# adamnelsonarcher/BB-OCR

Hardware: AMD Instinct MI355X
Metric: book-page images/sec end-to-end (detect+recognize) @1280x960 (higher is better)
Workload: dtype fp16

## Files before the change

bb-ocr_amd/_lib.py:

```python
from __future__ import annotations

import ctypes as C
import os

_HERE = os.path.dirname(os.path.abspath(__file__))
LIB_PATH = os.environ.get("BBOCR_LIB_PATH") or os.path.join(_HERE, "libbbocr.so")


class bbocr_config(C.Structure):
    _fields_ = [("device", C.c_int), ("det_sub_batch", C.c_int), ("rec_max_cols", C.c_int), ("precision", C.c_int), ("call_slots", C.c_int),
                ("host_threads", C.c_int), ("reserved", C.c_int * 2)]


PRECISIONS = {"bf16": 0, "fp16": 1, "exact": 2, "mixed": 3, "exact_rec": 4}
PAGE_GRAY, PAGE_BGR, PAGE_RGB, PAGE_YCBCR4, PAGE_YCBCR3 = 0, 1, 2, 3, 4
PAGE_PX_BYTES = {PAGE_GRAY: 1, PAGE_BGR: 3, PAGE_RGB: 3, PAGE_YCBCR4: 4, PAGE_YCBCR3: 3}


class bbocr_tensor_desc(C.Structure):
    _fields_ = [("name", C.c_char_p), ("ndim", C.c_int), ("shape", C.c_int64 * 4), ("data", C.POINTER(C.c_float))]


class bbocr_params(C.Structure):
    _fields_ = [
        ("text_threshold", C.c_double), ("low_text", C.c_double), ("link_threshold", C.c_double), ("mag_ratio", C.c_double),
        ("slope_ths", C.c_double), ("ycenter_ths", C.c_double), ("height_ths", C.c_double), ("width_ths", C.c_double),
        ("add_margin", C.c_double), ("contrast_ths", C.c_double), ("adjust_contrast", C.c_double),
        ("canvas_size", C.c_int), ("min_size", C.c_int), ("ignore_mask", C.c_uint * 4), ("decoder", C.c_int), ("beam_width", C.c_int), ("rotation_info", C.c_int * 4),
    ]


class bbocr_preproc_params(C.Structure):
    _fields_ = [("scale", C.c_double), ("blur_sigma", C.c_double), ("contrast", C.c_double), ("brightness", C.c_double),
                ("clahe_clip", C.c_double), ("unsharp_radius", C.c_double), ("unsharp_percent", C.c_int), ("unsharp_threshold", C.c_int),
                ("reserved", C.c_int * 4)]


class bbocr_jpeg_plan(C.Structure):
    _fields_ = [("width", C.c_int), ("height", C.c_int), ("components", C.c_int), ("sampling", (C.c_int * 2) * 3), ("restart_interval", C.c_int),
                ("mcu_cols", C.c_int), ("mcu_rows", C.c_int), ("segments", C.c_int), ("scan_offset", C.c_longlong), ("scan_bytes", C.c_longlong),
                ("supported", C.c_int), ("reason", C.c_int), ("orientation", C.c_int), ("reserved", C.c_int * 3)]


class bbocr_boxlist(C.Structure):
    _fields_ = [
        ("n_images", C.c_int), ("poly_off", C.POINTER(C.c_int)), ("polys", C.POINTER(C.c_int)),
        ("hori_off", C.POINTER(C.c_int)), ("hori", C.POINTER(C.c_int)),
        ("free_off", C.POINTER(C.c_int)), ("free_q", C.POINTER(C.c_double)),
    ]


class bbocr_result(C.Structure):
    _fields_ = [
        ("n_images", C.c_int), ("box_off", C.POINTER(C.c_int)), ("quads", C.POINTER(C.c_double)),
        ("is_free", C.POINTER(C.c_int)), ("text_off", C.POINTER(C.c_int)), ("text_idx", C.POINTER(C.c_int)),
        ("conf", C.POINTER(C.c_double)),
    ]


_vp = C.c_void_p
PROTOTYPES = {
    "bbocr_create": (C.c_int, [C.POINTER(bbocr_config), C.POINTER(_vp)]),
    "bbocr_destroy": (None, [_vp]),
    "bbocr_last_error": (C.c_char_p, [_vp]),
    "bbocr_default_params": (None, [C.POINTER(bbocr_params)]),
    "bbocr_load_weights": (C.c_int, [_vp, C.c_int, C.POINTER(bbocr_tensor_desc), C.c_int]),
    "bbocr_alloc_weights": (C.c_int, [_vp, C.c_int]),
    "bbocr_weights_blob_size": (C.c_int, [_vp, C.POINTER(C.c_size_t)]),
    "bbocr_weights_export": (C.c_int, [_vp, _vp, C.c_size_t]),
    "bbocr_weights_import": (C.c_int, [_vp, _vp, C.c_size_t]),
    "bbocr_dist_unique_id": (C.c_int, [_vp]),
    "bbocr_dist_init": (C.c_int, [_vp, C.c_int, C.c_int, _vp]),
    "bbocr_dist_finalize": (C.c_int, [_vp]),
    "bbocr_bcast_weights": (C.c_int, [_vp, C.c_int]),
    "bbocr_scatter_images": (C.c_int, [_vp, _vp, C.c_longlong, C.c_size_t, C.c_int, _vp, C.POINTER(C.c_longlong), C.POINTER(C.c_longlong)]),
    "bbocr_gather_results": (C.c_int, [_vp, _vp, C.c_size_t, C.c_int, C.POINTER(_vp), C.POINTER(C.c_size_t)]),
    "bbocr_result_pack": (C.c_int, [C.POINTER(bbocr_result), C.POINTER(_vp), C.POINTER(C.c_size_t)]),
    "bbocr_result_unpack": (C.c_int, [_vp, C.c_size_t, C.POINTER(C.POINTER(bbocr_result))]),
    "bbocr_free_bytes": (None, [_vp]),
    "bbocr_detect_dims": (C.c_int, [C.c_int, C.c_int, C.c_int, C.c_double, C.POINTER(C.c_int), C.POINTER(C.c_int), C.POINTER(C.c_int),
                                    C.POINTER(C.c_int), C.POINTER(C.c_double)]),
    "bbocr_detect": (C.c_int, [_vp, _vp, C.c_int, C.c_int, C.c_int, C.POINTER(bbocr_params), _vp]),
    "bbocr_boxes": (C.c_int, [_vp, _vp, C.c_int, C.c_int, C.c_int, C.c_double, C.POINTER(bbocr_params), C.POINTER(C.POINTER(bbocr_boxlist))]),
    "bbocr_recognize": (C.c_int, [_vp, _vp, C.c_int, C.c_int, C.c_int, C.POINTER(bbocr_boxlist), C.POINTER(bbocr_params),
                                  C.POINTER(C.POINTER(bbocr_result))]),
    "bbocr_readtext_batch": (C.c_int, [_vp, _vp, _vp, C.c_int, C.c_int, C.c_int, C.POINTER(bbocr_params), C.POINTER(C.POINTER(bbocr_result))]),
    "bbocr_free_boxlist": (None, [C.POINTER(bbocr_boxlist)]),
    "bbocr_free_result": (None, [C.POINTER(bbocr_result)]),
    "bbocr_stage_times": (C.c_int, [_vp, C.POINTER(C.c_float), C.c_int]),
    "bbocr_set_profiling": (C.c_int, [_vp, C.c_int]),
    "bbocr_conv_profile": (C.c_int, [_vp, C.c_int, C.POINTER(C.c_double), C.POINTER(C.c_double), C.POINTER(C.c_longlong)]),
    "bbocr_host_cpu_share": (C.c_int, []),
    "bbocr_host_component_polys": (C.c_int, [C.POINTER(C.c_int), C.POINTER(C.c_int), C.c_int, C.c_int, C.c_int, C.c_double, C.POINTER(C.c_int)]),
    "bbocr_host_group_boxes": (C.c_int, [C.POINTER(C.c_int), C.c_int, C.POINTER(bbocr_params), C.POINTER(C.POINTER(bbocr_boxlist))]),
    "bbocr_host_ctc_beam": (C.c_int, [C.POINTER(C.c_float), C.c_int, C.c_int, C.c_int, C.c_int, C.c_int, C.POINTER(C.c_int), C.POINTER(C.c_int)]),
    "bbocr_op_conv2d": (C.c_int, [_vp, _vp, C.c_int, C.c_int, C.c_int, C.c_int, C.POINTER(C.c_float), C.POINTER(C.c_float), C.c_int, C.c_int,
                                  C.c_int, C.c_int, C.c_int, C.c_int, C.c_int, C.c_int, _vp, C.c_int, C.c_int, _vp]),
    "bbocr_crnn_logits": (C.c_int, [_vp, _vp, C.c_int, C.c_int, _vp]),
    "bbocr_op_ctc": (C.c_int, [_vp, _vp, C.c_int, C.c_int, C.c_int, C.c_int, C.POINTER(C.c_int), C.POINTER(C.c_int), C.POINTER(C.c_double),
                               C.POINTER(C.c_uint), C.c_int]),
    "bbocr_op_resize_u8": (C.c_int, [_vp, _vp, C.c_int, C.c_int, C.c_int, C.c_int, _vp, C.c_int, C.c_int]),
    "bbocr_op_ycc_to_rgb": (C.c_int, [_vp, _vp, C.c_size_t, C.c_int, _vp, _vp]),
    "bbocr_upload_pages": (C.c_int, [_vp, C.POINTER(C.c_void_p), C.c_int, C.c_size_t, _vp]),
    "bbocr_op_crops": (C.c_int, [_vp, _vp, C.c_int, C.c_int, C.POINTER(C.c_int), C.c_int, C.POINTER(C.c_double), C.c_int, C.c_int, C.c_float,
                                 _vp, C.POINTER(C.c_int), C.c_int]),
    "bbocr_preprocess_book_cover": (C.c_int, [_vp, _vp, C.c_int, C.c_int, _vp, C.POINTER(C.c_int), C.POINTER(C.c_int)]),
    "bbocr_preproc_defaults": (None, [C.POINTER(bbocr_preproc_params), C.c_int]),
    "bbocr_preprocess_chain": (C.c_int, [_vp, _vp, C.c_int, C.c_int, C.POINTER(bbocr_preproc_params), _vp, C.POINTER(C.c_int), C.POINTER(C.c_int)]),
    "bbocr_op_preprocess_stage": (C.c_int, [_vp, C.c_int, _vp, C.c_int, C.c_int, _vp, C.c_int, C.c_int, C.c_double]),
    "bbocr_auto_crop": (C.c_int, [_vp, _vp, C.c_int, C.c_int, C.c_longlong, C.c_int, C.c_int, C.POINTER(C.c_int), C.POINTER(C.c_int),
                                  C.POINTER(C.c_int), C.c_int, C.POINTER(C.c_int)]),
    "bbocr_op_autocrop_stage": (C.c_int, [_vp, C.c_int, _vp, C.c_int, C.c_int, C.c_longlong, C.c_int, _vp]),
    "bbocr_ocr_thumbnail": (C.c_int, [_vp, _vp, C.c_int, C.c_int, C.c_longlong, C.c_int, C.c_int, C.c_int, _vp, _vp, C.POINTER(C.c_int),
                                      C.POINTER(C.c_int)]),
    "bbocr_op_thumbnail_stage": (C.c_int, [_vp, C.c_int, _vp, C.c_int, C.c_int, C.c_longlong, C.c_int, C.c_int, C.c_int, _vp, _vp,
                                           C.POINTER(C.c_int), C.POINTER(C.c_int)]),
    "bbocr_thumbnail_dims": (C.c_int, [C.c_int, C.c_int, C.c_int, C.POINTER(C.c_int), C.POINTER(C.c_int)]),
    "bbocr_host_thumbnail_plan": (C.c_int, [C.c_int, C.c_int, C.c_int, C.POINTER(C.c_int), C.POINTER(C.c_int), C.POINTER(C.c_int),
                                            C.POINTER(C.c_int), C.POINTER(C.c_float)]),
    "bbocr_host_resample_coeffs": (C.c_int, [C.c_int, C.c_float, C.c_float, C.c_int, C.POINTER(C.c_int), C.POINTER(C.c_int), C.c_int,
                                             C.POINTER(C.c_int)]),
    "bbocr_host_jpeg_qtables": (C.c_int, [C.c_int, C.POINTER(C.c_uint16)]),
    "bbocr_host_jpeg_plan": (C.c_int, [_vp, C.c_size_t, C.POINTER(bbocr_jpeg_plan)]),
    "bbocr_jpeg_decode": (C.c_int, [_vp, C.POINTER(C.c_void_p), C.POINTER(C.c_size_t), C.c_int, C.c_int, C.POINTER(C.c_void_p),
                                    C.POINTER(C.c_longlong), C.POINTER(C.c_int)]),
    "bbocr_jpeg_imread": (C.c_int, [_vp, C.POINTER(C.c_void_p), C.POINTER(C.c_size_t), C.c_int, C.POINTER(C.c_void_p), C.POINTER(C.c_longlong),
                                    C.POINTER(C.c_int)]),
    "bbocr_page_orient": (C.c_int, [_vp, _vp, C.c_int, C.c_int, C.c_longlong, C.c_int, C.c_int, C.c_int, _vp, C.c_longlong, C.POINTER(C.c_int),
                                    C.POINTER(C.c_int)]),
    "bbocr_op_jpeg_stage": (C.c_int, [_vp, C.c_int, _vp, C.c_size_t, C.c_int, _vp, C.c_size_t, C.POINTER(C.c_int)]),
    "bbocr_jpeg_encode_bound": (C.c_size_t, [C.c_int, C.c_int, C.c_int]),
    "bbocr_host_jpeg_header": (C.c_int, [C.c_int, C.c_int, C.c_int, C.c_int, _vp, C.c_int, _vp, C.c_size_t, C.POINTER(C.c_size_t)]),
    "bbocr_jpeg_encode": (C.c_int, [_vp, _vp, C.c_int, C.c_int, C.c_longlong, C.c_int, C.c_int, C.c_int, _vp, C.c_int, _vp, C.c_size_t,
                                    C.POINTER(C.c_size_t)]),
    "bbocr_op_jpeg_encode_stage": (C.c_int, [_vp, C.c_int, _vp, C.c_int, C.c_int, C.c_longlong, C.c_int, C.c_int, C.c_int, _vp, C.c_size_t,
                                             C.POINTER(C.c_size_t)]),
}

_lib = None


def load():
    global _lib
    if _lib is not None:
        return _lib
    if not os.path.exists(LIB_PATH):
        raise RuntimeError(
            f"{LIB_PATH} is missing: the MI355X backend has no CPU fallback. "
            "Build it with `python -c 'import __graft_entry__ as g; g.build()'` (hipcc --offload-arch=gfx950).")
    try:
        import torch
    except Exception:
        pass
    lib = C.CDLL(LIB_PATH)
    for name, (res, args) in PROTOTYPES.items():
        try:
            fn = getattr(lib, name)
        except AttributeError as e:
            raise RuntimeError(f"libbbocr.so does not export {name}") from e
        fn.restype = res
        fn.argtypes = args
    _lib = lib
    return lib
```

bb-ocr_amd/csrc/abi_ops.cpp:

```cpp
#include "ctx.h"

extern "C" {

int bbocr_op_preprocess_stage(bbocr_ctx* ctx, int stage, const uint8_t* dev_src, int H, int W, uint8_t* dev_dst, int dh, int dw, double param) {
    return guarded(ctx, [&](bbocr_ctx* ctx) {
        if (!dev_src || !dev_dst || H <= 0 || W <= 0 || dh <= 0 || dw <= 0) fail(BBOCR_ERR_ARG, "bad arguments");
        if (stage != 0 && (dh != H || dw != W)) fail(BBOCR_ERR_ARG, "only stage 0 changes the size");
        const size_t n = (size_t)H * W;
        if (stage == 0) {
            pp_resize(ctx, dev_src, H, W, dev_dst, dh, dw);
        } else if (stage == 1) {
            pp_gauss(ctx, dev_src, H, W, dev_dst, param);
        } else if (stage == 2 || stage == 3) {
            if (stage == 2) {
                ctx->pp_a.ensure(n);
                pp_gauss(ctx, dev_src, H, W, (uint8_t*)ctx->pp_a.p, 0.0);
            }
            HIPCHK(launch_pp_lut(dev_src, dev_dst, pp_fold_lut(ctx, n, stage == 2 ? param : 0.0, stage == 3 ? param : 0.0), n, ctx->stream));
        } else if (stage == 4) {
            pp_clahe(ctx, dev_src, H, W, pp_fold_lut(ctx, n, 0.0, 0.0), dev_dst, param);
        } else if (stage == 5) {
            ctx->pp_b.ensure(n);
            ctx->pp_c.ensure(n);
            pp_unsharp(ctx, dev_src, H, W, dev_dst, (uint8_t*)ctx->pp_b.p, (uint8_t*)ctx->pp_c.p, (float)param, 30, 3);
        } else if (stage == 7) {
            ctx->pp_b.ensure(n);
            ctx->pp_c.ensure(n);
            pp_unsharp(ctx, dev_src, H, W, dev_dst, (uint8_t*)ctx->pp_b.p, (uint8_t*)ctx->pp_c.p, 1.0f, (int)param, 3);
        } else if (stage == 6) {
            HIPCHK(launch_gray(dev_src, dev_dst, n, ctx->stream));
        } else {
            fail(BBOCR_ERR_ARG, "unknown pre-processing stage");
        }
        slot_sync(ctx, ctx->stream);
    });
}

int bbocr_host_cpu_share(void) { return host_cpu_share(); }

int bbocr_host_component_polys(const int* comps, const int* rowext, int n, int w, int h, double ratio, int* polys_out) {
    if (!comps || !rowext || !polys_out || n < 0 || w <= 0 || h <= 0 || !(ratio > 0)) return BBOCR_ERR_ARG;
    try {
        for (int i = 0; i < n; ++i) {
            const int* q = comps + (size_t)i * 7;
            bbocr::Component cc{q[0], q[1], q[2], q[3], q[4], q[5], q[6]};
            float box[4][2];
            bbocr::component_box(cc, rowext + (size_t)cc.row_off * 2, w, h, box);
            bbocr::box_to_poly(box, 1.0 / ratio, 1.0 / ratio, polys_out + (size_t)i * 8);
        }
    } catch (...) {
        return BBOCR_ERR_INTERNAL;
    }
    return BBOCR_OK;
}

int bbocr_host_group_boxes(const int* polys, int n, const bbocr_params* p, bbocr_boxlist** out) {
    if ((!polys && n > 0) || n < 0 || !out) return BBOCR_ERR_ARG;
    try {
        bbocr_params pp;
        bbocr_default_params(&pp);
        if (p) pp = *p;
        HostBoxes hb;
        hb.polys.assign(1, {});
        hb.hori.assign(1, {});
        hb.freeb.assign(1, {});
        for (int i = 0; i < n; ++i) {
            std::array<int, 8> a;
            memcpy(a.data(), polys + (size_t)i * 8, 32);
            hb.polys[0].push_back(a);
        }
        bbocr::GroupParams gp{pp.slope_ths, pp.ycenter_ths, pp.height_ths, pp.width_ths, pp.add_margin, pp.min_size};
        bbocr::group_text_box(hb.polys[0], gp, hb.hori[0], hb.freeb[0]);
        *out = export_boxes(hb);
    } catch (...) {
        return BBOCR_ERR_INTERNAL;
    }
    return BBOCR_OK;
}

int bbocr_host_ctc_beam(const float* probs, int n, int T, int C, int cs, int beam_width, int* text_off, int* text_idx) {
    if (!probs || !text_off || !text_idx || n <= 0 || T <= 0 || C <= 0 || C > cs || beam_width <= 0) return BBOCR_ERR_ARG;
    try {
        std::vector<int> seqs;
        for (int i = 0; i < n; ++i) { seqs.push_back(i * T); seqs.push_back(T); }
        std::vector<std::vector<int>> texts;
        ctc_beam_search_batch(probs, seqs.data(), n, C, cs, beam_width, texts);
        int o = 0;
        for (int i = 0; i < n; ++i) {
            text_off[i] = o;
            for (int v : texts[i]) text_idx[o++] = v;
        }
        text_off[n] = o;
    } catch (...) {
        return BBOCR_ERR_INTERNAL;
    }
    return BBOCR_OK;
}

int bbocr_op_conv2d(bbocr_ctx* ctx, const uint16_t* dev_in, int N, int H, int W, int Cin, const float* w, const float* bias, int Cout, int KH,
                    int KW, int pad, int dil, int relu_in, int relu_out, int out_f32, void* dev_out, int pool_mode, int pool_relu,
                    uint16_t* dev_pool_out) {
    return guarded(ctx, [&](bbocr_ctx* ctx) {
        if (!dev_in || !w || Cin <= 0 || (Cin & 31) || Cout <= 0 || KH <= 0 || KW <= 0) fail(BBOCR_ERR_ARG, "bad conv arguments");
        if (pool_mode < 0 || pool_mode > 2 || (pool_mode ? (!dev_pool_out || out_f32) : !dev_out)) fail(BBOCR_ERR_ARG, "bad conv output arguments");
        ConvPlan p = make_plan(Cin, Cout, KH, KW, pad, dil, det_el(ctx));
        std::vector<float> wv(w, w + (size_t)Cout * Cin * KH * KW), bv(Cout, 0.f);
        if (bias) std::copy(bias, bias + Cout, bv.begin());
        const size_t owned0 = ctx->owned.size();
        upload_plan(ctx, p, wv, bv);
        const int store = cdiv(Cout, 16) * 16;
        ConvArgs a = conv_args(p, Act{(uint16_t*)dev_in, N, H, W, Cin});
        a.relu_in0 = relu_in != 0; a.relu_out = relu_out != 0; a.out_f32 = out_f32 != 0;
        a.out = dev_out; a.out_cs = store; a.cout_store = store;
        a.pool_mode = pool_mode; a.pool_relu = pool_relu != 0; a.store_full = (pool_mode && dev_out) ? 1 : 0; a.pool_cs = store; a.pool_out = dev_pool_out;
        a.zero = ctx->zero_page;
        const hipError_t e = launch_conv(p, a, ctx->stream);
        const hipError_t e2 = hipStreamSynchronize(ctx->stream);
        while (ctx->owned.size() > owned0) { (void)hipFree(ctx->owned.back()); ctx->owned.pop_back(); ctx->owned_bytes.pop_back(); }
        HIPCHK(e);
        HIPCHK(e2);
    }, true);
}

int bbocr_crnn_logits(bbocr_ctx* ctx, const uint16_t* dev_crops, int n, int imgW, float* dev_logits) {
    return guarded(ctx, [&](bbocr_ctx* ctx) {
        if (!ctx->crnn_loaded) fail(BBOCR_ERR_STATE, "recogniser weights not loaded");
        if (!dev_crops || !dev_logits || n <= 0 || imgW < 64 || (imgW & 63)) fail(BBOCR_ERR_ARG, "bad crop batch");
        std::vector<BoxJob> jobs(n);
        std::vector<int> all(n);
        for (int i = 0; i < n; ++i) { jobs[i].d = CropDesc{}; jobs[i].d.imgW = imgW; all[i] = i; }
        RecPart part;
        rec_plan_part(jobs, all, 0, 0, part);
        const size_t rows = part.rows, rows_pad = align_up(rows, 256);
        ctx->seq_v.ensure(rows_pad * 256 * 2 * (rec_split(ctx) ? 2 : 1));
        ctx->seq_logits.ensure(rows_pad * 112 * 4);
        const CropDesc* dd = rec_upload_descs(ctx, part, ctx->crop_desc);
        uint16_t* wide = rec_wide_image(ctx, part);
        HIPCHK(hipMemsetAsync(wide, 0, 64 * part.cols * 2, ctx->stream));
        for (int i = 0; i < n; ++i)
            HIPCHK(hipMemcpy2DAsync(wide + part.descs[i].slot, part.cols * 2, dev_crops + (size_t)i * 64 * imgW, (size_t)imgW * 2, (size_t)imgW * 2, 64,
                                    hipMemcpyDeviceToDevice, ctx->stream));
        crnn_features_wide(ctx, part, dd, wide);
        RecRun run;
        rec_add_tables(run, part, lstm_tile_seqs(rec_mode(ctx)));
        ctx->seq_tables.ensure(run.tiles.size() * 4);
        HIPCHK(hipMemcpyAsync(ctx->seq_tables.p, run.tiles.data(), run.tiles.size() * 4, hipMemcpyHostToDevice, ctx->stream));
        crnn_sequence(ctx, rows_pad, (const int*)ctx->seq_tables.p, (int)(run.tiles.size() / 4), (float*)ctx->seq_logits.p);
        HIPCHK(hipMemcpyAsync(dev_logits, ctx->seq_logits.p, rows * 112 * 4, hipMemcpyDeviceToDevice, ctx->stream));
        slot_sync(ctx, ctx->stream);
    });
}

int bbocr_op_ctc(bbocr_ctx* ctx, const float* dev_logits, int n, int T, int C, int cs, int* text_off, int* text_idx, double* conf,
                 const unsigned int* ignore_mask, int beam_width) {
    return guarded(ctx, [&](bbocr_ctx* ctx) {
        if (!dev_logits || !text_off || !text_idx || !conf || n <= 0 || T <= 0 || C <= 0 || C > cs) fail(BBOCR_ERR_ARG, "bad ctc arguments");
        const bool beam = beam_width > 0;
        const size_t rows = (size_t)n * T;
        ctc_size(ctx, rows, n, cs, beam);
        std::vector<int> seqs;
        for (int i = 0; i < n; ++i) { seqs.push_back(i * T); seqs.push_back(T); }
        ctx->seq_tables.ensure(seqs.size() * 4);
        HIPCHK(hipMemcpyAsync(ctx->seq_tables.p, seqs.data(), seqs.size() * 4, hipMemcpyHostToDevice, ctx->stream));
        HIPCHK(launch_ctc(dev_logits, rows, C, cs, (const int*)ctx->seq_tables.p, n, (int*)ctx->ctc_idx.p, (float*)ctx->ctc_pmax.p,
                          (int*)ctx->ctc_out_idx.p, (CtcOut*)ctx->ctc_out.p, ctx->stream, ignore_mask, beam ? (float*)ctx->ctc_probs.p : nullptr));
        std::vector<int> oidx(rows);
        std::vector<CtcOut> oo(n);
        std::vector<float> probs(beam ? rows * cs : 0);
        std::vector<std::vector<int>> beam_texts;
        HIPCHK(hipMemcpyAsync(oidx.data(), ctx->ctc_out_idx.p, oidx.size() * 4, hipMemcpyDeviceToHost, ctx->stream));
        HIPCHK(hipMemcpyAsync(oo.data(), ctx->ctc_out.p, oo.size() * sizeof(CtcOut), hipMemcpyDeviceToHost, ctx->stream));
        if (beam) HIPCHK(hipMemcpyAsync(probs.data(), ctx->ctc_probs.p, probs.size() * sizeof(float), hipMemcpyDeviceToHost, ctx->stream));
        slot_sync(ctx, ctx->stream);
        if (beam) ctc_beam_search_batch(probs.data(), seqs.data(), n, C, cs, beam_width, beam_texts, &host_pool(ctx));
        std::vector<int> text;
        int o = 0;
        for (int i = 0; i < n; ++i) {
            text_off[i] = o;
            conf[i] = ctc_decode(oo[i], oidx.data() + (size_t)i * T, beam ? &beam_texts[i] : nullptr, text);
            for (int v : text) text_idx[o++] = v;
        }
        text_off[n] = o;
    });
}

int bbocr_op_resize_u8(bbocr_ctx* ctx, const uint8_t* dev_src, int N, int sh, int sw, int C, uint8_t* dev_dst, int dh, int dw) {
    return guarded(ctx, [&](bbocr_ctx* ctx) {
        if (!dev_src || !dev_dst || N <= 0 || sh <= 0 || sw <= 0 || dh <= 0 || dw <= 0 || C <= 0) fail(BBOCR_ERR_ARG, "bad resize arguments");
        HIPCHK(launch_resize_u8(dev_src, N, sh, sw, C, dev_dst, dh, dw, ctx->stream));
        slot_sync(ctx, ctx->stream);
    });
}

int bbocr_op_ycc_to_rgb(bbocr_ctx* ctx, const uint8_t* dev_ycc, size_t npix, int pixel_stride, uint8_t* dev_rgb, uint8_t* dev_gray) {
    return guarded(ctx, [&](bbocr_ctx* ctx) {
        if (!dev_ycc || !dev_rgb || npix == 0 || (pixel_stride != 3 && pixel_stride != 4)) fail(BBOCR_ERR_ARG, "bad colour-conversion arguments");
        HIPCHK(launch_ycc_to_rgb_gray(dev_ycc, pixel_stride, dev_rgb, dev_gray, npix, ctx->stream));
        slot_sync(ctx, ctx->stream);
    });
}

int bbocr_upload_pages(bbocr_ctx* root, const void* const* host_pages, int n, size_t bytes_each, void* dev_dst) {
    return lane_guarded(root, &bbocr_ctx::upload_lane, false, [&](hipStream_t st) {
        if (!host_pages || !dev_dst || n <= 0 || bytes_each == 0) fail(BBOCR_ERR_ARG, "bad upload arguments");
        for (int k = 0; k < n; ++k)
            if (!host_pages[k]) fail(BBOCR_ERR_ARG, "null page");
        for (int k = 0; k < n; ++k)
            HIPCHK(hipMemcpyAsync((unsigned char*)dev_dst + (size_t)k * bytes_each, host_pages[k], bytes_each, hipMemcpyHostToDevice, st));
        HIPCHK(hipStreamSynchronize(st));
    });
}

int bbocr_op_crops(bbocr_ctx* ctx, const uint8_t* dev_gray, int H, int W, const int* hori, int n_hori, const double* free_q, int n_free, int imgW,
                   float contrast, uint16_t* dev_out, int* n_out, int mode) {
    return guarded(ctx, [&](bbocr_ctx* ctx) {
        if (!dev_gray || !dev_out || !n_out || imgW < 64 || (imgW & 63) || mode < 0 || mode > 4) fail(BBOCR_ERR_ARG, "bad crop arguments");
        std::vector<BoxJob> jobs;
        auto take = [&](BoxJob& j) {
            if (mode == 0) {
                if (j.d.imgW == imgW) jobs.push_back(j);
                return;
            }
            j.d.imgW = imgW;
            j.d.rot = mode - 1;
            if (j.d.rot & 1) std::swap(j.d.rw, j.d.rh);
            crop_refit_fw(j.d);
            jobs.push_back(j);
        };
        for (int i = 0; i < n_hori; ++i) {
            BoxJob j;
            std::array<int, 4> b;
            memcpy(b.data(), hori + (size_t)i * 4, 16);
            if (plan_horizontal(b, 0, H, W, j)) take(j);
        }
        for (int i = 0; i < n_free; ++i) {
            BoxJob j;
            std::array<double, 8> f;
            memcpy(f.data(), free_q + (size_t)i * 8, 64);
            if (plan_free(f, 0, j)) take(j);
        }
        *n_out = (int)jobs.size();
        if (jobs.empty()) return;
        size_t a_total = 0, w_total = 0;
        rec_layout_scratch(jobs, 0, a_total, w_total);
        bool any_warp = false, any_tall = false;
        std::vector<CropDesc> descs;
        for (size_t i = 0; i < jobs.size(); ++i) {
            CropDesc& d = jobs[i].d;
            d.slot = (int)i;
            any_warp |= d.warp != 0;
            any_tall |= !(d.fw == d.rw && d.rh == 64);
            descs.push_back(d);
        }
        ctx->crop_scratch.ensure(std::max<size_t>(a_total, 16));
        ctx->crop_hscratch.ensure(std::max<size_t>(a_total, 16));
        ctx->crop_wscratch.ensure(std::max<size_t>(w_total, 16));
        ctx->crop_desc.ensure(descs.size() * sizeof(CropDesc));
        ctx->crop_luts.ensure(descs.size() * 256);
        HIPCHK(hipMemcpyAsync(ctx->crop_desc.p, descs.data(), descs.size() * sizeof(CropDesc), hipMemcpyHostToDevice, ctx->stream));
        HIPCHK(launch_crops(dev_gray, H, W, (const CropDesc*)ctx->crop_desc.p, 0, (int)descs.size(), imgW, any_warp, any_tall,
                            (uint8_t*)ctx->crop_wscratch.p, (uint8_t*)ctx->crop_scratch.p, (uint8_t*)ctx->crop_hscratch.p,
                            (const uint8_t*)ctx->crop_luts.p, dev_out, 1, ctx->stream));
        if (contrast > 0) {
            ctx->crop_hist.ensure(descs.size() * 256 * 4);
            HIPCHK(launch_crop_hist((const uint8_t*)ctx->crop_scratch.p, (const CropDesc*)ctx->crop_desc.p, 0, (int)descs.size(),
                                    (unsigned int*)ctx->crop_hist.p, ctx->stream));
            std::vector<unsigned int> hist(descs.size() * 256);
            HIPCHK(hipMemcpyAsync(hist.data(), ctx->crop_hist.p, hist.size() * 4, hipMemcpyDeviceToHost, ctx->stream));
            slot_sync(ctx, ctx->stream);
            std::vector<uint8_t> luts(descs.size() * 256);
            for (size_t k = 0; k < descs.size(); ++k)
                if (contrast_lut(&hist[k * 256], (size_t)descs[k].rw * descs[k].rh, (double)contrast, &luts[k * 256])) descs[k].lut_off = (int)(k * 256);
            HIPCHK(hipMemcpyAsync(ctx->crop_luts.p, luts.data(), luts.size(), hipMemcpyHostToDevice, ctx->stream));
            HIPCHK(hipMemcpyAsync(ctx->crop_desc.p, descs.data(), descs.size() * sizeof(CropDesc), hipMemcpyHostToDevice, ctx->stream));
        }
        HIPCHK(launch_crops(dev_gray, H, W, (const CropDesc*)ctx->crop_desc.p, 0, (int)descs.size(), imgW, any_warp, any_tall,
                            (uint8_t*)ctx->crop_wscratch.p, (uint8_t*)ctx->crop_scratch.p, (uint8_t*)ctx->crop_hscratch.p,
                            (const uint8_t*)ctx->crop_luts.p, dev_out, 2, ctx->stream, 0, 0, rec_mode(ctx)));
        slot_sync(ctx, ctx->stream);
    });
}

}
```

bb-ocr_amd/csrc/common.h:

```cpp
#pragma once
#include <hip/hip_runtime.h>
#include <stdint.h>
#include <atomic>
#include <string>

typedef __attribute__((ext_vector_type(8))) __bf16 bf16x8;
typedef __attribute__((ext_vector_type(8))) short s16x8;
typedef __attribute__((ext_vector_type(4))) float f32x4;
typedef __attribute__((ext_vector_type(4))) unsigned int u32x4;
typedef __attribute__((ext_vector_type(2))) unsigned int u32x2;

static inline uint16_t f32_to_bf16_host(float f) {
    uint32_t u;
    __builtin_memcpy(&u, &f, 4);
    if ((u & 0x7fffffffu) > 0x7f800000u) return (uint16_t)((u >> 16) | 0x40);
    u += 0x7fffu + ((u >> 16) & 1u);
    return (uint16_t)(u >> 16);
}
static inline float bf16_to_f32_host(uint16_t h) {
    uint32_t u = ((uint32_t)h) << 16;
    float f;
    __builtin_memcpy(&f, &u, 4);
    return f;
}

__device__ __forceinline__ float bf16_bits_to_f32(unsigned short h) {
    return __uint_as_float(((unsigned int)h) << 16);
}
__device__ __forceinline__ unsigned short f32_to_bf16_bits(float f) {
    __bf16 b = (__bf16)f;
    return __builtin_bit_cast(unsigned short, b);
}
typedef __attribute__((ext_vector_type(2))) __bf16 bf16x2_t;
typedef __attribute__((ext_vector_type(2))) float f32x2_t;
__device__ __forceinline__ unsigned int pack_bf16x2(float lo, float hi) {
    const f32x2_t v = {lo, hi};
    return __builtin_bit_cast(unsigned int, __builtin_convertvector(v, bf16x2_t));
}

typedef __attribute__((ext_vector_type(8))) _Float16 f16x8;
typedef __attribute__((ext_vector_type(2))) _Float16 f16x2_t;
static inline uint16_t f32_to_f16_host(float f) {
    const _Float16 h = (_Float16)f;
    uint16_t u;
    __builtin_memcpy(&u, &h, 2);
    return u;
}
static inline float f16_to_f32_host(uint16_t u) {
    _Float16 h;
    __builtin_memcpy(&h, &u, 2);
    return (float)h;
}
static inline uint16_t f32_to_el_host(int el, float f) { return el ? f32_to_f16_host(f) : f32_to_bf16_host(f); }
static inline float el_to_f32_host(int el, uint16_t u) { return el ? f16_to_f32_host(u) : bf16_to_f32_host(u); }

template <int EL> struct El;
template <> struct El<0> {
    typedef bf16x8 v8;
    static __device__ __forceinline__ f32x4 mfma(v8 a, v8 b, f32x4 c) { return __builtin_amdgcn_mfma_f32_16x16x32_bf16(a, b, c, 0, 0, 0); }
    static __device__ __forceinline__ unsigned int pack2(float lo, float hi) { return pack_bf16x2(lo, hi); }
    static __device__ __forceinline__ f32x2_t unpack2(unsigned int q) { return (f32x2_t){__uint_as_float(q << 16), __uint_as_float(q & 0xffff0000u)}; }
    static __device__ __forceinline__ unsigned short from_f32(float f) { return f32_to_bf16_bits(f); }
    static __device__ __forceinline__ float to_f32(unsigned short h) { return bf16_bits_to_f32(h); }
};
template <> struct El<1> {
    typedef f16x8 v8;
    static __device__ __forceinline__ f32x4 mfma(v8 a, v8 b, f32x4 c) { return __builtin_amdgcn_mfma_f32_16x16x32_f16(a, b, c, 0, 0, 0); }
    static __device__ __forceinline__ unsigned int pack2(float lo, float hi) {
        const f32x2_t v = {lo, hi};
        return __builtin_bit_cast(unsigned int, __builtin_convertvector(v, f16x2_t));
    }
    static __device__ __forceinline__ f32x2_t unpack2(unsigned int q) { return __builtin_convertvector(__builtin_bit_cast(f16x2_t, q), f32x2_t); }
    static __device__ __forceinline__ unsigned short from_f32(float f) { return __builtin_bit_cast(unsigned short, (_Float16)f); }
    static __device__ __forceinline__ float to_f32(unsigned short h) { return (float)__builtin_bit_cast(_Float16, h); }
};
__device__ __forceinline__ s16x8 sm16_key(s16x8 x) { return x ^ ((x >> 15) & (short)0x7fff); }

__device__ __forceinline__ int xcd_remap(int bid, int nblk) {
    const int q = nblk >> 3, r = nblk & 7, x = bid & 7, i = bid >> 3;
    return (x < r ? x * (q + 1) : r * (q + 1) + (x - r) * q) + i;
}

#define HIP_TRY(expr)                                                                      \
    do {                                                                                   \
        hipError_t _e = (expr);                                                            \
        if (_e != hipSuccess) {                                                            \
            throw std::string(#expr) + ": " + hipGetErrorString(_e);                       \
        }                                                                                  \
    } while (0)

static constexpr int kMaxDev = 32;
struct LdsOptIn {
    std::atomic<size_t> hw[kMaxDev];
};
static inline hipError_t lds_opt_in(LdsOptIn& st, const void* fn, size_t smem) {
    int d = 0;
    hipError_t e = hipGetDevice(&d);
    if (e != hipSuccess) return e;
    if (d < 0 || d >= kMaxDev) return hipErrorInvalidDevice;
    size_t cur = st.hw[d].load(std::memory_order_acquire);
    if (smem <= cur) return hipSuccess;
    e = hipFuncSetAttribute(fn, hipFuncAttributeMaxDynamicSharedMemorySize, (int)smem);
    if (e != hipSuccess) return e;
    while (cur < smem && !st.hw[d].compare_exchange_weak(cur, smem, std::memory_order_release)) {}
    return hipSuccess;
}
static inline int device_cus() {
    static std::atomic<int> n[kMaxDev];
    int d = 0;
    if (hipGetDevice(&d) != hipSuccess || d < 0 || d >= kMaxDev) return 256;
    int v = n[d].load(std::memory_order_acquire);
    if (v) return v;
    hipDeviceProp_t prop;
    v = (hipGetDeviceProperties(&prop, d) == hipSuccess && prop.multiProcessorCount > 0) ? prop.multiProcessorCount : 256;
    n[d].store(v, std::memory_order_release);
    return v;
}
```

bb-ocr_amd/csrc/conv_mfma.hip:

```cpp
#include "common.h"
#include "kernels.h"
#include <type_traits>
#include <utility>

__device__ __forceinline__ void lds_dma16(const void* gptr, const void* lds) {
    const unsigned la = (unsigned)(size_t)(const __attribute__((address_space(3))) void*)lds;
    asm volatile("s_mov_b32 m0, %1\n\ts_nop 0\n\tglobal_load_lds_dwordx4 %0, off" ::"v"(gptr), "s"(la) : "memory");
}

template <int EL, int MF, bool ADDUP = false>
__device__ __forceinline__ void conv_epilogue(const ConvArgs& a, f32x4 (&acc)[MF][4], int n, int nt, int oy0, int ox0, int wm, int wn, int fpr,
                                              int lane, int BN, int sub = 1, int sph = 0, int spw = 0) {
    const int g = lane >> 4, pl = lane & 15;
    const int cout0 = nt * BN + wn * 64 + g * 8;
    if (a.tail) {
        const float* tw = a.tail;
        const typename El<EL>::v8 w1f = *(const typename El<EL>::v8*)(a.tail_frag + lane * 8);
        float cb[8], b1r[4], w2a[4], w2b[4];
#pragma unroll
        for (int i = 0; i < 8; ++i) cb[i] = a.bias[(g & 1) * 8 + i];
#pragma unroll
        for (int r = 0; r < 4; ++r) { b1r[r] = tw[4 * g + r]; w2a[r] = tw[16 + 4 * g + r]; w2b[r] = tw[32 + 4 * g + r]; }
        const float b20 = tw[48], b21 = tw[49];
#pragma unroll
// ... 176 lines not shown
            store_frag(a.out, (size_t)(n * a.OH + oy) * a.OW * a.out_cs, a.out_cs, ox0 + fc * 16, a.OW, rowok && oy < a.OH, v, a.out_f32);
        }
        return;
    }
    auto pooled = [&](auto fpr_c) {
        constexpr int FPR = decltype(fpr_c)::value;
        if constexpr (MF % (2 * FPR) == 0) {
            const int POH = a.OH >> 1, POW = a.pool_mode == 1 ? (a.OW >> 1) : a.OW;
#pragma unroll
            for (int f = 0; f < MF; ++f) {
                if ((f / FPR) & 1) continue;
                const int F = wm * MF + f;
                const int fr = F / FPR, fc = F - fr * FPR;
                const int oy = oy0 + fr, xb = ox0 + fc * 16, ox = xb + pl;
                float v0[16], v1[16], m[16];
#pragma unroll
                for (int j = 0; j < 4; ++j)
#pragma unroll
                    for (int r = 0; r < 4; ++r) {
                        float x0 = fmaf(acc[f][j][r], sc, bs[j * 4 + r]), x1 = fmaf(acc[f + FPR][j][r], sc, bs[j * 4 + r]);
                        if (a.relu_out) { x0 = fmaxf(x0, 0.f); x1 = fmaxf(x1, 0.f); }
                        v0[j * 4 + r] = x0;
                        v1[j * 4 + r] = x1;
                        float p = fmaxf(x0, x1);
                        if (a.pool_relu) p = fmaxf(p, 0.f);
                        m[j * 4 + r] = p;
                    }
                if (a.store_full) {
                    store_frag(a.out, (size_t)(n * a.OH + oy) * a.OW * a.out_cs, a.out_cs, xb, a.OW, oy < a.OH, v0, a.out_f32);
                    store_frag(a.out, (size_t)(n * a.OH + oy + 1) * a.OW * a.out_cs, a.out_cs, xb, a.OW, oy + 1 < a.OH, v1, a.out_f32);
                }
                const int py = oy >> 1;
                const size_t prow = (size_t)(n * POH + py) * POW * a.pool_cs;
                if (a.pool_mode == 1) {
#pragma unroll
                    for (int i = 0; i < 16; ++i)
                        m[i] = fmaxf(m[i], __int_as_float(__builtin_amdgcn_update_dpp(0, __float_as_int(m[i]), 0xB1, 0xF, 0xF, true)));
                    const int px = ox >> 1;
                    auto store_pooled = [&](const float (&mv)[16], int coff) {
                        u32x4 lo, hi;
                        pack_runs(mv, lo, hi);
                        uint16_t* op = (uint16_t*)a.pool_out + prow + (size_t)px * a.pool_cs + cout0 + coff;
                        if (fullw) {
                            if (py < POH && px < POW) *(u32x4*)(op + (pl & 1) * 32) = (pl & 1) ? hi : lo;
                        } else if (!(pl & 1) && py < POH && px < POW) {
                            *(u32x4*)(op) = lo;
                            if (run1) *(u32x4*)(op + 32) = hi;
                        }
                    };
                    if (a.split_off) {
                        float mh[16], ml[16];
                        split_hi_lo(m, mh, ml);
                        store_pooled(mh, 0);
                        store_pooled(ml, a.split_off);
                    } else {
                        store_pooled(m, 0);
                    }
                } else {
                    store_frag(a.pool_out, prow, a.pool_cs, xb, POW, py < POH, m, false);
                }
            }
        }
    };
    if (fpr == 1) pooled(std::integral_constant<int, 1>{});
    else if (fpr == 2) pooled(std::integral_constant<int, 2>{});
    else pooled(std::integral_constant<int, 4>{});
}

template <int EL, int MF>
__device__ __forceinline__ void conv_epilogue_pool2x2_lean(const ConvArgs& a, f32x4 (&acc)[MF][4], int n, int oy0, int ox0, int wm, int lane,
                                                           int cout_base = 0) {
    static_assert(MF % 2 == 0, "fragment f and f + 1 are the two rows of a pooling window");
    const int g = lane >> 4, pl = lane & 15, odd = pl & 1;
    const int cout0 = cout_base + g * 8;
    const float sc = a.acc_scale;
    const float floor_v = (a.relu_out || a.pool_relu) ? 0.f : -__builtin_inff();
    float bsel[8];
#pragma unroll
    for (int q = 0; q < 2; ++q) {
        const f32x4 b4 = *(const f32x4*)(a.bias + cout0 + odd * 32 + q * 4);
        bsel[q * 4 + 0] = b4[0]; bsel[q * 4 + 1] = b4[1]; bsel[q * 4 + 2] = b4[2]; bsel[q * 4 + 3] = b4[3];
    }
    const int POH = a.OH >> 1, POW = a.OW >> 1;
    const int px = (ox0 + pl) >> 1;
#pragma unroll
    for (int f = 0; f < MF; f += 2) {
        const int py = (oy0 + wm * MF + f) >> 1;
        float o[8];
#pragma unroll
        for (int i = 0; i < 8; ++i) {
            const int i1 = 8 + i;
            float q0 = fmaxf(acc[f][i >> 2][i & 3], acc[f + 1][i >> 2][i & 3]);
            float q1 = fmaxf(acc[f][i1 >> 2][i1 & 3], acc[f + 1][i1 >> 2][i1 & 3]);
            q0 = fmaxf(q0, __int_as_float(__builtin_amdgcn_update_dpp(0, __float_as_int(q0), 0xB1 , 0xF, 0xF, true)));
            q1 = fmaxf(q1, __int_as_float(__builtin_amdgcn_update_dpp(0, __float_as_int(q1), 0xB1, 0xF, 0xF, true)));
            o[i] = fmaxf(fmaf(odd ? q1 : q0, sc, bsel[i]), floor_v);
        }
        const u32x4 pk = {El<EL>::pack2(o[0], o[1]), El<EL>::pack2(o[2], o[3]), El<EL>::pack2(o[4], o[5]), El<EL>::pack2(o[6], o[7])};
        uint16_t* op = (uint16_t*)a.pool_out + ((size_t)(n * POH + py) * POW + px) * a.pool_cs + cout0 + odd * 32;
        if (py < POH && px < POW) *(u32x4*)op = pk;
    }
}

template <int EL, int MF>
__device__ __forceinline__ void conv_epilogue_plain_lean(const ConvArgs& a, f32x4 (&acc)[MF][4], int n, int nt, int oy0, int ox0, int wm, int wn,
                                                         int fpr, int lane, int BN) {
    typedef short s16x2_t __attribute__((ext_vector_type(2)));
    const int g = lane >> 4, pl = lane & 15;
    const int cout0 = nt * BN + wn * 64 + g * 8;
    float bs[16];
#pragma unroll
    for (int h = 0; h < 2; ++h)
#pragma unroll
        for (int q = 0; q < 2; ++q) {
            const f32x4 b4 = *(const f32x4*)(a.bias + cout0 + h * 32 + q * 4);
            bs[h * 8 + q * 4 + 0] = b4[0]; bs[h * 8 + q * 4 + 1] = b4[1]; bs[h * 8 + q * 4 + 2] = b4[2]; bs[h * 8 + q * 4 + 3] = b4[3];
        }
    const bool relu = a.relu_out != 0;
    const bool inside = oy0 + a.TH <= a.OH && ox0 + a.TW <= a.OW;
    const s16x2_t z2 = {0, 0};
    const size_t lane_off = (size_t)(pl & 7) * a.out_cs + cout0 + (pl >> 3) * 32;
#pragma unroll
    for (int f = 0; f < MF; ++f) {
        const int F = wm * MF + f;
        const int fr = F / fpr, fc = F - fr * fpr;
        const int oy = oy0 + fr, xb = ox0 + fc * 16;
        unsigned int p[8];
#pragma unroll
        for (int i = 0; i < 8; ++i) {
            const int k = 2 * i;
            unsigned int q = El<EL>::pack2(acc[f][k >> 2][k & 3] + bs[k], acc[f][(k + 1) >> 2][(k + 1) & 3] + bs[k + 1]);
            if (relu) q = __builtin_bit_cast(unsigned int, __builtin_elementwise_max(__builtin_bit_cast(s16x2_t, q), z2));
            p[i] = q;
        }
        uint16_t* op = (uint16_t*)a.out + ((size_t)(n * a.OH + oy) * a.OW + xb) * a.out_cs + lane_off;
        u32x4 dA, dB;
#pragma unroll
        for (int i = 0; i < 4; ++i) {
            dA[i] = (unsigned)__builtin_amdgcn_update_dpp((int)p[i], (int)p[4 + i], 0x118 , 0xF, 0xC, false);
            dB[i] = (unsigned)__builtin_amdgcn_update_dpp((int)p[4 + i], (int)p[i], 0x108 , 0xF, 0x3, false);
        }
        if (inside) {
            *(u32x4*)op = dA;
            *(u32x4*)(op + (size_t)8 * a.out_cs) = dB;
        } else {
            const int xA = xb + (pl & 7);
            if (oy < a.OH && xA < a.OW) *(u32x4*)op = dA;
            if (oy < a.OH && xA + 8 < a.OW) *(u32x4*)(op + (size_t)8 * a.out_cs) = dB;
        }
    }
}

template <int EL, int MF>
__device__ __forceinline__ void conv_epilogue_post1x1(const ConvArgs& a, f32x4 (&acc)[MF][4], int n, int oy0, int ox0, int wm, int fpr, int lane) {
    const int g = lane >> 4, pl = lane & 15;
    const int cout0 = g * 8;
    const float sc = a.acc_scale;
    const float floor_v = a.relu_out ? 0.f : -__builtin_inff();
    float bs[16];
#pragma unroll
    for (int h = 0; h < 2; ++h)
#pragma unroll
        for (int q = 0; q < 2; ++q) {
            const f32x4 b4 = *(const f32x4*)(a.bias + cout0 + h * 32 + q * 4);
            bs[h * 8 + q * 4 + 0] = b4[0]; bs[h * 8 + q * 4 + 1] = b4[1]; bs[h * 8 + q * 4 + 2] = b4[2]; bs[h * 8 + q * 4 + 3] = b4[3];
        }
    typename El<EL>::v8 wf[2][4];
#pragma unroll
    for (int ks = 0; ks < 2; ++ks)
#pragma unroll
        for (int j = 0; j < 4; ++j) wf[ks][j] = *(const typename El<EL>::v8*)(a.post_w + ((size_t)(ks * 4 + j) * 64 + lane) * 8);
#pragma unroll
    for (int f = 0; f < MF; ++f) {
        const int F = wm * MF + f;
        const int fr = F / fpr, fc = F - fr * fpr;
        const int oy = oy0 + fr, xb = ox0 + fc * 16;
        u32x4 bk[2];
#pragma unroll
        for (int h = 0; h < 2; ++h)
#pragma unroll
            for (int i = 0; i < 4; ++i) {
                const int k = h * 8 + i * 2;
                const float x0 = fmaxf(fmaf(acc[f][k >> 2][k & 3], sc, bs[k]), floor_v), x1 = fmaxf(fmaf(acc[f][(k + 1) >> 2][(k + 1) & 3], sc, bs[k + 1]), floor_v);
                bk[h][i] = El<EL>::pack2(x0, x1);
            }
        f32x4 y[4];
#pragma unroll
        for (int j = 0; j < 4; ++j) {
            y[j] = El<EL>::mfma(wf[0][j], __builtin_bit_cast(typename El<EL>::v8, bk[0]), (f32x4){0.f, 0.f, 0.f, 0.f});
            y[j] = El<EL>::mfma(wf[1][j], __builtin_bit_cast(typename El<EL>::v8, bk[1]), y[j]);
        }
        const u32x4 lo = {El<EL>::pack2(y[0][0], y[0][1]), El<EL>::pack2(y[0][2], y[0][3]), El<EL>::pack2(y[1][0], y[1][1]), El<EL>::pack2(y[1][2], y[1][3])};
        const u32x4 hi = {El<EL>::pack2(y[2][0], y[2][1]), El<EL>::pack2(y[2][2], y[2][3]), El<EL>::pack2(y[3][0], y[3][1]), El<EL>::pack2(y[3][2], y[3][3])};
        u32x4 dA, dB;
#pragma unroll
        for (int i = 0; i < 4; ++i) {
            dA[i] = (unsigned)__builtin_amdgcn_update_dpp((int)lo[i], (int)hi[i], 0x118 , 0xF, 0xC, false);
            dB[i] = (unsigned)__builtin_amdgcn_update_dpp((int)hi[i], (int)lo[i], 0x108 , 0xF, 0x3, false);
        }
        const int co = cout0 + (pl >> 3) * 32;
        const int xA = xb + (pl & 7), xB = xb + 8 + (pl & 7);
        uint16_t* op = (uint16_t*)a.out + (size_t)(n * a.OH + oy) * a.OW * a.out_cs + co;
        if (oy < a.OH && xA < a.OW) *(u32x4*)(op + (size_t)xA * a.out_cs) = dA;
        if (oy < a.OH && xB < a.OW) *(u32x4*)(op + (size_t)xB * a.out_cs) = dB;
    }
}

void pack_post1x1_weights(const float* w, uint16_t* out, int el) {
    size_t o = 0;
    for (int ks = 0; ks < 2; ++ks)
        for (int nf = 0; nf < 4; ++nf)
            for (int l = 0; l < 64; ++l) {
                const int row = l & 15;
                const int cout = (nf >> 1) * 32 + (row >> 2) * 8 + (nf & 1) * 4 + (row & 3);
                for (int j = 0; j < 8; ++j) out[o++] = f32_to_el_host(el, w[(size_t)cout * 64 + ks * 32 + 8 * (l >> 4) + j]);
            }
}

template <int EL, int WM, int WN, int MF, int PITER>
__global__ void __launch_bounds__(WM * WN * 64, 2) conv_mfma_kernel(const ConvArgs a) {
    constexpr int NW = WM * WN, NT = NW * 64, BN = WN * 64;
    constexpr int WBUF = BN * 64;
    constexpr int WPIECES = WBUF / 16;
    extern __shared__ __attribute__((aligned(16))) unsigned char smem[];
    constexpr int WRING = 2;
    unsigned char* const wbuf = smem;
    unsigned char* const pbuf = smem + WRING * WBUF;
    const int patch_bytes = a.NP * 64;

    const int tid = threadIdx.x;
    const int lane = tid & 63;
    const int wave = __builtin_amdgcn_readfirstlane(tid >> 6);
    const int wm = wave / WN, wn = wave % WN;

    int bid = xcd_remap(blockIdx.x, gridDim.x);
    const int nt = bid % a.ntiles_n;
    bid /= a.ntiles_n;
    const int tx = bid % a.tiles_x;
    bid /= a.tiles_x;
    const int ty = bid % a.tiles_y;
    const int n = bid / a.tiles_y;
    const int oy0 = ty * a.TH, ox0 = tx * a.TW;
    const int iy0 = oy0 - a.pad_h, ix0 = ox0 - a.pad_w;
    const int nk = a.nchunks * a.ntaps;

    const int n_wi = a.NP >> 4;
    const int l_pix = (lane & 7) + ((lane >> 5) << 3);
    const int l_kg = (lane >> 3) & 3;
    int src_pix[PITER];
#pragma unroll
    for (int it = 0; it < PITER; ++it) {
        const int wi = wave + it * NW;
        int sp = -1;
        if (wi < n_wi) {
            const int pix = wi * 16 + l_pix;
            const int py = pix / a.PW, px = pix - py * a.PW;
            const int iy = iy0 + py, ix = ix0 + px;
            if (py < a.PH && iy >= 0 && iy < a.H && ix >= 0 && ix < a.W) sp = (n * a.H + iy) * a.W + ix;
        }
        src_pix[it] = sp;
    }
    constexpr int NPART = (PITER + 3) / 4, PH = PITER / NPART;
    u32x4 pre[PH];
    auto load_part = [&](int chunk, auto part_c) {
        constexpr int part = decltype(part_c)::value;
        const int c = chunk * 32;
        const bool s0 = c < a.C0;
        const uint16_t* src = s0 ? a.in0 : a.in1;
        const int cs = s0 ? a.in0_cs : a.in1_cs;
        const int cb = (s0 ? c : c - a.C0) + l_kg * 8;
#pragma unroll
        for (int i = 0; i < PH; ++i) {
            const int sp = src_pix[part * PH + i];
            u32x4 v = {0u, 0u, 0u, 0u};
            if (sp >= 0) v = *(const u32x4*)(src + (size_t)sp * cs + cb);
            pre[i] = v;
        }
    };
    auto store_part = [&](int chunk, auto part_c) {
        constexpr int part = decltype(part_c)::value;
        unsigned char* pb = pbuf + (chunk & 1) * patch_bytes;
        const bool relu = (chunk * 32 < a.C0) ? a.relu_in0 : a.relu_in1;
#pragma unroll
        for (int i = 0; i < PH; ++i) {
            const int wi = wave + (part * PH + i) * NW;
            if (wi < n_wi) {
                u32x4 v = pre[i];
                if (relu) {
                    const s16x8 z = {0, 0, 0, 0, 0, 0, 0, 0};
                    v = __builtin_bit_cast(u32x4, __builtin_elementwise_max(__builtin_bit_cast(s16x8, v), z));
                }
                *(u32x4*)(pb + (size_t)(l_kg * a.NP + wi * 16 + l_pix) * 16) = v;
            }
        }
    };
    using P0 = std::integral_constant<int, 0>;
    const int S = (a.ntaps - 1) / NPART;
    auto stage_patch_load = [&](int chunk, int tap) {
        if (tap == 0) load_part(chunk, P0{});
        if constexpr (NPART > 1) { if (tap == S) load_part(chunk, std::integral_constant<int, (NPART > 1 ? 1 : 0)>{}); }
        if constexpr (NPART > 2) { if (tap == 2 * S) load_part(chunk, std::integral_constant<int, (NPART > 2 ? 2 : 0)>{}); }
        if constexpr (NPART > 3) { if (tap == 3 * S) load_part(chunk, std::integral_constant<int, (NPART > 3 ? 3 : 0)>{}); }
    };
    auto stage_patch_store = [&](int chunk, int tap) {
        if (tap == S - 1) store_part(chunk, P0{});
        if constexpr (NPART > 1) { if (tap == 2 * S - 1) store_part(chunk, std::integral_constant<int, (NPART > 1 ? 1 : 0)>{}); }
        if constexpr (NPART > 2) { if (tap == 3 * S - 1) store_part(chunk, std::integral_constant<int, (NPART > 2 ? 2 : 0)>{}); }
        if constexpr (NPART > 3) { if (tap == 4 * S - 1) store_part(chunk, std::integral_constant<int, (NPART > 3 ? 3 : 0)>{}); }
    };
    auto stage_patch_now = [&](int chunk) {
        load_part(chunk, P0{});
        store_part(chunk, P0{});
        if constexpr (NPART > 1) { load_part(chunk, std::integral_constant<int, (NPART > 1 ? 1 : 0)>{}); store_part(chunk, std::integral_constant<int, (NPART > 1 ? 1 : 0)>{}); }
        if constexpr (NPART > 2) { load_part(chunk, std::integral_constant<int, (NPART > 2 ? 2 : 0)>{}); store_part(chunk, std::integral_constant<int, (NPART > 2 ? 2 : 0)>{}); }
        if constexpr (NPART > 3) { load_part(chunk, std::integral_constant<int, (NPART > 3 ? 3 : 0)>{}); store_part(chunk, std::integral_constant<int, (NPART > 3 ? 3 : 0)>{}); }
    };
    const unsigned char* wsrc = (const unsigned char*)a.wpk + (size_t)nt * nk * WBUF;
    auto issue_w = [&](int ks, int buf) {
#pragma unroll
        for (int p0 = 0; p0 < WPIECES; p0 += NT) {
            if (p0 + wave * 64 < WPIECES) {
                __builtin_amdgcn_global_load_lds(
                    (const __attribute__((address_space(1))) void*)(wsrc + (size_t)ks * WBUF + (size_t)(p0 + tid) * 16),
                    (__attribute__((address_space(3))) void*)(wbuf + buf * WBUF + (p0 + wave * 64) * 16), 16, 0, 0);
            }
        }
    };

    const int fpr = a.TW >> 4;
    int frag_off[MF];
#pragma unroll
    for (int f = 0; f < MF; ++f) {
        const int F = wm * MF + f;
        const int fr = F / fpr, fc = F - fr * fpr;
        frag_off[f] = (fr * a.PW + fc * 16) * 16;
    }
    const int lane_patch_off = ((lane >> 4) * a.NP + (lane & 15)) * 16;
    const int lane_w_off = wn * 4 * 1024 + lane * 16;

    f32x4 acc[MF][4];
#pragma unroll
    for (int f = 0; f < MF; ++f)
#pragma unroll
        for (int j = 0; j < 4; ++j) acc[f][j] = (f32x4){0.f, 0.f, 0.f, 0.f};

    {
        issue_w(0, 0);
        stage_patch_now(0);
        __syncthreads();
        int ks = 0;
        for (int c = 0; c < a.nchunks; ++c) {
            const bool more = (c + 1 < a.nchunks);
            if (more && a.ntaps < 3) load_part(c + 1, P0{});
            const unsigned char* pbase = pbuf + (c & 1) * patch_bytes + lane_patch_off;
            int ky = 0, kx = 0;
            for (int tap = 0; tap < a.ntaps; ++tap, ++ks) {
                if (more && a.ntaps >= 3) stage_patch_load(c + 1, tap);
                if (ks + 1 < nk) issue_w(ks + 1, (ks + 1) & 1);
                const unsigned char* wb = wbuf + (ks & 1) * WBUF + lane_w_off;
                typename El<EL>::v8 af[4];
#pragma unroll
                for (int j = 0; j < 4; ++j) af[j] = *(const typename El<EL>::v8*)(wb + j * 1024);
                const unsigned char* pb = pbase + ((ky * a.PW + kx) * a.dil) * 16;
                typename El<EL>::v8 bq[MF];
#pragma unroll
                for (int f = 0; f < MF; ++f) bq[f] = *(const typename El<EL>::v8*)(pb + frag_off[f]);
#pragma unroll
                for (int f = 0; f < MF; ++f) {
#pragma unroll
                    for (int j = 0; j < 4; ++j) acc[f][j] = El<EL>::mfma(af[j], bq[f], acc[f][j]);
                }
                __builtin_amdgcn_sched_group_barrier(0x100, 4 + MF, 0);
                __builtin_amdgcn_sched_group_barrier(0x008, 4 * MF, 0);
                if (more) {
                    if (a.ntaps >= 3) stage_patch_store(c + 1, tap);
                    else if (tap == a.ntaps - 1) store_part(c + 1, P0{});
                }
                __syncthreads();
                if (++kx == a.KW) { kx = 0; ++ky; }
            }
        }
    }

    conv_epilogue<EL, MF>(a, acc, n, nt, oy0, ox0, wm, wn, fpr, lane, BN);
}

template <int EL, int WM, int WN, int MF, int NPB, int RING, int NPS = NPB * 64, bool FUSE1 = false, int NF = 4, int EPI = 0, int KS = 3>
__global__ void __launch_bounds__(WM * WN * 64, 2) conv3x3_dma_kernel(const ConvArgs a) {
    constexpr int NTAP = KS * KS, PAD = KS == 3 ? 1 : 0;
    static_assert((KS == 3 || KS == 2) && (KS == 3 || (!FUSE1 && EPI == 0)), "kernel size");
    constexpr int NW = WM * WN, NT = NW * 64, BN = WN * 64;
    static_assert(NW == 4, "one wave per 8-channel group of the patch");
    constexpr int WBUF = BN * 64, WPIECES = WBUF / 16, WPT = WPIECES / NT;
    static_assert(WPIECES % NT == 0 && (RING == 3 || RING == 4), "uniform DMA issue");
    constexpr int NP = NPS, PSLOTS = NTAP + 1 - RING;
    constexpr int PPER = (NPB + PSLOTS - 1) / PSLOTS;
    static_assert(NPS <= NPB * 64 && NPS > (NPB - 1) * 64 && NPS % 4 == 0, "patch size");
    static_assert(PSLOTS >= 1 && PPER * PSLOTS >= NPB, "patch does not fit the DMA schedule");
    extern __shared__ __attribute__((aligned(16))) unsigned char smem[];
    unsigned char* const wbuf = smem;
    unsigned char* const pbuf = smem + RING * WBUF;
    constexpr int patch_bytes = NP * 64;

    const int tid = threadIdx.x;
    const int lane = tid & 63;
    const int wave = __builtin_amdgcn_readfirstlane(tid >> 6);
    const int wm = wave / WN, wn = wave % WN;
    const int sub = a.sub;
    const int nk = a.nchunks * NTAP;
    const int fpr = FUSE1 ? 1 : a.TW >> 4;
    const int PW = FUSE1 ? 18 : a.PW;

    const int tile = xcd_remap(blockIdx.x, gridDim.x);
    struct Geo {
        int n, nt, oy0, ox0, sph, spw;
        const unsigned char* wsrc;
    };
    auto geom = [&](int id, Geo& g) {
        g.nt = id % a.ntiles_n;
        id /= a.ntiles_n;
        const int tx = id % a.tiles_x;
        id /= a.tiles_x;
        const int ty = id % a.tiles_y;
        int n = id / a.tiles_y;
        g.sph = 0; g.spw = 0;
        g.n = n;
        g.oy0 = ty * a.TH; g.ox0 = tx * a.TW;
        g.wsrc = (const unsigned char*)a.wpk + (size_t)g.nt * nk * WBUF;
    };
    int spix[NPB];
    const int pw_magic = (65536 + a.PW - 1) / a.PW;
    const int stack_magic = ((1 << 20) + a.stack) / (a.stack + 1);
    auto geom_pix = [&](const Geo& g) {
        const int iy0 = g.oy0 - PAD, ix0 = g.ox0 - PAD;
#pragma unroll
        for (int pb = 0; pb < NPB; ++pb) {
            const int pix = pb * 64 + lane;
            const int py = (pix * pw_magic) >> 16, px = pix - py * a.PW;
            int ly = iy0 + py;
            const int lx = ix0 + px;
            int sph = 0, spw = 0;
            bool rowok = ly >= 0;
            if (sub > 1) {
                const int vy = ly < 0 ? 0 : ly;
                const int q = (vy * stack_magic) >> 20;
                ly = vy - q * (a.stack + 1);
                sph = q / sub;
                spw = q - sph * sub;
                rowok = rowok && ly < a.stack && q < sub * sub;
            }
            const int iy = ly * sub + sph, ix = lx * sub + spw;
            spix[pb] = (py < a.PH && rowok && iy < a.H && lx >= 0 && ix < a.W) ? (g.n * a.H + iy) * a.W + ix : -1;
        }
    };
    Geo cur;
    geom(tile, cur);
    if constexpr (!FUSE1) geom_pix(cur);

    auto issue_p = [&](int sp, int chunk, int par, auto pb_c) {
        constexpr int pb = decltype(pb_c)::value;
        const int c = chunk * 32;
        const bool s0 = c < a.C0;
        const uint16_t* src = s0 ? a.in0 : a.in1;
        const int cs = s0 ? a.in0_cs : a.in1_cs;
        const int cb = (s0 ? c : c - a.C0) + wave * 8;
        const uint16_t* gp = sp >= 0 ? src + (size_t)sp * cs + cb : (const uint16_t*)a.zero;
        if ((pb + 1) * 64 <= NPS || pb * 64 + lane < NPS)
            lds_dma16(gp, pbuf + par * patch_bytes + (wave * NP + pb * 64) * 16);
    };
    auto issue_w = [&](const unsigned char* slice, int slot) {
#pragma unroll
        for (int p0 = 0; p0 < WPIECES; p0 += NT) lds_dma16(slice + (size_t)(p0 + tid) * 16, wbuf + slot * WBUF + (p0 + wave * 64) * 16);
    };
    int frag_off[MF];
#pragma unroll
    for (int f = 0; f < MF; ++f) {
        const int F = wm * MF + f;
        const int fr = F / fpr, fc = F - fr * fpr;
        frag_off[f] = (fr * PW + fc * 16) * 16;
    }
    const int lane_patch_off = ((lane >> 4) * NP + (lane & 15)) * 16;
    const int lane_w_off = wn * 4 * 1024 + lane * 16;

    struct Sched {
        static constexpr int pcnt(int tap) {
            if (FUSE1 || tap >= PSLOTS) return 0;
            const int base = NPB / PSLOTS, extra = NPB % PSLOTS;
            return base + (tap < extra ? 1 : 0);
        }
        static constexpr int pfirst(int tap) { int s = 0; for (int t = 0; t < tap; ++t) s += pcnt(t); return s; }
        static constexpr int wcnt(bool more, int tap) { return (more || tap < NTAP - (RING - 1)) ? WPT : 0; }
        static constexpr int younger(bool more, int tap) {
            int nv = wcnt(more, tap) + (more ? pcnt(tap) : 0);
            for (int back = 1; back <= RING - 2; ++back) {
                const int t = tap - back;
                const bool m = t >= 0 ? more : true;
                const int tt = t >= 0 ? t : t + NTAP;
                const int pc = m ? pcnt(tt) : 0;
                nv += (back == RING - 2) ? pc : (wcnt(m, tt) + pc);
            }
            return nv;
        }
    };
    static_assert(FUSE1 || Sched::pfirst(NTAP) == NPB, "patch DMA schedule must cover the patch");

#pragma unroll
    for (int i = 0; i < RING - 1; ++i)
        if (i < nk) issue_w(cur.wsrc + (size_t)i * WBUF, i);
    if constexpr (!FUSE1) {
        [&]<int... PB>(std::integer_sequence<int, PB...>) { (issue_p(spix[PB], 0, 0, std::integral_constant<int, PB>{}), ...); }(std::make_integer_sequence<int, NPB>{});
    } else {
        static_assert(!FUSE1 || (RING == 3 && BN == 64 && NPS == 324), "fused conv1_1 producer: 16x16 tiles, 3-deep ring of 4 KB slices");
        u32x2* const rgbp = (u32x2*)(wbuf + 2 * WBUF);
        const uint8_t* rgb = (const uint8_t*)a.in0;
        const float m0 = 0.485f * 255.0f, m1 = 0.456f * 255.0f, m2 = 0.406f * 255.0f;
        const float s0 = 0.229f * 255.0f, s1 = 0.224f * 255.0f, s2 = 0.225f * 255.0f;
        static_assert(NT == 256, "two patch pixels per thread");
        int pq[2];
        bool on_canvas[2];
        unsigned int cr[2], cg[2], cb[2];
#pragma unroll
        for (int it = 0; it < 2; ++it) {
            const int p = tid + it * NT;
            const int py = p / 20, px = p - py * 20;
            const int iy = cur.oy0 - 2 + py, ix = cur.ox0 - 2 + px;
            pq[it] = p;
            on_canvas[it] = p < 400 && iy >= 0 && iy < a.H && ix >= 0 && ix < a.W;
            const bool on_page = on_canvas[it] && iy < a.rgb_H && ix < a.rgb_W;
            const uint8_t* q = rgb + (on_page ? ((size_t)(cur.n * a.rgb_H + iy) * a.rgb_W + ix) * 3 : (size_t)cur.n * a.rgb_H * a.rgb_W * 3);
            cr[it] = q[0]; cg[it] = q[1]; cb[it] = q[2];
            if (!on_page) { cr[it] = 0u; cg[it] = 0u; cb[it] = 0u; }
        }
        typename El<EL>::v8 w1[4];
#pragma unroll
        for (int j = 0; j < 4; ++j) w1[j] = *(const typename El<EL>::v8*)(a.c11_w + ((size_t)j * 64 + lane) * 8);
        const int g = lane >> 4, pl = lane & 15;
        f32x4 b1[4];
#pragma unroll
        for (int h = 0; h < 2; ++h)
#pragma unroll
            for (int q4 = 0; q4 < 2; ++q4) b1[h * 2 + q4] = *(const f32x4*)(a.c11_b + h * 32 + g * 8 + q4 * 4);
        __builtin_amdgcn_sched_barrier(0);
#pragma unroll
        for (int it = 0; it < 2; ++it) {
            if (pq[it] < 400) {
                u32x2 v = {0u, 0u};
                if (on_canvas[it]) {
                    v[0] = El<EL>::pack2(((float)cr[it] - m0) / s0, ((float)cg[it] - m1) / s1);
                    v[1] = El<EL>::pack2(((float)cb[it] - m2) / s2, 0.f);
                }
                rgbp[pq[it]] = v;
            }
        }
        __syncthreads();
        auto frag_geo = [&](int fi, int& pp, int& py, int& px) {
            pp = fi * 16 + pl;
            py = pp / 18;
            px = pp - py * 18;
        };
#pragma unroll
        for (int b3 = 0; b3 < 2; ++b3) {
            typename El<EL>::v8 bfr[3];
            int pps[3], pys[3], pxs[3];
#pragma unroll
            for (int q = 0; q < 3; ++q) {
                const int fi = wave + (b3 * 3 + q) * NW;
                frag_geo(fi < 21 ? fi : 20, pps[q], pys[q], pxs[q]);
                const int pc = pps[q] < 324 ? pys[q] * 20 + pxs[q] : 0;
                const int t0 = 2 * g, t1 = t0 + 1;
                const u32x2 a0 = rgbp[pc + (t0 / 3) * 20 + (t0 % 3)];
                const u32x2 a1 = rgbp[pc + (t1 / 3) * 20 + (t1 % 3)];
                const u32x2 t8 = rgbp[pc + 2 * 20 + 2];
                const unsigned int x = g == 0 ? (t8[0] << 16) : (g == 1 ? (t8[1] << 16) : 0u);
                const unsigned int y = g == 0 ? (t8[0] & 0xffff0000u) : 0u;
                bfr[q] = __builtin_bit_cast(typename El<EL>::v8, (u32x4){a0[0], a0[1] | x, a1[0], a1[1] | y});
            }
            f32x4 d[3][4];
#pragma unroll
            for (int q = 0; q < 3; ++q)
#pragma unroll
                for (int j = 0; j < 4; ++j) d[q][j] = El<EL>::mfma(w1[j], bfr[q], b1[j]);
#pragma unroll
            for (int q = 0; q < 3; ++q) {
                const int fi = wave + (b3 * 3 + q) * NW;
                const int pp = pps[q];
                const int iy = cur.oy0 - 1 + pys[q], ix = cur.ox0 - 1 + pxs[q];
                const bool inside = iy >= 0 && iy < a.H && ix >= 0 && ix < a.W;
                const float cap = inside ? __builtin_inff() : 0.f;
                if (fi < 21 && pp < 324) {
#pragma unroll
                    for (int h = 0; h < 2; ++h) {
                        u32x4 o;
#pragma unroll
                        for (int i = 0; i < 4; ++i) {
                            const int k = h * 8 + i * 2;
                            const float x0 = __builtin_amdgcn_fmed3f(d[q][k >> 2][k & 3], 0.f, cap), x1 = __builtin_amdgcn_fmed3f(d[q][(k + 1) >> 2][(k + 1) & 3], 0.f, cap);
                            o[i] = El<EL>::pack2(x0, x1);
                        }
                        *(u32x4*)(pbuf + h * patch_bytes + (g * NP + pp) * 16) = o;
                    }
                }
            }
        }
    }
    asm volatile("s_waitcnt vmcnt(0) lgkmcnt(0)\n\ts_barrier" ::: "memory");

    int wslot = 0, par = 0;
    const unsigned char* wp = cur.wsrc + (size_t)(RING - 1) * WBUF;
    f32x4 acc[MF][4];
#pragma unroll
    for (int f = 0; f < MF; ++f)
#pragma unroll
        for (int j = 0; j < 4; ++j) acc[f][j] = (f32x4){0.f, 0.f, 0.f, 0.f};
    static_assert(MF % 2 == 0 && MF >= 4, "B fragments are scheduled in pairs, four ahead");
    typename El<EL>::v8 pre[4];
    auto step = [&](auto tap_c, auto more_c, int c) {
        constexpr int tap = decltype(tap_c)::value;
        constexpr bool MORE = decltype(more_c)::value;
        constexpr int ky = tap / KS, kx = tap % KS;
        const unsigned char* wb = wbuf + wslot * WBUF + lane_w_off;
        const unsigned char* pb = pbuf + par * patch_bytes + lane_patch_off + (ky * PW + kx) * 16;
        typename El<EL>::v8 af[NF], bq[MF];
#pragma unroll
        for (int j = 0; j < NF; ++j) af[j] = *(const typename El<EL>::v8*)(wb + j * 1024);
        if constexpr (tap == 0) {
#pragma unroll
            for (int f = 0; f < 4; ++f) bq[f] = *(const typename El<EL>::v8*)(pb + frag_off[f]);
        } else {
#pragma unroll
            for (int f = 0; f < 4; ++f) bq[f] = pre[f];
        }
        if constexpr (Sched::wcnt(MORE, tap) > 0) {
            int slot = wslot + RING - 1;
            if (slot >= RING) slot -= RING;
            issue_w(wp, slot);
            wp += WBUF;
        }
        if constexpr (MORE && Sched::pcnt(tap) > 0) {
            constexpr int p0 = Sched::pfirst(tap);
            const int nc = c + 1;
            [&]<int... I>(std::integer_sequence<int, I...>) { (issue_p(spix[p0 + I], nc, par ^ 1, std::integral_constant<int, p0 + I>{}), ...); }(
                std::make_integer_sequence<int, Sched::pcnt(tap)>{});
        }
        __builtin_amdgcn_sched_barrier(0);
        constexpr int kyn = (tap + 1) / KS, kxn = (tap + 1) % KS;
        const unsigned char* pbn = pbuf + par * patch_bytes + lane_patch_off + (kyn * PW + kxn) * 16;
#pragma unroll
        for (int g = 0; g < MF / 2; ++g) {
#pragma unroll
            for (int f = 2 * g; f < 2 * g + 2; ++f)
#pragma unroll
                for (int j = 0; j < NF; ++j) acc[f][j] = El<EL>::mfma(af[j], bq[f], acc[f][j]);
            __builtin_amdgcn_sched_barrier(0);
#pragma unroll
            for (int f = 2 * g + 4; f < 2 * g + 6; ++f) {
                if (f < MF) bq[f] = *(const typename El<EL>::v8*)(pb + frag_off[f]);
                else if constexpr (tap < NTAP - 1) pre[f - MF] = *(const typename El<EL>::v8*)(pbn + frag_off[f - MF]);
            }
            __builtin_amdgcn_sched_barrier(0);
        }
        asm volatile("s_waitcnt vmcnt(%0)\n\ts_barrier" ::"n"(Sched::younger(MORE, tap)) : "memory");
        wslot = wslot + 1 == RING ? 0 : wslot + 1;
    };
    auto relu_patch = [&](int c) {
        if (!((c * 32 < a.C0) ? a.relu_in0 : a.relu_in1)) return;
        const s16x8 z = {0, 0, 0, 0, 0, 0, 0, 0};
        s16x8* pp = (s16x8*)(pbuf + par * patch_bytes);
#pragma unroll
        for (int i = 0; i < (NP * 4 + NT - 1) / NT; ++i) {
            const int k = tid + i * NT;
            if ((i + 1) * NT <= NP * 4 || k < NP * 4) pp[k] = __builtin_elementwise_max(pp[k], z);
        }
        asm volatile("s_waitcnt lgkmcnt(0)\n\ts_barrier" ::: "memory");
    };
    auto chunk = [&](auto more_c, int c) {
        relu_patch(c);
        [&]<int... T>(std::integer_sequence<int, T...>) { (step(std::integral_constant<int, T>{}, more_c, c), ...); }(std::make_integer_sequence<int, NTAP>{});
        par ^= 1;
    };
    for (int c = 0; c + 1 < a.nchunks; ++c) chunk(std::true_type{}, c);
    chunk(std::false_type{}, a.nchunks - 1);
    if constexpr (FUSE1) conv_epilogue_pool2x2_lean<EL, MF>(a, acc, cur.n, cur.oy0, cur.ox0, wm, lane);
    else if constexpr (EPI == 1) conv_epilogue_post1x1<EL, MF>(a, acc, cur.n, cur.oy0, cur.ox0, wm, fpr, lane);
    else if constexpr (KS == 3 && NF == 4) {
        if (a.lean == 1) conv_epilogue_plain_lean<EL, MF>(a, acc, cur.n, cur.nt, cur.oy0, cur.ox0, wm, wn, fpr, lane, BN);
        else if (a.lean == 3) conv_epilogue_pool2x2_lean<EL, MF>(a, acc, cur.n, cur.oy0, cur.ox0, wm, lane, cur.nt * BN + wn * 64);
        else conv_epilogue<EL, MF>(a, acc, cur.n, cur.nt, cur.oy0, cur.ox0, wm, wn, fpr, lane, BN, sub, cur.sph, cur.spw);
    } else conv_epilogue<EL, MF>(a, acc, cur.n, cur.nt, cur.oy0, cur.ox0, wm, wn, fpr, lane, BN, sub, cur.sph, cur.spw);
}

template <int EL, int NCH, bool DB, int NF = 2, bool LEAN = false>
__global__ void __launch_bounds__(256, 2) conv3x3_resw_kernel(const ConvArgs a) {
    static_assert(NF == 2 || (NF == 4 && NCH == 1), "resident weights");
    constexpr int MF = 4, NP = 324, NPB = 6, NK = NCH * 9;
    constexpr int WSL = NF * 1024;
    constexpr int PCH = NP * 64;
    constexpr int NBUF = DB ? 2 : 1;
    extern __shared__ __attribute__((aligned(16))) unsigned char smem[];
    unsigned char* const wres = smem;
    unsigned char* const pbuf = smem + NK * WSL;
    const int tid = threadIdx.x, lane = tid & 63;
    const int wave = __builtin_amdgcn_readfirstlane(tid >> 6);
    const int wm = wave;
    const int ntiles = a.N * a.tiles_x * a.tiles_y;
    {
        const unsigned char* wsrc = (const unsigned char*)a.wpk;
        if constexpr (NF == 4) {
#pragma unroll
            for (int ks = 0; ks < NK; ++ks)
                __builtin_amdgcn_global_load_lds((const __attribute__((address_space(1))) void*)(wsrc + (size_t)ks * 4096 + (size_t)tid * 16),
                                                 (__attribute__((address_space(3))) void*)(wres + ks * WSL + wave * 1024), 16, 0, 0);
        } else {
#pragma unroll
            for (int k2 = 0; k2 < (NK + 1) / 2; ++k2) {
                const int ks = k2 * 2 + (tid >> 7);
                if (ks < NK)
                    __builtin_amdgcn_global_load_lds((const __attribute__((address_space(1))) void*)(wsrc + (size_t)ks * 4096 + (size_t)(tid & 127) * 16),
                                                     (__attribute__((address_space(3))) void*)(wres + (k2 * 2 + (wave >> 1)) * WSL + (wave & 1) * 1024), 16, 0, 0);
            }
        }
    }
    const int pw_magic = (65536 + 18 - 1) / 18;
    auto issue_patch = [&](int tile, int buf) {
        int id = tile;
        const int tx = id % a.tiles_x;
        id /= a.tiles_x;
        const int ty = id % a.tiles_y;
        const int n = id / a.tiles_y;
        const int iy0 = ty * 16 - 1, ix0 = tx * 16 - 1;
#pragma unroll
        for (int pb = 0; pb < NPB; ++pb) {
            const int pix = pb * 64 + lane;
            const int py = (pix * pw_magic) >> 16, px = pix - py * 18;
            const int iy = iy0 + py, ix = ix0 + px;
            const bool ok = py < 18 && iy >= 0 && iy < a.H && ix >= 0 && ix < a.W;
            const size_t sp = ((size_t)(n * a.H + iy) * a.W + ix) * a.in0_cs + wave * 8;
#pragma unroll
            for (int c = 0; c < NCH; ++c) {
                const uint16_t* gp = ok ? a.in0 + sp + c * 32 : (const uint16_t*)a.zero;
                if ((pb + 1) * 64 <= NP || pix < NP)
                    __builtin_amdgcn_global_load_lds((const __attribute__((address_space(1))) void*)gp,
                                                     (__attribute__((address_space(3))) void*)(pbuf + (buf * NCH + c) * PCH + (wave * NP + pb * 64) * 16), 16, 0, 0);
            }
        }
    };
    int frag_off[MF];
#pragma unroll
    for (int f = 0; f < MF; ++f) frag_off[f] = ((wm * MF + f) * 18) * 16;
    const int lane_patch_off = ((lane >> 4) * NP + (lane & 15)) * 16;
    const int lane_w_off = lane * 16;

    int tile = xcd_remap(blockIdx.x, gridDim.x);
    if (tile < ntiles) issue_patch(tile, 0);
    int buf = 0;
    for (; tile < ntiles; tile += gridDim.x) {
        const int next = tile + gridDim.x;
        if constexpr (DB) {
            asm volatile("s_waitcnt lgkmcnt(0)\n\ts_barrier" ::: "memory");
            if (next < ntiles) {
                issue_patch(next, buf ^ 1);
                asm volatile("s_waitcnt vmcnt(%0)\n\ts_barrier" ::"n"(NPB * NCH) : "memory");
            } else {
                asm volatile("s_waitcnt vmcnt(0)\n\ts_barrier" ::: "memory");
            }
        } else {
            asm volatile("s_waitcnt vmcnt(0)\n\ts_barrier" ::: "memory");
        }
        f32x4 acc[MF][4];
#pragma unroll
        for (int f = 0; f < MF; ++f)
#pragma unroll
            for (int j = 0; j < 4; ++j) acc[f][j] = (f32x4){0.f, 0.f, 0.f, 0.f};
#pragma unroll
        for (int c = 0; c < NCH; ++c) {
            const unsigned char* pc = pbuf + (buf * NCH + c) * PCH + lane_patch_off;
            const bool relu = a.relu_in0;
#pragma unroll
            for (int tap = 0; tap < 9; ++tap) {
                const unsigned char* wb = wres + (c * 9 + tap) * WSL + lane_w_off;
                const unsigned char* pb = pc + ((tap / 3) * 18 + (tap % 3)) * 16;
                typename El<EL>::v8 af[NF], bq[MF];
#pragma unroll
                for (int j = 0; j < NF; ++j) af[j] = *(const typename El<EL>::v8*)(wb + j * 1024);
#pragma unroll
                for (int f = 0; f < MF; ++f) bq[f] = *(const typename El<EL>::v8*)(pb + frag_off[f]);
                if (relu) {
                    const s16x8 z = {0, 0, 0, 0, 0, 0, 0, 0};
#pragma unroll
                    for (int f = 0; f < MF; ++f) bq[f] = __builtin_bit_cast(typename El<EL>::v8, __builtin_elementwise_max(__builtin_bit_cast(s16x8, bq[f]), z));
                }
#pragma unroll
                for (int f = 0; f < MF; ++f)
#pragma unroll
                    for (int j = 0; j < NF; ++j) acc[f][j] = El<EL>::mfma(af[j], bq[f], acc[f][j]);
            }
        }
        int id = tile;
        const int tx = id % a.tiles_x;
        id /= a.tiles_x;
        const int ty = id % a.tiles_y;
        const int n = id / a.tiles_y;
        if constexpr (!DB) {
            asm volatile("s_waitcnt lgkmcnt(0)\n\ts_barrier" ::: "memory");
            if (next < ntiles) issue_patch(next, 0);
        }
        if constexpr (LEAN) conv_epilogue_pool2x2_lean<EL, MF>(a, acc, n, ty * 16, tx * 16, wm, lane);
        else conv_epilogue<EL, MF>(a, acc, n, 0, ty * 16, tx * 16, wm, 0, 1, lane, 64);
        if constexpr (DB) buf ^= 1;
    }
}

template <int EL>
static hipError_t launch_resw(const ConvArgs& a, hipStream_t s) {
    const int ntiles = a.N * a.tiles_x * a.tiles_y;
    const int ncu = device_cus();
    auto go = [&](auto kern, size_t smem, int per_cu, LdsOptIn& attr) -> hipError_t {
        if (hipError_t e = lds_opt_in(attr, (const void*)kern, smem); e != hipSuccess) return e;
        const int grid = ntiles < ncu * per_cu ? ntiles : ncu * per_cu;
        hipLaunchKernelGGL(kern, dim3(grid), dim3(256), smem, s, a);
        return hipGetLastError();
    };
    constexpr size_t P = 324 * 64, W1 = 9 * 2048, W2 = 18 * 2048;
    static LdsOptIn at[3];
    if (a.cout_store == 64) return go(conv3x3_resw_kernel<EL, 1, true, 4, true>, 9 * 4096 + 2 * P, 2, at[2]);
    if (a.nchunks == 1) return go(conv3x3_resw_kernel<EL, 1, true>, W1 + 2 * P, 2, at[0]);
    return go(conv3x3_resw_kernel<EL, 2, false>, W2 + 2 * P, 2, at[1]);
}

template <int EL>
__global__ void __launch_bounds__(256, 2) conv3x3_up4_kernel(const ConvArgs a) {
    constexpr int MF = 4, NF = 2, NP = 324, NK = 18, WSL = NF * 1024, PCH = NP * 64, NFRAG = 21;
    typedef typename El<EL>::v8 v8;
    extern __shared__ __attribute__((aligned(16))) unsigned char smem[];
    unsigned char* const wres = smem;
    unsigned char* const pbuf = smem + NK * WSL;
    const int tid = threadIdx.x, lane = tid & 63;
// ... 221 lines not shown
    for (int i = 0; i < RING - 1; ++i)
        if (i < nk) issue(i, i);
    asm volatile("s_waitcnt vmcnt(0) lgkmcnt(0)\n\ts_barrier" ::: "memory");
    int slot = 0;
    for (int ks = 0; ks < nk; ++ks) {
        const bool ahead = ks + RING - 1 < nk;
        if (ahead) {
            int sl = slot + RING - 1;
            if (sl >= RING) sl -= RING;
            issue(ks + RING - 1, sl);
        }
        const unsigned char* sb = smem + slot * SLOT;
        typename El<EL>::v8 af[4], bq[MF];
#pragma unroll
        for (int j = 0; j < 4; ++j) af[j] = *(const typename El<EL>::v8*)(sb + lane_w_off + j * 1024);
#pragma unroll
        for (int f = 0; f < MF; ++f) bq[f] = *(const typename El<EL>::v8*)(sb + lane_p_off + f * 256);
        if ((ks * 32 < a.C0) ? a.relu_in0 : a.relu_in1) {
            const s16x8 z = {0, 0, 0, 0, 0, 0, 0, 0};
#pragma unroll
            for (int f = 0; f < MF; ++f) bq[f] = __builtin_bit_cast(typename El<EL>::v8, __builtin_elementwise_max(__builtin_bit_cast(s16x8, bq[f]), z));
        }
#pragma unroll
        for (int f = 0; f < MF; ++f)
#pragma unroll
            for (int j = 0; j < 4; ++j) acc[f][j] = El<EL>::mfma(af[j], bq[f], acc[f][j]);
        if (ahead) asm volatile("s_waitcnt vmcnt(%0) lgkmcnt(0)\n\ts_barrier" ::"n"((RING - 2) * (WPT + PBW)) : "memory");
        else asm volatile("s_waitcnt vmcnt(0) lgkmcnt(0)\n\ts_barrier" ::: "memory");
        slot = slot + 1 == RING ? 0 : slot + 1;
    }
    conv_epilogue<EL, MF, ADDUP>(a, acc, 0, nt, 0, px0, wm, wn, 16, lane, BN);
}

template <int EL, int WM, int WN, int MF, bool ADDUP>
static hipError_t launch_dma1x1_k(const ConvArgs& a, long long grid, hipStream_t s) {
    constexpr int RING = 3, NPX = WM * MF * 16;
    auto k = conv1x1_dma_kernel<EL, WM, WN, MF, RING, ADDUP>;
    const size_t smem = (size_t)RING * ((size_t)WN * 64 * 64 + (size_t)NPX * 64);
    static LdsOptIn attr;
    if (hipError_t e = lds_opt_in(attr, (const void*)k, smem); e != hipSuccess) return e;
    hipLaunchKernelGGL(k, dim3((int)grid), dim3(WM * WN * 64), smem, s, a);
    return hipGetLastError();
}

template <int EL, int WM, int WN, int MF>
static hipError_t launch_dma1x1(ConvArgs a, hipStream_t s) {
    constexpr int NPX = WM * MF * 16;
    const long long total = (long long)a.N * a.H * a.W;
    if (total > 0x7fffffffLL) return hipErrorInvalidValue;
    a.N = 1; a.OH = 1; a.OW = (int)total; a.TH = 1; a.TW = NPX; a.tiles_y = 1;
    a.tiles_x = (int)((total + NPX - 1) / NPX);
    const long long grid = (long long)a.tiles_x * a.ntiles_n;
    if (grid > 0x7fffffffLL) return hipErrorInvalidValue;
    return a.addup ? launch_dma1x1_k<EL, WM, WN, MF, true>(a, grid, s) : launch_dma1x1_k<EL, WM, WN, MF, false>(a, grid, s);
}

static inline int cdiv(int a, int b) { return (a + b - 1) / b; }

size_t conv_packed_elems(const ConvPlan& p) {
    return (size_t)p.Cout_pad * p.Cin_pad * p.KH * p.KW;
}

void pack_conv_weights(const ConvPlan& p, const float* w, uint16_t* out) {
    const int BN = p.BN, ntn = p.Cout_pad / BN, nch = p.Cin_pad / 32, ntaps = p.KH * p.KW, nfr = BN / 16;
    size_t o = 0;
    for (int nt = 0; nt < ntn; ++nt)
        for (int c = 0; c < nch; ++c)
            for (int tap = 0; tap < ntaps; ++tap)
                for (int fr = 0; fr < nfr; ++fr) {
                    const int wn = fr >> 2, nf = fr & 3;
                    for (int l = 0; l < 64; ++l) {
                        const int row = l & 15;
                        const int cout = nt * BN + wn * 64 + (nf >> 1) * 32 + (row >> 2) * 8 + (nf & 1) * 4 + (row & 3);
                        for (int j = 0; j < 8; ++j) {
                            const int cin = c * 32 + 8 * (l >> 4) + j;
                            float v = 0.f;
                            if (cout < p.Cout && cin < p.Cin) v = w[((size_t)cout * p.Cin + cin) * ntaps + tap];
                            out[o++] = f32_to_el_host(p.el, v);
                        }
                    }
                }
}

template <int EL, int WM, int WN, int MF, int PITER>
static hipError_t launch_one(const ConvArgs& a, size_t smem, int grid, hipStream_t s) {
    auto k = conv_mfma_kernel<EL, WM, WN, MF, PITER>;
    static LdsOptIn attr;
    if (hipError_t e = lds_opt_in(attr, (const void*)k, smem); e != hipSuccess) return e;
    hipLaunchKernelGGL(k, dim3(grid), dim3(WM * WN * 64), smem, s, a);
    return hipGetLastError();
}

template <int EL, int WM, int WN, int MF, int PITER>
static hipError_t launch_cfg(const ConvArgs& a, int grid, hipStream_t s) {
    const size_t smem = (size_t)2 * WN * 64 * 64 + (size_t)2 * a.NP * 64;
    if (smem > 160 * 1024) return hipErrorInvalidValue;
    return launch_one<EL, WM, WN, MF, PITER>(a, smem, grid, s);
}

template <int EL, int WM, int WN, int MF, int NPB, int RING, int NPS = NPB * 64, bool FUSE1 = false, int NF = 4, int EPI = 0, int KS = 3>
static hipError_t launch_dma_one(ConvArgs a, int grid, hipStream_t s) {
    auto k = conv3x3_dma_kernel<EL, WM, WN, MF, NPB, RING, NPS, FUSE1, NF, EPI, KS>;
    const size_t smem_max = (size_t)RING * WN * 64 * 64 + (size_t)2 * NPS * 64;
    const size_t smem = (a.nchunks == 1 && !FUSE1) ? smem_max - (size_t)NPS * 64 : smem_max;
    static LdsOptIn attr;
    if (hipError_t e = lds_opt_in(attr, (const void*)k, smem_max); e != hipSuccess) return e;
    {
        a.lean = 0;
        const bool plain = !FUSE1 && EPI == 0 && KS == 3 && NF == 4 && a.sub == 1 && !a.out_f32 && !a.tail && !a.split_off && !a.addup && !a.post_w &&
                           a.acc_scale == 1.f && a.cout_store == a.ntiles_n * WN * 64 && a.out_cs % 8 == 0;
        if (plain && a.pool_mode == 0 && a.out) a.lean = 1;
        else if (plain && a.pool_mode == 1 && !a.store_full && a.TH == 16 && a.TW == 16 && a.pool_out) a.lean = 3;
    }
    hipLaunchKernelGGL(k, dim3(grid), dim3(WM * WN * 64), smem, s, a);
    return hipGetLastError();
}

template <int EL, int WM, int WN, int MF>
static hipError_t launch_dma(const ConvArgs& a, int npb, int grid, hipStream_t s) {
    if constexpr (WN == 1) {
        if (a.c11_w) {
            if (!(npb == 6 && a.PH == 18 && a.PW == 18 && a.TH == 16 && a.TW == 16 && a.nchunks == 2 && a.sub == 1)) return hipErrorInvalidValue;
            if (!(a.pool_mode == 1 && !a.store_full && !a.split_off && !a.out_f32 && !a.tail && a.cout_store == 64 && a.ntiles_n == 1 && a.acc_scale > 0.f))
                return hipErrorInvalidValue;
            return launch_dma_one<EL, WM, WN, MF, 6, 3, 324, true>(a, grid, s);
        }
    }
    if (a.post_w) {
        if constexpr (WN == 1)
            if (npb == 6 && a.PH == 18 && a.PW == 18 && a.cout_store == 64 && a.ntiles_n == 1 && a.sub == 1 && !a.pool_mode && !a.split_off &&
                !a.out_f32 && !a.tail && !a.addup)
                return launch_dma_one<EL, WM, WN, MF, 6, 3, 324, false, 4, 1>(a, grid, s);
        return hipErrorNotSupported;
    }
    if constexpr (WN == 1) {
        if (npb == 6 && a.PH * a.PW == 324) {
            if (a.cout_store <= 32 && a.nchunks <= 2 && a.sub == 1 && !a.C1 && !a.pool_mode && a.TH == 16 && a.TW == 16 && a.ntiles_n == 1)
                return launch_resw<EL>(a, s);
            if (a.cout_store == 64 && a.nchunks == 1 && a.sub == 1 && !a.C1 && a.pool_mode == 1 && !a.store_full && !a.split_off && !a.out_f32 &&
                !a.tail && !a.relu_in0 && a.TH == 16 && a.TW == 16 && a.ntiles_n == 1 && a.acc_scale > 0.f)
                return launch_resw<EL>(a, s);
            if (a.cout_store <= 32) return launch_dma_one<EL, WM, WN, MF, 6, 3, 324, false, 2>(a, grid, s);
            return launch_dma_one<EL, WM, WN, MF, 6, 3, 324>(a, grid, s);
        }
        if (npb == 6) return launch_dma_one<EL, WM, WN, MF, 6, 3>(a, grid, s);
    } else if (npb == 6) {
        const size_t wb = (size_t)WN * 64 * 64, pb = (size_t)2 * npb * 64 * 64;
        return 4 * wb + pb <= 80 * 1024 ? launch_dma_one<EL, WM, WN, MF, 6, 4>(a, grid, s) : launch_dma_one<EL, WM, WN, MF, 6, 3>(a, grid, s);
    }
    if (npb == 7) return launch_dma_one<EL, WM, WN, MF, 7, 3>(a, grid, s);
    return hipErrorInvalidValue;
}

int conv_plan_bn(int Cout) {
    return Cout > 64 ? 128 : 64;
}

template <int EL>
static hipError_t launch_conv_el(const ConvPlan& p, ConvArgs a, hipStream_t s) {
    const int BN = p.BN;
    constexpr int NWV = 4;
    constexpr int BM = 256;
    a.KH = p.KH; a.KW = p.KW; a.pad_h = p.pad_h; a.pad_w = p.pad_w; a.dil = p.dil;
    a.OH = a.H + 2 * p.pad_h - (p.KH - 1) * p.dil;
    a.OW = a.W + 2 * p.pad_w - (p.KW - 1) * p.dil;
    if (a.OH <= 0 || a.OW <= 0) return hipErrorInvalidValue;
    a.ntaps = p.KH * p.KW;
    a.sub = 1;
    if (a.post_w && !(a.zero && p.KH == 3 && p.KW == 3 && p.dil == 1 && p.pad_h == 1 && p.pad_w == 1 && BN == 64 && p.Cout_pad == 64))
        return hipErrorNotSupported;
    if (a.zero && !a.pool_mode && p.KH == 3 && p.KW == 3 && p.dil > 1 && p.pad_h == p.dil && p.pad_w == p.dil) {
        const int d = p.dil, LH = cdiv(a.OH, d), LW = cdiv(a.OW, d);
        long long best = -1;
        for (int th = 16; th >= 4; th >>= 1) {
            const int tw = 256 / th, ph = th + 2, pw = tw + 2, npb = cdiv(ph * pw, 64);
            if (npb != 6 && npb != 7) continue;
            const long long cost = (long long)cdiv(d * d * (LH + 1), th) * cdiv(LW, tw);
            if (best < 0 || cost < best) { best = cost; a.TH = th; a.TW = tw; a.PH = ph; a.PW = pw; a.NP = npb * 64; }
        }
        if (best > 0 && (a.C0 + a.C1 == p.Cin_pad) && !(a.C0 & 31) && !(a.C1 & 31) && [&] {
                const long long vmax = (long long)d * d * (LH + 1) + 18, magic = ((1LL << 20) + LH) / (LH + 1);
                return vmax * (magic * (LH + 1) - (1LL << 20)) < (1LL << 20) && vmax * magic < (1LL << 31);
            }()) {
            a.sub = d;
            a.stack = LH;
            a.tiles_x = cdiv(LW, a.TW);
            a.tiles_y = cdiv(d * d * (LH + 1), a.TH);
            a.ntiles_n = p.Cout_pad / BN;
            a.nchunks = p.Cin_pad / 32;
            a.wpk = p.d_w;
            a.bias = p.d_b;
            const long long g = (long long)a.N * a.tiles_x * a.tiles_y * a.ntiles_n;
            if (g > 0 && g <= 0x7fffffffLL)
                return BN == 128 ? launch_dma<EL, 2, 2, 8>(a, a.NP / 64, (int)g, s) : launch_dma<EL, 4, 1, 4>(a, a.NP / 64, (int)g, s);
            a.sub = 1;
            a.stack = 0;
        }
    }
    const int ring = 2;
    const int max_piter = 16;
    const bool dma2x2 = a.zero && p.KH == 2 && p.KW == 2 && p.dil == 1 && p.pad_h == 0 && p.pad_w == 0 && !a.pool_mode && !a.tail &&
                        !a.addup && !a.post_w && (BN == 128 || BN == 64);
    if (dma2x2) {
        a.TH = 4; a.TW = 64; a.PH = 5; a.PW = 65; a.NP = 384;
    } else {
        long long best = -1;
        for (int th = 16; th >= 4; th >>= 1) {
            const int tw = BM / th;
            const int ph = th + (p.KH - 1) * p.dil, pw = tw + (p.KW - 1) * p.dil;
            const int np = cdiv(ph * pw, 16) * 16;
            const int pit = cdiv(np / 16, NWV), pit_r = pit <= 4 ? 4 : (pit <= 8 ? 8 : 16), nparts = pit_r / 4;
            if (pit > max_piter || (size_t)ring * BN * 64 + (size_t)2 * np * 64 > 160 * 1024) continue;
            if (a.ntaps >= 3 ? (a.ntaps - 1) / nparts < 1 : nparts > 1) continue;
            if (a.pool_mode && (BN == 128 ? 8 : 4) % (2 * (tw / 16)) != 0) continue;
            const long long tiles = (long long)cdiv(a.OH, th) * cdiv(a.OW, tw);
            const long long cost = tiles * ((long long)BM * a.ntaps + 2LL * np);
            if (best < 0 || cost < best) { best = cost; a.TH = th; a.TW = tw; a.PH = ph; a.PW = pw; a.NP = np; }
        }
        if (best < 0) return hipErrorInvalidValue;
    }
    a.tiles_x = cdiv(a.OW, a.TW);
    a.tiles_y = cdiv(a.OH, a.TH);
    a.ntiles_n = p.Cout_pad / BN;
    a.nchunks = p.Cin_pad / 32;
    if (a.C0 + a.C1 != p.Cin_pad || (a.C0 & 31) || (a.C1 & 31)) return hipErrorInvalidValue;
    if ((a.in0_cs & 7) || (a.C1 && (a.in1_cs & 7)) || (a.out_cs & (a.out_f32 ? 3 : 7)) || (a.cout_store & 15)) return hipErrorInvalidValue;
    a.wpk = p.d_w;
    a.bias = p.d_b;
    const long long grid_ll = (long long)a.N * a.tiles_x * a.tiles_y * a.ntiles_n;
    if (grid_ll <= 0 || grid_ll > 0x7fffffffLL) return hipErrorInvalidValue;
    const int grid = (int)grid_ll;
    if (a.addup && !(p.KH == 1 && p.KW == 1 && a.zero && !a.pool_mode && !a.out_f32 && !a.tail && a.cout_store % 64 == 0 &&
                     a.cout_store == p.Cout_pad))
        return hipErrorInvalidValue;
    if (p.KH == 1 && p.KW == 1 && p.pad_h == 0 && p.pad_w == 0 && a.zero && !a.pool_mode)
        return BN == 256 ? launch_dma1x1<EL, 2, 4, 8>(a, s) : (BN == 128 ? launch_dma1x1<EL, 2, 2, 8>(a, s) : launch_dma1x1<EL, 4, 1, 4>(a, s));
    if (dma2x2)
        return BN == 128 ? launch_dma_one<EL, 2, 2, 8, 6, 4, 384, false, 4, 0, 2>(a, grid, s) : launch_dma_one<EL, 4, 1, 4, 6, 3, 384, false, 4, 0, 2>(a, grid, s);
    if (p.KH == 3 && p.KW == 3 && p.dil == 1 && p.pad_h == 1 && p.pad_w == 1 && a.zero) {
        const int npb = cdiv(a.PH * a.PW, 64);
        if (npb == 6 || npb == 7) {
            a.NP = npb * 64;
            return BN == 128 ? launch_dma<EL, 2, 2, 8>(a, npb, grid, s) : launch_dma<EL, 4, 1, 4>(a, npb, grid, s);
        }
    }
    if (a.c11_w || a.addup || a.post_w) return hipErrorNotSupported;
    const int piter = cdiv(a.NP / 16, NWV);
    if (BN == 128) return piter <= 4 ? launch_cfg<EL, 2, 2, 8, 4>(a, grid, s) : (piter <= 8 ? launch_cfg<EL, 2, 2, 8, 8>(a, grid, s) : launch_cfg<EL, 2, 2, 8, 16>(a, grid, s));
    if (BN == 64) return piter <= 4 ? launch_cfg<EL, 4, 1, 4, 4>(a, grid, s) : (piter <= 8 ? launch_cfg<EL, 4, 1, 4, 8>(a, grid, s) : launch_cfg<EL, 4, 1, 4, 16>(a, grid, s));
    return hipErrorInvalidValue;
}

hipError_t launch_conv(const ConvPlan& p, ConvArgs a, hipStream_t s) {
    a.acc_scale = p.acc_scale;
    if (a.split_off && (a.out_f32 || a.tail || a.addup || p.el != 1)) return hipErrorInvalidValue;
    return p.el ? launch_conv_el<1>(p, a, s) : launch_conv_el<0>(p, a, s);
}
```

bb-ocr_amd/csrc/crnn_misc.hip:

```cpp
#include "common.h"
#include "kernels.h"

__global__ void __launch_bounds__(256) crop_warp_kernel(const uint8_t* __restrict__ gray, int H, int W, const CropDesc* __restrict__ descs,
                                                        int first, uint8_t* __restrict__ wscratch) {
    const CropDesc d = descs[first + blockIdx.y];
    if (!d.warp) return;
    const uint8_t* src = gray + (size_t)d.img * H * W;
    uint8_t* dst = wscratch + d.warp_off;
    const int total = d.sw * d.sh;
    for (int i = blockIdx.x * 256 + threadIdx.x; i < total; i += gridDim.x * 256) {
        const int x = i % d.sw, y = i / d.sw;
        const double X0 = d.Minv[0] * (double)x + (d.Minv[1] * (double)y + d.Minv[2]);
        const double Y0 = d.Minv[3] * (double)x + (d.Minv[4] * (double)y + d.Minv[5]);
        const double W0 = d.Minv[6] * (double)x + (d.Minv[7] * (double)y + d.Minv[8]);
        const double Wi = W0 != 0.0 ? 32.0 / W0 : 0.0;
        double fX = X0 * Wi, fY = Y0 * Wi;
        fX = fX < -2147483648.0 ? -2147483648.0 : (fX > 2147483647.0 ? 2147483647.0 : fX);
        fY = fY < -2147483648.0 ? -2147483648.0 : (fY > 2147483647.0 ? 2147483647.0 : fY);
        const long long X = (long long)rint(fX), Y = (long long)rint(fY);
        long long sxl = X >> 5, syl = Y >> 5;
        sxl = sxl < -32768 ? -32768 : (sxl > 32767 ? 32767 : sxl);
        syl = syl < -32768 ? -32768 : (syl > 32767 ? 32767 : syl);
        const int sx = (int)sxl, sy = (int)syl;
        const int ax = (int)(X & 31), ay = (int)(Y & 31);
// ... 239 lines not shown
                f32x2_t best = {0.f, 0.f};
#pragma unroll
                for (int py = 0; py < 2; ++py)
#pragma unroll
                    for (int px = 0; px < 2; ++px) {
                        f32x2_t a = bias;
#pragma unroll
                        for (int ky = 0; ky < 3; ++ky)
#pragma unroll
                            for (int kx = 0; kx < 3; ++kx) {
                                const f32x2_t wv = *(const f32x2_t*)(w + (ky * 3 + kx) * 32 + c);
                                const float x = v[py + ky][px + kx];
                                a = __builtin_elementwise_fma(wv, (f32x2_t){x, x}, a);
                            }
                        best = __builtin_elementwise_max(best, a);
                    }
                if constexpr (MODE == REC_SPLIT) {
                    const float h0 = El<1>::to_f32(El<1>::from_f32(best[0])), h1 = El<1>::to_f32(El<1>::from_f32(best[1]));
                    o[c2] = El<1>::pack2(h0, h1);
                    ol[c2] = El<1>::pack2((best[0] - h0) * SPLIT_LO_SCALE, (best[1] - h1) * SPLIT_LO_SCALE);
                } else {
                    o[c2] = El<MODE == REC_F16 ? 1 : 0>::pack2(best[0], best[1]);
                }
            }
            *(u32x4*)(op + c8) = o;
            if constexpr (MODE == REC_SPLIT) *(u32x4*)(op + 32 + c8) = ol;
        }
    }
}

void pack_crnn_conv0_mfma(const float* w_tap_major, uint16_t* out, int el) {
    size_t o = 0;
    for (int j = 0; j < 2; ++j)
        for (int l = 0; l < 64; ++l) {
            const int m = l & 15, kg = l >> 4;
            const int cout = 8 * (m >> 2) + 4 * j + (m & 3);
            for (int t = 0; t < 8; ++t) {
                const float v = w_tap_major[t * 32 + cout];
                const float hi = el_to_f32_host(el, f32_to_el_host(el, v));
                const float lo = el_to_f32_host(el, f32_to_el_host(el, v - hi));
                const float lo2 = el_to_f32_host(el, f32_to_el_host(el, (v - hi) - lo));
                out[o++] = f32_to_el_host(el, kg == 0 ? hi : (kg == 1 ? lo : (kg == 2 ? lo2 : 0.f)));
            }
        }
}

template <int EL>
__global__ void __launch_bounds__(256) crnn_conv0_mfma_kernel(const uint16_t* __restrict__ in, const uint16_t* __restrict__ afrag, const float* __restrict__ w,
                                                              const float* __restrict__ b, uint16_t* __restrict__ out, int W) {
    constexpr int TW = 64, PITCH = TW + 16, ROWS = 66;
    __shared__ __attribute__((aligned(16))) uint16_t tile[ROWS * PITCH];
    typedef typename El<EL>::v8 v8;
    const int tid = threadIdx.x, lane = tid & 63, wave = tid >> 6;
    const int g = lane >> 4, n = lane & 15;
    const int x0 = blockIdx.x * TW, img = blockIdx.y;
    const int OW = W >> 1;
    const uint16_t* src = in + (size_t)img * 64 * W;
    for (int idx = tid; idx < ROWS * (PITCH / 4); idx += 256) {
        const int row = idx / (PITCH / 4), ch = idx - row * (PITCH / 4);
        const int iy = row - 1, ix = x0 - 8 + ch * 4;
        u32x2 v = {0u, 0u};
        if (iy >= 0 && iy < 64 && ix >= 0 && ix + 4 <= W) v = *(const u32x2*)(src + (size_t)iy * W + ix);
        *(u32x2*)(tile + row * PITCH + ch * 4) = v;
    }
    const v8 a0 = *(const v8*)(afrag + (size_t)lane * 8), a1 = *(const v8*)(afrag + (size_t)(64 + lane) * 8);
    float w8[8], bi[8];
#pragma unroll
    for (int i = 0; i < 8; ++i) {
        w8[i] = w[8 * 32 + 8 * g + i];
        bi[i] = b[8 * g + i];
    }
    __syncthreads();
    auto frag = [&](int y, int cf, f32x4& d0, f32x4& d1) {
        const uint16_t* p = tile + (y + 1) * PITCH + 8 + cf * 16 + n;
        u32x4 bq;
#pragma unroll
        for (int i = 0; i < 4; ++i) {
            const int t0 = 2 * i, t1 = 2 * i + 1;
            const unsigned int lo = p[(t0 / 3 - 1) * PITCH + (t0 % 3 - 1)], hi = p[(t1 / 3 - 1) * PITCH + (t1 % 3 - 1)];
            bq[i] = lo | (hi << 16);
        }
        const float x8 = El<EL>::to_f32(p[PITCH + 1]);
        d0 = El<EL>::mfma(a0, __builtin_bit_cast(v8, bq), (f32x4){bi[0], bi[1], bi[2], bi[3]});
        d1 = El<EL>::mfma(a1, __builtin_bit_cast(v8, bq), (f32x4){bi[4], bi[5], bi[6], bi[7]});
#pragma unroll
        for (int r = 0; r < 4; ++r) {
            d0[r] = fmaf(w8[r], x8, d0[r]);
            d1[r] = fmaf(w8[4 + r], x8, d1[r]);
        }
    };
#pragma unroll 1
    for (int rp = 0; rp < 8; ++rp) {
        const int y = 2 * (wave * 8 + rp);
#pragma unroll
        for (int cf = 0; cf < 4; ++cf) {
            f32x4 u0, u1, l0, l1;
            frag(y, cf, u0, u1);
            frag(y + 1, cf, l0, l1);
            float m[8];
#pragma unroll
            for (int r = 0; r < 4; ++r) {
                m[r] = __builtin_fmaxf(__builtin_fmaxf(u0[r], l0[r]), 0.f);
                m[4 + r] = __builtin_fmaxf(__builtin_fmaxf(u1[r], l1[r]), 0.f);
            }
#pragma unroll
            for (int i = 0; i < 8; ++i)
                m[i] = fmaxf(m[i], __int_as_float(__builtin_amdgcn_update_dpp(0, __float_as_int(m[i]), 0xB1 , 0xF, 0xF, true)));
            const int px = (x0 + cf * 16 + n) >> 1;
            if (!(n & 1) && px < OW) {
                const u32x4 o = {El<EL>::pack2(m[0], m[1]), El<EL>::pack2(m[2], m[3]), El<EL>::pack2(m[4], m[5]), El<EL>::pack2(m[6], m[7])};
                *(u32x4*)(out + (((size_t)img * 32 + (y >> 1)) * OW + px) * 32 + 8 * g) = o;
            }
        }
    }
}

hipError_t launch_crnn_conv0(const uint16_t* in, const float* w, const float* b, uint16_t* out, int n, int W, int mode, hipStream_t s,
                             const uint16_t* afrag) {
    const size_t total = (size_t)n * 32 * (W / 2);
    if (total == 0) return hipSuccess;
    if (afrag && mode != REC_SPLIT && (W & 3) == 0 && n <= 65535) {
        const dim3 grid((W + 63) / 64, n);
        if (mode == REC_F16) hipLaunchKernelGGL(crnn_conv0_mfma_kernel<1>, grid, dim3(256), 0, s, in, afrag, w, b, out, W);
        else hipLaunchKernelGGL(crnn_conv0_mfma_kernel<0>, grid, dim3(256), 0, s, in, afrag, w, b, out, W);
        return hipGetLastError();
    }
    const int grid = (int)((total + 255) / 256 < 16384 ? (total + 255) / 256 : 16384);
    if (mode == REC_SPLIT) hipLaunchKernelGGL(crnn_conv0_kernel<REC_SPLIT>, dim3(grid), dim3(256), 0, s, in, w, b, out, n, W);
    else if (mode == REC_F16) hipLaunchKernelGGL(crnn_conv0_kernel<REC_F16>, dim3(grid), dim3(256), 0, s, in, w, b, out, n, W);
    else hipLaunchKernelGGL(crnn_conv0_kernel<REC_BF16>, dim3(grid), dim3(256), 0, s, in, w, b, out, n, W);
    return hipGetLastError();
}

template <int MODE>
__device__ __forceinline__ void rowmean3_8(const uint16_t* p0, const uint16_t* p1, const uint16_t* p2, uint16_t* o, int lo_off) {
    typedef El<MODE == REC_BF16 ? 0 : 1> E;
    const u32x4 a = *(const u32x4*)(p0), bq = *(const u32x4*)(p1), c = *(const u32x4*)(p2);
    u32x4 oh, ol;
    if constexpr (MODE == REC_SPLIT) {
        const u32x4 al = *(const u32x4*)(p0 + lo_off), bl = *(const u32x4*)(p1 + lo_off), cl = *(const u32x4*)(p2 + lo_off);
        const float inv = 1.0f / SPLIT_LO_SCALE;
#pragma unroll
        for (int j = 0; j < 4; ++j) {
            const f32x2_t m = ((E::unpack2(a[j]) + E::unpack2(al[j]) * inv) + (E::unpack2(bq[j]) + E::unpack2(bl[j]) * inv) +
                               (E::unpack2(c[j]) + E::unpack2(cl[j]) * inv)) / 3.0f;
            const f32x2_t h = E::unpack2(E::pack2(m[0], m[1]));
            oh[j] = E::pack2(h[0], h[1]);
            ol[j] = E::pack2((m[0] - h[0]) * SPLIT_LO_SCALE, (m[1] - h[1]) * SPLIT_LO_SCALE);
        }
        *(u32x4*)(o) = oh;
        *(u32x4*)(o + lo_off) = ol;
    } else {
#pragma unroll
        for (int j = 0; j < 4; ++j) {
            const f32x2_t m = (E::unpack2(a[j]) + E::unpack2(bq[j]) + E::unpack2(c[j])) / 3.0f;
            oh[j] = E::pack2(m[0], m[1]);
        }
        *(u32x4*)(o) = oh;
    }
}

__global__ void __launch_bounds__(256) crnn_zero_gaps_kernel(uint16_t* __restrict__ t, const CropDesc* __restrict__ descs, int first, int H, int Wl,
                                                             int C8, int shift, int gapw) {
    const CropDesc d = descs[first + blockIdx.x];
    const int x0 = (d.slot + d.imgW) >> shift;
    const int total = H * gapw * C8;
    for (int i = threadIdx.x; i < total; i += 256) {
        const int c8 = i % C8, r = i / C8;
        const int gx = r % gapw, y = r / gapw;
        if (x0 + gx < Wl) *(u32x4*)(t + ((size_t)y * Wl + x0 + gx) * C8 * 8 + (size_t)c8 * 8) = (u32x4){0u, 0u, 0u, 0u};
    }
}
hipError_t launch_crnn_zero_gaps(uint16_t* t, const CropDesc* descs_dev, int first, int count, int H, int Wl, int C, int shift, hipStream_t s) {
    if (count <= 0) return hipSuccess;
    hipLaunchKernelGGL(crnn_zero_gaps_kernel, dim3(count), dim3(256), 0, s, t, descs_dev, first, H, Wl, C / 8, shift, 4 >> shift);
    return hipGetLastError();
}

template <int MODE>
__global__ void __launch_bounds__(256) rowmean3_gather_kernel(const uint16_t* __restrict__ in, int Wc, int C8, const CropDesc* __restrict__ descs,
                                                              int first, uint16_t* __restrict__ out) {
    constexpr int M = MODE == REC_SPLIT ? 2 : 1;
    const CropDesc d = descs[first + blockIdx.y];
    const int T = d.imgW / 4 - 1, xs = d.slot >> 2;
    const size_t plane = (size_t)Wc * C8 * 8 * M;
    const int total = T * C8;
    for (int i = blockIdx.x * 256 + threadIdx.x; i < total; i += gridDim.x * 256) {
        const int t = i / C8, c8 = i - t * C8;
        const uint16_t* p = in + ((size_t)(xs + t) * C8 * M + c8) * 8;
        rowmean3_8<MODE>(p, p + plane, p + 2 * plane, out + ((size_t)(d.pad_ + t) * C8 * M + c8) * 8, C8 * 8);
    }
}
hipError_t launch_rowmean3_gather(const uint16_t* in, int Wc, int C, const CropDesc* descs_dev, int first, int count, uint16_t* out, int mode,
                                  hipStream_t s) {
    if (count <= 0) return hipSuccess;
    if (mode == REC_SPLIT) hipLaunchKernelGGL(rowmean3_gather_kernel<REC_SPLIT>, dim3(8, count), dim3(256), 0, s, in, Wc, C / 8, descs_dev, first, out);
    else if (mode == REC_F16) hipLaunchKernelGGL(rowmean3_gather_kernel<REC_F16>, dim3(8, count), dim3(256), 0, s, in, Wc, C / 8, descs_dev, first, out);
    else hipLaunchKernelGGL(rowmean3_gather_kernel<REC_BF16>, dim3(8, count), dim3(256), 0, s, in, Wc, C / 8, descs_dev, first, out);
    return hipGetLastError();
}
```

bb-ocr_amd/csrc/ctx.h:

```cpp
#pragma once
#include "../../include/bbocr.h"

#include <algorithm>
#include <atomic>
#include <chrono>
#include <condition_variable>
#include <cmath>
#include <cstring>
#include <functional>
#include <map>
#include <memory>
#include <mutex>
#include <string>
#include <thread>
#include <unordered_map>
#include <vector>

#include "boxpost.h"
#include "hostpool.h"
#include "common.h"
#include "kernels.h"


using clk = std::chrono::steady_clock;
// ... 169 lines not shown

    struct ProfRec { hipEvent_t e0, e1; double flops; int group; };
    int profiling = 0;
    int prof_group = 0;
    std::vector<ProfRec> prof_recs;
    std::vector<hipEvent_t> prof_pool;
    double prof_ms[2] = {0, 0}, prof_flops[2] = {0, 0};
    long long prof_launches[2] = {0, 0};

    void* dist_comm = nullptr;
    int dist_rank = 0, dist_world = 0;
    std::unique_ptr<HostPool> pool;
    std::vector<void*> owned;
    std::vector<size_t> owned_bytes;

    Arena arena;
    DevBuf heat, gray, resized;
    DevBuf ccl_label, ccl_stat, ccl_slot, ccl_comps, ccl_rowext, ccl_counters;
    DevBuf crop_desc, crop_scratch, crop_hscratch, crop_wscratch, crop_luts, crop_hist;
    DevBuf ctc_idx, ctc_pmax, ctc_out_idx, ctc_out, ctc_probs, crop_desc2;
    PinBuf desc_pin, desc_pin2;
    PinBuf ctc_pin;
    DevBuf seq_v, seq_xp, seq_h, seq_lin, seq_logits, seq_tables;
};

inline int det_el(const bbocr_ctx* c) { return (c->cfg.precision == BBOCR_PREC_FP16 || c->cfg.precision == BBOCR_PREC_EXACT || c->cfg.precision == BBOCR_PREC_EXACT_REC) ? 1 : 0; }
inline int rec_el(const bbocr_ctx* c) { return c->cfg.precision != BBOCR_PREC_BF16 ? 1 : 0; }
inline bool rec_split(const bbocr_ctx* c) { return c->cfg.precision == BBOCR_PREC_EXACT || c->cfg.precision == BBOCR_PREC_EXACT_REC; }
inline bool det_split(const bbocr_ctx* c) { return c->cfg.precision == BBOCR_PREC_EXACT; }

struct TensorMap {
    std::unordered_map<std::string, const bbocr_tensor_desc*> m;
    bool zeros = false;
    std::vector<float> zero_buf;
    TensorMap() : zeros(true), zero_buf((size_t)5 << 20, 0.f) {}
    TensorMap(const bbocr_tensor_desc* d, int n) {
        for (int i = 0; i < n; ++i) {
            std::string k = d[i].name ? d[i].name : "";
            if (k.rfind("module.", 0) == 0) k = k.substr(7);
            m[k] = &d[i];
        }
    }
    const float* get(const std::string& name, size_t numel, bool required = true) const {
        if (zeros) {
            if (zero_buf.size() < numel) fail(BBOCR_ERR_INTERNAL, "allocation-only load: tensor '" + name + "' larger than the zero buffer");
            return zero_buf.data();
        }
        auto it = m.find(name);
        if (it == m.end()) {
            if (required) fail(BBOCR_ERR_WEIGHTS, "missing tensor '" + name + "'");
            return nullptr;
        }
        size_t n = 1;
        for (int i = 0; i < it->second->ndim; ++i) n *= (size_t)it->second->shape[i];
        if (n != numel || !it->second->data)
            fail(BBOCR_ERR_WEIGHTS, "tensor '" + name + "' has " + std::to_string(n) + " elements, expected " + std::to_string(numel));
        return it->second->data;
    }
};

struct RgbSource { const uint8_t* rgb; int Himg, Wimg; };

struct DetDims {
    int H32, W32, h, w, th, tw;
    double ratio;
};

struct HostBoxes {
    std::vector<std::vector<std::array<int, 8>>> polys;
    std::vector<std::vector<std::array<int, 4>>> hori;
    std::vector<std::vector<std::array<double, 8>>> freeb;
};

struct BoxJob {
    int img;
    bool is_free;
    double quad[8];
    CropDesc d;
    std::vector<int> text;
    double conf = 0.0;
};

struct RecChunk {
    int imgW, T, first, n;
    size_t row0;
};

struct RecPart {
    std::vector<CropDesc> descs;
    std::vector<int> order;
    std::vector<RecChunk> chunks;
    size_t rows = 0, cols = 0;
    bool any_warp = false, any_tall = false;
};

struct RecRun {
    std::vector<int> tiles, seqs, seq_k;
    size_t rows = 0;
    int n_results = 0;
};

struct RecEarly {
    bool active = false;
    int pages = 0;
    std::vector<BoxJob> jobs;
    std::vector<int> box_off;
    size_t a_total = 0, w_total = 0;
    RecPart part;
};

constexpr int REC_GAP = 4;

template <typename T> inline T* upload(bbocr_ctx* c, const std::vector<T>& v) {
    void* d = nullptr;
    HIPCHK(hipMalloc(&d, v.size() * sizeof(T)));
    c->owned.push_back(d);
    c->owned_bytes.push_back(v.size() * sizeof(T));
    HIPCHK(hipMemcpy(d, v.data(), v.size() * sizeof(T), hipMemcpyHostToDevice));
    return (T*)d;
}

ConvPlan make_plan(int Cin, int Cout, int KH, int KW, int pad, int dil, int el = 0, int bn = 0);
void upload_plan(bbocr_ctx* c, ConvPlan& p, const std::vector<float>& w, const std::vector<float>& b);
void free_weights(bbocr_ctx* c);
size_t weights_blob_bytes(const bbocr_ctx* c);
void weights_export(bbocr_ctx* c, void* dev_dst, size_t bytes);
void weights_import(bbocr_ctx* c, const void* dev_src, size_t bytes);
void load_craft(bbocr_ctx* c, const TensorMap& tm);
void load_crnn(bbocr_ctx* c, const TensorMap& tm);
ConvArgs conv_args(const ConvPlan& p, const Act& a0, const Act* a1 = nullptr, const Act* addup = nullptr);
hipError_t launch_conv_profiled(bbocr_ctx* c, const ConvPlan& p, ConvArgs a, bool may_decline = false);
void run_conv(bbocr_ctx* c, const ConvPlan& p, const Act& a0, bool relu0, const Act* a1, bool relu1, bool relu_out, void* out, int out_cs, int cout_store, bool out_f32, const Act* addup = nullptr);
void prof_collect(bbocr_ctx* c);
Act conv_act(bbocr_ctx* c, const ConvPlan& p, const Act& a0, bool relu0, const Act* a1, bool relu1, bool relu_out, int store);
Act conv_pool_act(bbocr_ctx* c, const ConvPlan& p, const Act& a0, bool relu0, bool relu_out, int store, int mode, bool pool_relu, Act* full, const RgbSource* rgb = nullptr);
Act pool_act(bbocr_ctx* c, const Act& a, int kh, int kw, int sh, int sw, int ph, int pw, bool relu_in);
void craft_up_stage(bbocr_ctx* c, const ConvPlan& py, const ConvPlan& ps, const Act& y, const Act& skip, uint16_t* z, uint16_t* out);
bool craft_up3b_post(bbocr_ctx* c, const Act& u3a, uint16_t* u3b, uint16_t* z);
bool craft_up4(bbocr_ctx* c, const Act& s1, const uint16_t* z, uint16_t* u4b);
void craft_cls_tail(bbocr_ctx* c, const Act& c2, float* heat);
DetDims det_dims(int H, int W, int canvas, double mag);
void detect_impl(bbocr_ctx* c, const uint8_t* rgb, int B, int H, int W, const bbocr_params& p, float* heat, const std::function<void(int, int)>& after_sub = nullptr);
void boxes_impl(bbocr_ctx* c, const float* heat, int B, int h, int w, double ratio, const bbocr_params& p, HostBoxes& hb, hipStream_t st);
bbocr_boxlist* export_boxes(const HostBoxes& hb);
void import_boxes(const bbocr_boxlist* bl, HostBoxes& hb);
bool plan_horizontal(const std::array<int, 4>& box, int img, int H, int W, BoxJob& j);
bool plan_free(const std::array<double, 8>& fq, int img, BoxJob& j);
int rec_mode(const bbocr_ctx* c);
void crop_refit_fw(CropDesc& d);
void rec_layout_scratch(std::vector<BoxJob>& jobs, size_t first, size_t& a_total, size_t& w_total);
bool contrast_lut(const unsigned int* hist, size_t npx, double target, uint8_t* lut);
void rec_plan_part(const std::vector<BoxJob>& jobs, const std::vector<int>& sel, int res0, size_t row_base, RecPart& part);
const CropDesc* rec_upload_descs(bbocr_ctx* c, const RecPart& part, DevBuf& desc_buf);
uint16_t* rec_wide_image(bbocr_ctx* c, const RecPart& part);
void crnn_features_wide(bbocr_ctx* c, const RecPart& part, const CropDesc* descs, const uint16_t* wide);
void rec_add_tables(RecRun& run, const RecPart& part, int tile_seqs);
void crnn_sequence(bbocr_ctx* c, size_t rows_pad, const int* tiles_dev, int ntiles, float* logits);
void ctc_size(bbocr_ctx* c, size_t rows, int nseq, int cs, bool beam);
double ctc_decode(const CtcOut& o, const int* idx, const std::vector<int>* beam_text, std::vector<int>& text);
void rec_early_begin(bbocr_ctx* c, const uint8_t* gray, int pages, int B, int H, int W, const HostBoxes& hb, const bbocr_params& p, RecEarly& e);
void recognize_impl(bbocr_ctx* c, const uint8_t* gray, int B, int H, int W, const HostBoxes& hb, const bbocr_params& p, std::vector<BoxJob>& jobs, std::vector<int>& box_off, RecEarly* early = nullptr);
bbocr_result* export_result(int B, const std::vector<BoxJob>& jobs, const std::vector<int>& box_off);
void pp_resize(bbocr_ctx* c, const uint8_t* src, int H, int W, uint8_t* dst, int dh, int dw, bool src_bgr = false);
void pp_gauss(bbocr_ctx* c, const uint8_t* src, int H, int W, uint8_t* dst, double sigma);
const uint8_t* pp_fold_lut(bbocr_ctx* c, size_t n, double contrast, double brightness);
void pp_clahe(bbocr_ctx* c, const uint8_t* src, int H, int W, const uint8_t* d_lut, uint8_t* dst, double clip_limit);
void pp_unsharp(bbocr_ctx* c, const uint8_t* src, int H, int W, uint8_t* dst, uint8_t* tmp1, uint8_t* tmp2, float radius, int percent, int threshold);
void preprocess_chain_impl(bbocr_ctx* c, const uint8_t* bgr, int H, int W, const bbocr_preproc_params& q, uint8_t* out, int dh, int dw);
void gaussian_taps_fixed(int n, double sigma, int* k);

inline HostPool& host_pool(bbocr_ctx* c) {
    if (!c->pool) {
        const int want = c->cfg.host_threads > 0 ? c->cfg.host_threads : std::min(16, host_cpu_share());
        c->pool.reset(new HostPool(std::max(1, std::min(want, 64)) - 1));
    }
    return *c->pool;
}

inline bool other_call_in_flight(bbocr_ctx* c) {
    bbocr_ctx* root = c->root;
    std::lock_guard<std::mutex> lk(root->pool_mu);
    if (root != c && root->slot_busy) return true;
    for (bbocr_ctx* s : root->slots)
        if (s != c && s->slot_busy) return true;
    return false;
}

struct EnqLock {
    std::unique_lock<std::mutex> lk;
    explicit EnqLock(bbocr_ctx* c) : lk(c->root->enq_mu) {}
};
constexpr int kMaxSlots = 2;
bbocr_ctx* slot_create(bbocr_ctx* root);
void slot_destroy(bbocr_ctx* s);
void publish_times(const bbocr_ctx* s);
void dist_release(bbocr_ctx* root);

inline void slot_sync(bbocr_ctx* c, hipStream_t st) {
    if (!c->sync_ev) HIPCHK(hipEventCreateWithFlags(&c->sync_ev, hipEventDisableTiming));
    HIPCHK(hipEventRecord(c->sync_ev, st));
    HIPCHK(hipEventSynchronize(c->sync_ev));
}

inline void prof_release(bbocr_ctx* c, const bbocr_ctx::ProfRec& r) { c->prof_pool.push_back(r.e0); c->prof_pool.push_back(r.e1); }

inline void guarded_drain(bbocr_ctx* ctx) {
    if (ctx->stream) (void)hipStreamSynchronize(ctx->stream);
    if (ctx->stream2) (void)hipStreamSynchronize(ctx->stream2);
    if (ctx->seq_stream) (void)hipStreamSynchronize(ctx->seq_stream);
    ctx->cur = ctx->stream;
    (void)hipGetLastError();
    for (auto& r : ctx->prof_recs) prof_release(ctx, r);
    ctx->prof_recs.clear();
}

struct SlotLease {
    bbocr_ctx* root;
    bbocr_ctx* slot = nullptr;
    bool exclusive;
    SlotLease(bbocr_ctx* r, bool excl) : root(r), exclusive(excl) {
        std::unique_lock<std::mutex> lk(root->pool_mu);
        const int max_slots = root->cfg.call_slots == 1 ? 1 : kMaxSlots;
        if (exclusive) {
            root->pool_cv.wait(lk, [&] {
                if (root->slot_busy) return false;
                for (bbocr_ctx* s : root->slots) if (s->slot_busy) return false;
                return true;
            });
            root->slot_busy = true;
            for (bbocr_ctx* s : root->slots) s->slot_busy = true;
            slot = root;
            return;
        }
        for (;;) {
            if (!root->slot_busy) { slot = root; break; }
            for (bbocr_ctx* s : root->slots) if (!s->slot_busy) { slot = s; break; }
            if (slot) break;
            if ((int)root->slots.size() + 1 < max_slots) {
                slot = slot_create(root);
                root->slots.push_back(slot);
                break;
            }
            root->pool_cv.wait(lk);
        }
        slot->slot_busy = true;
        if (slot != root) {
            static_cast<WeightView&>(*slot) = static_cast<const WeightView&>(*root);
            slot->cfg = root->cfg;
            slot->profiling = root->profiling;
        }
    }
    ~SlotLease() {
        {
            std::lock_guard<std::mutex> lk(root->pool_mu);
            if (exclusive) {
                root->slot_busy = false;
                for (bbocr_ctx* s : root->slots) s->slot_busy = false;
            } else if (slot) {
                slot->slot_busy = false;
            }
        }
        root->pool_cv.notify_all();
    }
};

inline void set_err(bbocr_ctx* root, const std::string& m) {
    std::lock_guard<std::mutex> lk(root->pool_mu);
    root->err = m;
}

template <typename F> inline int status_of(bbocr_ctx* root, F&& f) {
    if (!root) return BBOCR_ERR_ARG;
    try {
        f();
        return BBOCR_OK;
    } catch (const StatusError& se) {
        set_err(root, se.msg);
        return se.code;
    } catch (const std::exception& ex) {
        set_err(root, ex.what());
        return BBOCR_ERR_INTERNAL;
    } catch (...) {
        set_err(root, "unknown failure");
        return BBOCR_ERR_INTERNAL;
    }
}

template <typename F> inline int guarded(bbocr_ctx* root, F&& f, bool exclusive = false) {
    return status_of(root, [&] {
        HIPCHK(hipSetDevice(root->cfg.device));
        SlotLease lease(root, exclusive);
        bbocr_ctx* ctx = lease.slot;
        try {
            ctx->cur = ctx->stream;
            HIPCHK(hipStreamSynchronize(nullptr));
            f(ctx);
            publish_times(ctx);
        } catch (...) {
            guarded_drain(ctx);
            throw;
        }
    });
}

template <typename F> inline int lane_guarded(bbocr_ctx* root, SideLane bbocr_ctx::*which, bool wait_default, F&& f) {
    return status_of(root, [&] {
        HIPCHK(hipSetDevice(root->cfg.device));
        SideLane& lane = root->*which;
// ... 13 lines not shown
```

bb-ocr_amd/csrc/kernels.h:

```cpp
#pragma once
#include <hip/hip_runtime.h>
#include <stdint.h>
#include <vector>

struct ConvArgs {
    const uint16_t* in0;
    const uint16_t* in1;
    const uint16_t* wpk;
    const float* bias;
    void* out;
    int C0, C1;
    int in0_cs, in1_cs;
    int N, H, W, OH, OW;
    int KH, KW, pad_h, pad_w, dil;
    int TH, TW, tiles_x, tiles_y, ntiles_n;
    int PH, PW, NP;
    int relu_in0, relu_in1, relu_out, out_f32;
    int out_cs, cout_store;
    int nchunks, ntaps;
    int pool_mode, pool_relu, store_full, pool_cs;
    void* pool_out;
    const uint16_t* aux_w;
    const float* tail;
    const uint16_t* tail_frag;
    const uint16_t* post_w;
    int sub;
    int stack;
    const void* zero;
    const uint16_t* addup;
    int up_H, up_W, up_cs;
    const uint16_t* c11_w;
    const float* c11_b;
    int rgb_H, rgb_W;
    const float* aux_b;
    float acc_scale;
    int lean;
    int split_off;
};

struct ConvPlan {
    int Cin = 0, Cout = 0;
    int Cin_pad = 0, Cout_pad = 0;
    int KH = 1, KW = 1, pad_h = 0, pad_w = 0, dil = 1;
    int BN = 64;
    int el = 0;
    float acc_scale = 1.f;
    int split = 0;
    uint16_t* d_w = nullptr;
    float* d_b = nullptr;
};

int conv_plan_bn(int Cout);
size_t conv_packed_elems(const ConvPlan& p);
void pack_conv_weights(const ConvPlan& p, const float* w, uint16_t* out);
hipError_t launch_conv(const ConvPlan& p, ConvArgs a, hipStream_t s);
hipError_t launch_up4_fused(const ConvPlan& p1, const ConvPlan& p3, ConvArgs a, hipStream_t s);

void pack_post1x1_weights(const float* w , uint16_t* out , int el);
void pack_conv1_1_weights_fused(const float* w , uint16_t* out , int el);
hipError_t launch_maxpool(const uint16_t* in, uint16_t* out, int N, int H, int W, int C, int kh, int kw, int sh, int sw, int ph, int pw,
                          int relu_in, hipStream_t s);
hipError_t launch_gray(const uint8_t* rgb, uint8_t* gray, size_t npix, hipStream_t s);
hipError_t launch_ycc_to_rgb_gray(const uint8_t* ycc, int stride, uint8_t* rgb, uint8_t* gray, size_t npix, hipStream_t s);
__device__ __forceinline__ void jpeg_ycc_to_rgb(int y, int cb, int cr, uint8_t* rgb) {
    cb -= 128;
    cr -= 128;
    int r = y + ((91881 * cr + 32768) >> 16);
    int g = y + ((-22554 * cb + 32768 - 46802 * cr) >> 16);
    int b = y + ((116130 * cb + 32768) >> 16);
    rgb[0] = (uint8_t)(r < 0 ? 0 : (r > 255 ? 255 : r));
    rgb[1] = (uint8_t)(g < 0 ? 0 : (g > 255 ? 255 : g));
    rgb[2] = (uint8_t)(b < 0 ? 0 : (b > 255 ? 255 : b));
}
hipError_t launch_resize_u8(const uint8_t* src, int N, int sh, int sw, int C, uint8_t* dst, int dh, int dw, hipStream_t s);

hipError_t launch_pair_conv1_1(const uint8_t* rgb, int N, int Hi, int Wi, int H, int W, const float* w , const float* b, uint16_t* out,
                               hipStream_t s);
hipError_t launch_pair_relu(const uint16_t* in, uint16_t* out, size_t npix, int C, hipStream_t s);
hipError_t launch_pair_maxpool3x3s1(const uint16_t* in, uint16_t* out, int N, int H, int W, int C, hipStream_t s);
hipError_t launch_pair_upcat(const uint16_t* y, int yh, int yw, int Cy, const uint16_t* skip, int Cs, uint16_t* out, int N, int H, int W, hipStream_t s);
hipError_t launch_pair_cls_tail(const uint16_t* in , const float* w1 , const float* tail , float* heat,
                                size_t npix, hipStream_t s);

struct CclOut {
    int root, left, top, right, bottom, area, row_off, img;
};
hipError_t launch_ccl(const float* heat, int N, int h, int w, float low_text, float link_thr, double text_thr, int* label, int* stat,
                      int* slot, CclOut* comps, int* rowext, int* counters, int cap_comps, int cap_rows, hipStream_t s);

struct CropDesc {
    int img;
    int sx0, sy0, sw, sh;
    int rw, rh;
    int fw;
    int imgW;
    int slot;
    int warp;
    int warp_off;
    int a_off;
    int lut_off;
    int pad_;
    int rot;
    double Minv[9];
};
hipError_t launch_crops(const uint8_t* gray, int H, int W, const CropDesc* descs_dev, int first, int count, int imgW, int any_warp,
                        int any_tall, uint8_t* wscratch, uint8_t* scratch, uint8_t* hscratch, const uint8_t* luts, uint16_t* out_bucket,
                        int stage_mask, hipStream_t s, int wide_row_stride = 0, int gap = 0, int mode = 0);
enum { REC_BF16 = 0, REC_F16 = 1, REC_SPLIT = 2 };
constexpr float SPLIT_LO_SCALE = 2048.f;
hipError_t launch_crop_hist(const uint8_t* scratch, const CropDesc* descs_dev, int first, int count, unsigned int* hist, hipStream_t s);
hipError_t launch_crnn_conv0(const uint16_t* in, const float* w , const float* b, uint16_t* out, int n, int W, int mode, hipStream_t s,
                             const uint16_t* afrag = nullptr );
void pack_crnn_conv0_mfma(const float* w_tap_major , uint16_t* out , int el);
hipError_t launch_crnn_zero_gaps(uint16_t* t, const CropDesc* descs_dev, int first, int count, int H, int Wl, int C, int shift, hipStream_t s);
hipError_t launch_rowmean3_gather(const uint16_t* in, int Wc, int C, const CropDesc* descs_dev, int first, int count, uint16_t* out, int mode,
                                  hipStream_t s);
hipError_t launch_lstm(const void* xproj, const uint16_t* whh_pk, uint16_t* out, const int* tiles_dev, int ntiles, int mode, float acc_scale,
                       hipStream_t s);
int lstm_tile_seqs(int mode);
size_t lstm_whh_packed_elems();
void pack_lstm_whh8(const float* whh_fwd, const float* whh_bwd, uint16_t* out, int el);
size_t lstm_whh_split_packed_elems();
float pack_lstm_whh_split(const float* whh_fwd, const float* whh_bwd, uint16_t* out);
int lstm8_xproj_channel(int dir, int gate, int unit);
struct CtcOut { int len; int cnt; float prod; int pad; };
hipError_t launch_ctc(const float* logits, size_t rows, int C, int cs, const int* seqs_dev, int nseq, int* idx_tmp, float* pmax_tmp,
                      int* out_idx, CtcOut* out, hipStream_t s, const unsigned int* ignore = nullptr, float* probs_out = nullptr);
void ctc_beam_search_host(const float* mat, int T, int C, int cs, int beam_width, std::vector<int>& text);
class HostPool;
void ctc_beam_search_batch(const float* probs, const int* seqs, int nseq, int C, int cs, int beam_width, std::vector<std::vector<int>>& texts,
                           HostPool* pool = nullptr);

int pp_resize_tile_rows(int H, int W, int dh, int dw);
hipError_t launch_pp_resize_cubic(const uint8_t* src, int H, int W, uint8_t* dst, int dh, int dw, const int* x0, const double* wx, const long long* nx,
                                  const int* y0, const double* wy, const long long* ny, unsigned long long KX, unsigned long long KY, hipStream_t s, int src_bgr = 0);
hipError_t launch_pp_gauss3(const uint8_t* src, int H, int W, uint8_t* dst, int k0, int k1, int k2, unsigned long long* sum, hipStream_t s);
hipError_t launch_pp_clahe_hist(const uint8_t* src, int H, int W, const uint8_t* lut, int tw, int th, int tx, int ty, unsigned int* hist,
                                hipStream_t s);
hipError_t launch_pp_clahe_apply(const uint8_t* src, int H, int W, const uint8_t* lut, const uint8_t* tile_luts, int tw, int th, int tx, int ty,
                                 uint8_t* dst, hipStream_t s);
hipError_t launch_pp_box_pass(const uint8_t* src, uint8_t* dst, int H, int W, int vertical, int r, unsigned int ww, unsigned int fw, hipStream_t s);
hipError_t launch_pp_fold_lut(const unsigned long long* sum, unsigned long long n, float contrast, float brightness, uint8_t* lut, hipStream_t s);
hipError_t launch_pp_clahe_luts(const unsigned int* hist, int tiles, int clip, float lut_scale, uint8_t* tile_luts, hipStream_t s);
hipError_t launch_pp_lut(const uint8_t* src, uint8_t* dst, const uint8_t* lut, size_t total, hipStream_t s);
bool pp_unsharp_fused_ok(int H, int W, int r, const uint8_t* a, const uint8_t* b, const uint8_t* c);
hipError_t launch_pp_unsharp_fused(const uint8_t* in, uint8_t* tmp, uint8_t* dst, int H, int W, unsigned int ww, unsigned int fw, int percent,
                                   int threshold, hipStream_t s);
hipError_t launch_pp_unsharp(const uint8_t* in, const uint8_t* blur, uint8_t* dst, size_t total, int percent, int threshold, hipStream_t s);

constexpr int AC_BOX = 35, AC_BOX_R = 17, AC_MEAN_C = 10;
constexpr int AC_GAU = 31, AC_GAU_R = 15, AC_GAU_C = 5;
struct AcTaps { int k[AC_GAU]; };
hipError_t launch_ac_gray_blur(const uint8_t* src, int H, int W, size_t pitch, int channels, uint8_t* dst, hipStream_t s);
hipError_t launch_ac_cues(const uint8_t* e, int H, int W, const AcTaps& taps, uint16_t* rbox, uint16_t* rgau, uint8_t* part, uint8_t* grad,
                          unsigned int* hist, int* thr, hipStream_t s);
hipError_t launch_ac_pack(const uint8_t* e, const uint8_t* part, const uint8_t* grad, const int* thr, int H, int W, int WW, uint32_t* bits, hipStream_t s);
hipError_t launch_ac_rect(const uint32_t* src, uint32_t* tmp, uint32_t* dst, int H, int W, int WW, int rx, int ry, int erode, const uint32_t* or_with,
                          hipStream_t s);
hipError_t launch_ac_components(const uint32_t* bits, int H, int W, int WW, int* label, uint8_t* flag, int* count, int cap, int* boxes, hipStream_t s);
hipError_t launch_ac_unpack(const uint32_t* bits, const int* label, int H, int W, int WW, uint8_t* dst, hipStream_t s);

enum : int { PAGE_GRAY = 0, PAGE_BGR = 1, PAGE_RGB = 2, PAGE_YCC4 = 3, PAGE_YCC3 = 4 };
__host__ __device__ constexpr int page_px_bytes(int layout) { return layout == PAGE_GRAY ? 1 : (layout == PAGE_YCC4 ? 4 : 3); }

constexpr int TH_PRECISION_BITS = 22;
struct ThQuant { unsigned short q[2][64]; };
hipError_t launch_th_reduce(const uint8_t* src, size_t pitch, int layout, int H, int W, int fx, int fy, uint8_t* dst, int rh, int rw, int C,
                            hipStream_t s);
hipError_t launch_th_resample_h(const uint8_t* src, size_t pitch, int layout, int y0, int rows, int ow, int C, const int* bounds, const int* kk,
                                int ksize, uint8_t* dst, hipStream_t s);
hipError_t launch_th_resample_v(const uint8_t* src, size_t spitch, int y0, int width, int oh, const int* bounds, const int* kk, int ksize,
                                uint8_t* dst, size_t dpitch, hipStream_t s);
hipError_t launch_th_jpeg(const uint8_t* src, size_t pitch, int C, int H, int W, const ThQuant& q, uint8_t* yp, int wp, uint8_t* cbp, uint8_t* crp,
                          hipStream_t s);
hipError_t launch_th_upsample(const uint8_t* yp, int wp, const uint8_t* cbp, const uint8_t* crp, int H, int W, int gray_only, uint8_t* rgb,
                              uint8_t* gray, uint8_t* ycc, hipStream_t s);
hipError_t launch_th_direct(const uint8_t* src, size_t pitch, int layout, int H, int W, uint8_t* rgb, uint8_t* gray, hipStream_t s);

constexpr int JE_TILE = 256;
constexpr int JE_STUFF_TILE = 2048;
constexpr int JE_BLOCK_MAX_BITS = 22 + 63 * 26;
struct JeHuff { uint32_t dc[2][16], ac[2][256]; };
struct JeStdTable { unsigned char bits[16], vals[162]; int n; };
constexpr JeStdTable JE_STD[4] = {
    {{0, 1, 5, 1, 1, 1, 1, 1, 1, 0, 0, 0, 0, 0, 0, 0}, {0, 1, 2, 3, 4, 5, 6, 7, 8, 9, 10, 11}, 12},
    {{0, 2, 1, 3, 3, 2, 4, 3, 5, 5, 4, 4, 0, 0, 1, 0x7D},
     {0x01, 0x02, 0x03, 0x00, 0x04, 0x11, 0x05, 0x12, 0x21, 0x31, 0x41, 0x06, 0x13, 0x51, 0x61, 0x07, 0x22, 0x71, 0x14, 0x32, 0x81, 0x91, 0xA1,
      0x08, 0x23, 0x42, 0xB1, 0xC1, 0x15, 0x52, 0xD1, 0xF0, 0x24, 0x33, 0x62, 0x72, 0x82, 0x09, 0x0A, 0x16, 0x17, 0x18, 0x19, 0x1A, 0x25, 0x26,
      0x27, 0x28, 0x29, 0x2A, 0x34, 0x35, 0x36, 0x37, 0x38, 0x39, 0x3A, 0x43, 0x44, 0x45, 0x46, 0x47, 0x48, 0x49, 0x4A, 0x53, 0x54, 0x55, 0x56,
      0x57, 0x58, 0x59, 0x5A, 0x63, 0x64, 0x65, 0x66, 0x67, 0x68, 0x69, 0x6A, 0x73, 0x74, 0x75, 0x76, 0x77, 0x78, 0x79, 0x7A, 0x83, 0x84, 0x85,
      0x86, 0x87, 0x88, 0x89, 0x8A, 0x92, 0x93, 0x94, 0x95, 0x96, 0x97, 0x98, 0x99, 0x9A, 0xA2, 0xA3, 0xA4, 0xA5, 0xA6, 0xA7, 0xA8, 0xA9, 0xAA,
      0xB2, 0xB3, 0xB4, 0xB5, 0xB6, 0xB7, 0xB8, 0xB9, 0xBA, 0xC2, 0xC3, 0xC4, 0xC5, 0xC6, 0xC7, 0xC8, 0xC9, 0xCA, 0xD2, 0xD3, 0xD4, 0xD5, 0xD6,
      0xD7, 0xD8, 0xD9, 0xDA, 0xE1, 0xE2, 0xE3, 0xE4, 0xE5, 0xE6, 0xE7, 0xE8, 0xE9, 0xEA, 0xF1, 0xF2, 0xF3, 0xF4, 0xF5, 0xF6, 0xF7, 0xF8, 0xF9,
      0xFA}, 162},
    {{0, 3, 1, 1, 1, 1, 1, 1, 1, 1, 1, 0, 0, 0, 0, 0}, {0, 1, 2, 3, 4, 5, 6, 7, 8, 9, 10, 11}, 12},
    {{0, 2, 1, 2, 4, 4, 3, 4, 7, 5, 4, 4, 0, 1, 2, 0x77},
     {0x00, 0x01, 0x02, 0x03, 0x11, 0x04, 0x05, 0x21, 0x31, 0x06, 0x12, 0x41, 0x51, 0x07, 0x61, 0x71, 0x13, 0x22, 0x32, 0x81, 0x08, 0x14, 0x42,
      0x91, 0xA1, 0xB1, 0xC1, 0x09, 0x23, 0x33, 0x52, 0xF0, 0x15, 0x62, 0x72, 0xD1, 0x0A, 0x16, 0x24, 0x34, 0xE1, 0x25, 0xF1, 0x17, 0x18, 0x19,
      0x1A, 0x26, 0x27, 0x28, 0x29, 0x2A, 0x35, 0x36, 0x37, 0x38, 0x39, 0x3A, 0x43, 0x44, 0x45, 0x46, 0x47, 0x48, 0x49, 0x4A, 0x53, 0x54, 0x55,
      0x56, 0x57, 0x58, 0x59, 0x5A, 0x63, 0x64, 0x65, 0x66, 0x67, 0x68, 0x69, 0x6A, 0x73, 0x74, 0x75, 0x76, 0x77, 0x78, 0x79, 0x7A, 0x82, 0x83,
      0x84, 0x85, 0x86, 0x87, 0x88, 0x89, 0x8A, 0x92, 0x93, 0x94, 0x95, 0x96, 0x97, 0x98, 0x99, 0x9A, 0xA2, 0xA3, 0xA4, 0xA5, 0xA6, 0xA7, 0xA8,
      0xA9, 0xAA, 0xB2, 0xB3, 0xB4, 0xB5, 0xB6, 0xB7, 0xB8, 0xB9, 0xBA, 0xC2, 0xC3, 0xC4, 0xC5, 0xC6, 0xC7, 0xC8, 0xC9, 0xCA, 0xD2, 0xD3, 0xD4,
      0xD5, 0xD6, 0xD7, 0xD8, 0xD9, 0xDA, 0xE2, 0xE3, 0xE4, 0xE5, 0xE6, 0xE7, 0xE8, 0xE9, 0xEA, 0xF2, 0xF3, 0xF4, 0xF5, 0xF6, 0xF7, 0xF8, 0xF9,
      0xFA}, 162},
};
constexpr JeHuff je_std_huff() {
    JeHuff h{};
    for (int t = 0; t < 4; ++t) {
        uint32_t* out = (t & 1) ? h.ac[t >> 1] : h.dc[t >> 1];
        uint32_t code = 0;
        int k = 0;
        for (int len = 1; len <= 16; ++len) {
            for (int i = 0; i < JE_STD[t].bits[len - 1]; ++i) out[JE_STD[t].vals[k++]] = (code++ << 5) | (uint32_t)len;
            code <<= 1;
        }
    }
    return h;
}
inline int je_blocks(int H, int W, int components) {
    return components == 1 ? ((H + 7) / 8) * ((W + 7) / 8) : 6 * ((H + 15) / 16) * ((W + 15) / 16);
}
hipError_t launch_je_coef(const uint8_t* src, size_t pitch, int layout, int components, int H, int W, const ThQuant& q, short* coef, hipStream_t s);
hipError_t launch_je_sizes(const short* coef, int n, int components, unsigned int* local, unsigned long long* tile_bits, hipStream_t s);
hipError_t launch_je_scan(unsigned long long* v, int n, hipStream_t s);
hipError_t launch_je_offsets(const unsigned int* local, const unsigned long long* tile_off, int n, long long* out, hipStream_t s);
hipError_t launch_je_pack(const short* coef, int n, int components, const unsigned int* local, const unsigned long long* tile_off, uint32_t* words,
                          hipStream_t s);
hipError_t launch_je_ff_count(const uint8_t* scan, long long bytes, unsigned long long* tile_ff, hipStream_t s);
hipError_t launch_je_stuff(const uint8_t* scan, long long bytes, const unsigned long long* tile_off, uint8_t* out, hipStream_t s);

constexpr int ORIENT_TILE = 64;
bool page_orient_pair_ok(int layout, int dst_layout);
hipError_t launch_page_orient(const uint8_t* src, int H, int W, size_t pitch, int layout, int orientation, int dst_layout, uint8_t* dst,
                              size_t dst_pitch, hipStream_t s);

constexpr int JD_LANES = 64;
constexpr int JD_SUBSEQ_BITS = 1024;
struct JpegHuff {
    unsigned short look[512];
    int maxcode[18];
    int valoff[18];
    unsigned char val[256];
};
struct JpegDesc {
    const uint8_t* data;
    const int* seg_byte;
    const int* seg_sub;
    const int* sub_seg;
    unsigned long long* entry;
    unsigned long long* exits;
    int* count;
    int* scan;
    int* first;
    int* flags;
    int* status;
    short* coef;
    uint8_t* plane[3];
    uint8_t* out;
    long long pitch;
    const JpegHuff* huff;
    const unsigned short* quant;
    int W, H, ncomp, bpm, mcux, mcuy, nmcu, ri, nseg, nsub, S, nblocks, px, passes;
    int tab_dc[3], tab_ac[3];
};
enum : int { JD_ERR_SYNC = 1, JD_ERR_CODE = 2, JD_ERR_COUNT = 4 };
hipError_t launch_jd_sync(const JpegDesc* descs, int n, int max_groups, int pass, hipStream_t s);
hipError_t launch_jd_scan(const JpegDesc* descs, int n, hipStream_t s);
hipError_t launch_jd_write(const JpegDesc* descs, int n, int max_groups, hipStream_t s);
hipError_t launch_jd_dc(const JpegDesc* descs, int n, int max_seg, hipStream_t s);
// ... 3 lines not shown
```

bb-ocr_amd/csrc/recognizer.cpp:

```cpp
#include "ctx.h"

void crop_refit_fw(CropDesc& d) {
    const int cw = (int)std::ceil(64 * ((double)d.rw / (double)d.rh));
    d.fw = cw > d.imgW ? d.imgW : cw;
}

static bool plan_sizes(CropDesc& d, int width, int height) {
    double ratio = (double)width / (double)height;
    if (ratio < 1.0) {
        ratio = 1.0 / ratio;
        d.rw = 64; d.rh = (int)(64 * ratio);
    } else {
        d.rw = (int)(64 * ratio); d.rh = 64;
    }
    if ((int)(64 * ratio) == 0) return false;
    d.imgW = (int)std::ceil(std::max(ratio, 1.0)) * 64;
    crop_refit_fw(d);
    return d.rw > 0 && d.rh > 0 && d.fw > 0;
}

bool plan_horizontal(const std::array<int, 4>& box, int img, int H, int W, BoxJob& j) {
    const int x_min = std::max(0, box[0]), x_max = std::min(box[1], W), y_min = std::max(0, box[2]), y_max = std::min(box[3], H);
    const int width = x_max - x_min, height = y_max - y_min;
    if (width <= 0 || height <= 0) return false;
    j.img = img;
    j.is_free = false;
    const double q[8] = {(double)x_min, (double)y_min, (double)x_max, (double)y_min, (double)x_max, (double)y_max, (double)x_min, (double)y_max};
    memcpy(j.quad, q, sizeof(q));
    CropDesc& d = j.d;
    memset(&d, 0, sizeof(d));
    d.img = img; d.sx0 = x_min; d.sy0 = y_min; d.sw = width; d.sh = height; d.warp = 0; d.lut_off = -1;
    return plan_sizes(d, width, height);
}

bool plan_free(const std::array<double, 8>& fq, int img, BoxJob& j) {
    float rect[4][2];
    for (int i = 0; i < 4; ++i) { rect[i][0] = (float)fq[2 * i]; rect[i][1] = (float)fq[2 * i + 1]; }
    auto dist = [&](int a, int b) {
        const float dx = rect[a][0] - rect[b][0], dy = rect[a][1] - rect[b][1];
        const float t0 = dx * dx, t1 = dy * dy;
        return std::sqrt(t0 + t1);
    };
    const int maxW = std::max((int)dist(2, 3), (int)dist(1, 0));
    const int maxH = std::max((int)dist(1, 2), (int)dist(0, 3));
    if (maxW <= 0 || maxH <= 0) return false;
    j.img = img;
    j.is_free = true;
    memcpy(j.quad, fq.data(), 64);
    CropDesc& d = j.d;
    memset(&d, 0, sizeof(d));
    d.img = img; d.sx0 = 0; d.sy0 = 0; d.sw = maxW; d.sh = maxH; d.warp = 1; d.lut_off = -1;
    bbocr::perspective_inverse(rect, maxW, maxH, d.Minv);
    return plan_sizes(d, maxW, maxH);
}

int rec_mode(const bbocr_ctx* c) { return rec_split(c) ? REC_SPLIT : (rec_el(c) ? REC_F16 : REC_BF16); }
static inline int rec_mul(const bbocr_ctx* c) { return rec_split(c) ? 2 : 1; }

void crnn_features_wide(bbocr_ctx* c, const RecPart& part, const CropDesc* descs, const uint16_t* wide) {
    Arena& ar = c->arena;
    c->prof_group = 1;
    const int m = rec_mul(c), Wt = (int)part.cols, count = (int)part.descs.size();
    Act c0{ar.alloc<uint16_t>((size_t)32 * (Wt / 2) * 32 * m), 1, 32, Wt / 2, 32 * m};
    if (!ar.dry) HIPCHK(launch_crnn_conv0(wide, c->r0_wb, c->r0_wb + 288, c0.p, 1, Wt, rec_mode(c), c->cur, c->r0_afrag));
    auto gaps = [&](const Act& a, int shift) {
        if (!ar.dry) HIPCHK(launch_crnn_zero_gaps(a.p, descs, 0, count, a.H, a.W, a.C, shift, c->cur));
    };
    gaps(c0, 1);
    Act q1 = conv_pool_act(c, c->r1, c0, false, true, 64, 1, false, nullptr);
    gaps(q1, 2);
    Act c2 = conv_act(c, c->r2, q1, false, nullptr, false, true, 128);
    gaps(c2, 2);
    Act q2 = conv_pool_act(c, c->r3, c2, false, true, 128, 2, false, nullptr);
    gaps(q2, 2);
    Act c4 = conv_act(c, c->r4, q2, false, nullptr, false, true, 256);
    gaps(c4, 2);
    Act q3 = conv_pool_act(c, c->r5, c4, false, true, 256, 2, false, nullptr);
    gaps(q3, 2);
    Act c6 = conv_act(c, c->r6, q3, false, nullptr, false, true, 256);
    if (!ar.dry) HIPCHK(launch_rowmean3_gather(c6.p, c6.W, 256, descs, 0, count, (uint16_t*)c->seq_v.p, rec_mode(c), c->cur));
}

void crnn_sequence(bbocr_ctx* c, size_t rows_pad, const int* tiles_dev, int ntiles, float* logits) {
    c->prof_group = 1;
    c->arena.dry = false;
    const bool sp = rec_split(c);
    const int m = rec_mul(c);
    c->seq_xp.ensure(rows_pad * 2048 * (sp ? 4 : 2));
    c->seq_h.ensure(rows_pad * 512 * 2 * m);
    c->seq_lin.ensure(rows_pad * 256 * 2 * m);
    const int Hh = (int)(rows_pad / 256);
    Act cur{(uint16_t*)c->seq_v.p, 1, Hh, 256, 256 * m};
    for (int l = 0; l < 2; ++l) {
        run_conv(c, c->xproj[l], cur, false, nullptr, false, false, c->seq_xp.p, 2048, 2048, sp);
        HIPCHK(launch_lstm(c->seq_xp.p, c->whh[l], (uint16_t*)c->seq_h.p, tiles_dev, ntiles, rec_mode(c), c->whh_scale[l], c->cur));
        Act hh{(uint16_t*)c->seq_h.p, 1, Hh, 256, 512 * m};
        uint16_t* dst = (uint16_t*)(l == 0 ? c->seq_lin.p : c->seq_v.p);
        run_conv(c, c->lin[l], hh, false, nullptr, false, false, dst, 256 * m, 256, false);
        cur.p = dst;
    }
    run_conv(c, c->pred, cur, false, nullptr, false, false, logits, 112, 112, true);
}

static size_t rec_max_rows(const bbocr_ctx* c) { return c->cfg.rec_max_cols > 0 ? (size_t)std::max(64, c->cfg.rec_max_cols / 4) : (size_t)1500000; }

void rec_plan_part(const std::vector<BoxJob>& jobs, const std::vector<int>& sel, int res0, size_t row_base, RecPart& part) {
    std::map<int, std::vector<int>> buckets;
    for (size_t k = 0; k < sel.size(); ++k) buckets[jobs[sel[k]].d.imgW].push_back((int)k);
    size_t rows = row_base, cols = 0;
    for (auto& kv : buckets) {
        const int imgW = kv.first, T = imgW / 4 - 1;
        RecChunk ch{imgW, T, (int)part.descs.size(), (int)kv.second.size(), rows};
        for (int i = 0; i < ch.n; ++i) {
            const int k = kv.second[i];
            CropDesc d = jobs[sel[k]].d;
            if (cols > 0x7ff00000u) fail(BBOCR_ERR_OVERFLOW, "recogniser pass wider than 2^31 columns");
            d.slot = (int)cols;
            d.pad_ = (int)(rows + (size_t)i * T);
            cols += (size_t)imgW + REC_GAP;
            part.any_warp |= d.warp != 0;
            part.any_tall |= !(d.fw == d.rw && d.rh == 64);
            part.descs.push_back(d);
            part.order.push_back(res0 + k);
        }
        rows += (size_t)ch.n * T;
        part.chunks.push_back(ch);
    }
    part.rows = rows - row_base;
    part.cols = cols;
}

const CropDesc* rec_upload_descs(bbocr_ctx* c, const RecPart& part, DevBuf& desc_buf) {
    const size_t bytes = part.descs.size() * sizeof(CropDesc);
    desc_buf.ensure(bytes);
    PinBuf& pin = (&desc_buf == &c->crop_desc2) ? c->desc_pin2 : c->desc_pin;
    pin.ensure(bytes);
    memcpy(pin.p, part.descs.data(), bytes);
    HIPCHK(hipMemcpyAsync(desc_buf.p, pin.p, bytes, hipMemcpyHostToDevice, c->stream));
    return (const CropDesc*)desc_buf.p;
}

uint16_t* rec_wide_image(bbocr_ctx* c, const RecPart& part) {
    c->arena.begin(true);
    (void)c->arena.alloc<uint16_t>((size_t)64 * part.cols);
    crnn_features_wide(c, part, nullptr, nullptr);
    c->arena.buf.ensure(c->arena.off);
    c->arena.begin(false);
    return c->arena.alloc<uint16_t>((size_t)64 * part.cols);
}

static void rec_launch_part(bbocr_ctx* c, const uint8_t* gray, int H, int W, const RecPart& part, DevBuf& desc_buf, bool stage_a) {
    if (part.descs.empty()) return;
    EnqLock enq(c);
    const CropDesc* dd = rec_upload_descs(c, part, desc_buf);
    const int n = (int)part.descs.size(), Wt = (int)part.cols;
    auto crops = [&](uint16_t* wide, int stage) {
        HIPCHK(launch_crops(gray, H, W, dd, 0, n, 0, part.any_warp, part.any_tall, (uint8_t*)c->crop_wscratch.p, (uint8_t*)c->crop_scratch.p,
                            (uint8_t*)c->crop_hscratch.p, (const uint8_t*)c->crop_luts.p, wide, stage, c->stream, wide ? Wt : 0, wide ? REC_GAP : 0,
                            wide ? rec_mode(c) : 0));
    };
    if (stage_a) crops(nullptr, 1);
    uint16_t* wide = rec_wide_image(c, part);
    crops(wide, 2);
    crnn_features_wide(c, part, dd, wide);
    if (!c->feat_ev) HIPCHK(hipEventCreateWithFlags(&c->feat_ev, hipEventDisableTiming));
    HIPCHK(hipEventRecord(c->feat_ev, c->stream));
}

void rec_add_tables(RecRun& run, const RecPart& part, int tile_seqs) {
    for (const RecChunk& ch : part.chunks) {
        for (int s0 = 0; s0 < ch.n; s0 += tile_seqs) {
            run.tiles.push_back((int)(ch.row0 + (size_t)s0 * ch.T));
            run.tiles.push_back(std::min(tile_seqs, ch.n - s0));
            run.tiles.push_back(ch.T);
            run.tiles.push_back(0);
        }
        for (int i = 0; i < ch.n; ++i) {
            run.seqs.push_back((int)(ch.row0 + (size_t)i * ch.T));
            run.seqs.push_back(ch.T);
            run.seq_k.push_back(part.order[ch.first + i]);
        }
    }
    run.rows += part.rows;
}

void ctc_size(bbocr_ctx* c, size_t rows, int nseq, int cs, bool beam) {
    c->ctc_idx.ensure(rows * 4);
    c->ctc_pmax.ensure(rows * 4);
    c->ctc_out_idx.ensure(rows * 4);
    c->ctc_out.ensure((size_t)nseq * sizeof(CtcOut));
    if (beam) c->ctc_probs.ensure(rows * cs * sizeof(float));
}

double ctc_decode(const CtcOut& o, const int* idx, const std::vector<int>* beam_text, std::vector<int>& text) {
    if (beam_text) text = *beam_text;
    else text.assign(idx, idx + o.len);
    return o.cnt > 0 ? std::pow((double)o.prod, 2.0 / std::sqrt((double)o.cnt)) : 0.0;
}

static void rec_finish(bbocr_ctx* c, RecRun& run, std::vector<std::vector<int>>& texts, std::vector<double>& confs) {
    const size_t rows = run.rows;
    if (rows == 0) return;
    const size_t rows_pad = align_up(rows, 256);
    auto t0 = clk::now();
    {
        std::vector<int>& tiles = run.tiles;
        const size_t nt = tiles.size() / 4;
        std::vector<size_t> perm(nt);
        for (size_t i = 0; i < nt; ++i) perm[i] = i;
        std::stable_sort(perm.begin(), perm.end(), [&](size_t x, size_t y) { return tiles[x * 4 + 2] > tiles[y * 4 + 2]; });
        std::vector<int> t2(tiles.size());
        for (size_t i = 0; i < nt; ++i) memcpy(&t2[i * 4], &tiles[perm[i] * 4], 16);
        tiles.swap(t2);
    }
    const std::vector<int>&tiles = run.tiles, &seqs = run.seqs;
    const int ntiles = (int)(tiles.size() / 4), nseq = (int)(seqs.size() / 2);
    c->seq_logits.ensure(rows_pad * 112 * 4);
    c->seq_tables.ensure((tiles.size() + seqs.size()) * 4);
    int* tiles_dev = (int*)c->seq_tables.p;
    int* seqs_dev = tiles_dev + tiles.size();
    const bool beam = c->beam_width > 0;
    ctc_size(c, rows, nseq, 112, beam);
    const size_t oo_off = align_up(rows * 4, 16);
    c->ctc_pin.ensure(oo_off + (size_t)nseq * sizeof(CtcOut));
    const int* oidx = (const int*)c->ctc_pin.p;
    const CtcOut* oo = (const CtcOut*)((const char*)c->ctc_pin.p + oo_off);
    std::vector<float> probs(beam ? rows * 112 : 0);
    std::vector<std::vector<int>> beam_texts;
    if (!c->seq_t1) { HIPCHK(hipEventCreate(&c->seq_t1)); HIPCHK(hipEventCreate(&c->seq_t2)); }
    {
        hipStream_t ss = (c->seq_stream && c->feat_ev) ? c->seq_stream : c->stream;
        std::unique_lock<std::mutex> enq;
        if (ss == c->stream) enq = std::unique_lock<std::mutex>(c->root->enq_mu);
        else HIPCHK(hipStreamWaitEvent(ss, c->feat_ev, 0));
        c->cur = ss;
        struct Restore { bbocr_ctx* c; ~Restore() { c->cur = c->stream; } } restore{c};
        HIPCHK(hipMemcpyAsync(tiles_dev, tiles.data(), tiles.size() * 4, hipMemcpyHostToDevice, ss));
        HIPCHK(hipMemcpyAsync(seqs_dev, seqs.data(), seqs.size() * 4, hipMemcpyHostToDevice, ss));
        crnn_sequence(c, rows_pad, tiles_dev, ntiles, (float*)c->seq_logits.p);
        HIPCHK(hipEventRecord(c->seq_t1, ss));
        HIPCHK(launch_ctc((const float*)c->seq_logits.p, rows, 97, 112, seqs_dev, nseq, (int*)c->ctc_idx.p, (float*)c->ctc_pmax.p,
                          (int*)c->ctc_out_idx.p, (CtcOut*)c->ctc_out.p, ss, c->ignore_mask, beam ? (float*)c->ctc_probs.p : nullptr));
        HIPCHK(hipMemcpyAsync(c->ctc_pin.p, c->ctc_out_idx.p, rows * 4, hipMemcpyDeviceToHost, ss));
        HIPCHK(hipMemcpyAsync((char*)c->ctc_pin.p + oo_off, c->ctc_out.p, (size_t)nseq * sizeof(CtcOut), hipMemcpyDeviceToHost, ss));
        if (beam) HIPCHK(hipMemcpyAsync(probs.data(), c->ctc_probs.p, probs.size() * sizeof(float), hipMemcpyDeviceToHost, ss));
        HIPCHK(hipEventRecord(c->seq_t2, ss));
    }
    HIPCHK(hipEventSynchronize(c->seq_t2));
    float ctc_ms = 0.f;
    HIPCHK(hipEventElapsedTime(&ctc_ms, c->seq_t1, c->seq_t2));
    c->times[4] += (float)ms_since(t0) - ctc_ms;
    c->times[5] += ctc_ms;
    t0 = clk::now();
    if (beam) ctc_beam_search_batch(probs.data(), seqs.data(), nseq, 97, 112, c->beam_width, beam_texts, &host_pool(c));
    for (int i = 0; i < nseq; ++i) {
        const int k = run.seq_k[i];
        confs[k] = ctc_decode(oo[i], oidx + seqs[2 * i], beam ? &beam_texts[i] : nullptr, texts[k]);
    }
    c->times[5] += (float)ms_since(t0);
}

static std::vector<std::vector<int>> rec_split_runs(const bbocr_ctx* c, const std::vector<BoxJob>& jobs, const std::vector<int>& sel) {
    std::vector<int> byw(sel.size());
    for (size_t k = 0; k < sel.size(); ++k) byw[k] = (int)k;
    std::stable_sort(byw.begin(), byw.end(), [&](int x, int y) { return jobs[sel[x]].d.imgW < jobs[sel[y]].d.imgW; });
    std::vector<std::vector<int>> runs(1);
    size_t rows = 0;
    for (int k : byw) {
        const size_t t = (size_t)(jobs[sel[k]].d.imgW / 4 - 1);
        if (!runs.back().empty() && rows + t > rec_max_rows(c)) { runs.emplace_back(); rows = 0; }
        runs.back().push_back(k);
        rows += t;
    }
    return runs;
}

static void recognise_pass(bbocr_ctx* c, const uint8_t* gray, int H, int W, std::vector<BoxJob>& jobs, const std::vector<int>& sel,
                           bool stage_a, std::vector<std::vector<int>>& texts, std::vector<double>& confs) {
    texts.assign(sel.size(), {});
    confs.assign(sel.size(), 0.0);
    if (sel.empty()) return;
    for (const std::vector<int>& ks : rec_split_runs(c, jobs, sel)) {
        std::vector<int> sub(ks.size());
        for (size_t i = 0; i < ks.size(); ++i) sub[i] = sel[ks[i]];
        RecPart part;
        rec_plan_part(jobs, sub, 0, 0, part);
        for (size_t i = 0; i < part.order.size(); ++i) part.order[i] = ks[part.order[i]];
        auto t0 = clk::now();
        c->seq_v.ensure(align_up(part.rows, 256) * 256 * 2 * rec_mul(c));
        rec_launch_part(c, gray, H, W, part, c->crop_desc, stage_a);
        c->times[3] += (float)ms_since(t0);
        RecRun run;
        rec_add_tables(run, part, lstm_tile_seqs(rec_mode(c)));
        rec_finish(c, run, texts, confs);
    }
}

static double percentile_u8(const unsigned int* hist, size_t n, double q) {
// ... 266 lines not shown
```

include/bbocr.h:

```cpp
#ifndef BBOCR_H
#define BBOCR_H
#include <stddef.h>
#include <stdint.h>
#ifdef __cplusplus
extern "C" {
#endif

typedef struct bbocr_ctx bbocr_ctx;

enum bbocr_status {
    BBOCR_OK = 0,
    BBOCR_ERR_ARG = -1,
    BBOCR_ERR_HIP = -2,
    BBOCR_ERR_WEIGHTS = -3,
    BBOCR_ERR_STATE = -4,
    BBOCR_ERR_OVERFLOW = -5,
    BBOCR_ERR_INTERNAL = -6,
    BBOCR_ERR_DATA = -7
};

typedef struct bbocr_config {
    int device;
    int det_sub_batch;
    int rec_max_cols;
    int precision;
    int call_slots;
    int host_threads;
    int reserved[2];
} bbocr_config;
enum { BBOCR_PREC_BF16 = 0, BBOCR_PREC_FP16 = 1, BBOCR_PREC_EXACT = 2, BBOCR_PREC_MIXED = 3, BBOCR_PREC_EXACT_REC = 4 };

typedef struct bbocr_tensor_desc {
    const char* name;
    int ndim;
    int64_t shape[4];
    const float* data;
} bbocr_tensor_desc;

enum { BBOCR_DECODER_GREEDY = 0, BBOCR_DECODER_BEAMSEARCH = 1 };

typedef struct bbocr_params {
    double text_threshold;
    double low_text;
    double link_threshold;
    double mag_ratio;
    double slope_ths;
    double ycenter_ths;
    double height_ths;
    double width_ths;
    double add_margin;
    double contrast_ths;
    double adjust_contrast;
    int canvas_size;
    int min_size;
    unsigned int ignore_mask[4];
    int decoder;
    int beam_width;
    int rotation_info[4];
} bbocr_params;

typedef struct bbocr_boxlist {
    int n_images;
    int* poly_off;
    int* polys;
    int* hori_off;
    int* hori;
    int* free_off;
    double* free_q;
} bbocr_boxlist;

typedef struct bbocr_result {
    int n_images;
    int* box_off;
    double* quads;
    int* is_free;
    int* text_off;
    int* text_idx;
    double* conf;
} bbocr_result;

int bbocr_create(const bbocr_config* cfg, bbocr_ctx** out);
void bbocr_destroy(bbocr_ctx* ctx);
const char* bbocr_last_error(bbocr_ctx* ctx);
void bbocr_default_params(bbocr_params* p);

int bbocr_load_weights(bbocr_ctx* ctx, int which, const bbocr_tensor_desc* descs, int n);

int bbocr_alloc_weights(bbocr_ctx* ctx, int which );
int bbocr_weights_blob_size(bbocr_ctx* ctx, size_t* bytes);
int bbocr_weights_export(bbocr_ctx* ctx, void* dev_blob, size_t bytes);
int bbocr_weights_import(bbocr_ctx* ctx, const void* dev_blob, size_t bytes);

int bbocr_dist_unique_id(void* id128);
int bbocr_dist_init(bbocr_ctx* ctx, int rank, int world, const void* id128);
int bbocr_dist_finalize(bbocr_ctx* ctx);
int bbocr_bcast_weights(bbocr_ctx* ctx, int root);
int bbocr_scatter_images(bbocr_ctx* ctx, const uint8_t* dev_all, long long n_units, size_t unit_bytes, int root, uint8_t* dev_local, long long* first,
                         long long* count);
int bbocr_gather_results(bbocr_ctx* ctx, const void* local, size_t local_bytes, int root, void** all, size_t* sizes);
int bbocr_result_pack(const bbocr_result* r, void** bytes, size_t* n);
int bbocr_result_unpack(const void* bytes, size_t n, bbocr_result** out);
void bbocr_free_bytes(void* p);

int bbocr_detect_dims(int H, int W, int canvas_size, double mag_ratio, int* H32, int* W32, int* rh, int* rw, double* ratio);

int bbocr_detect(bbocr_ctx* ctx, const uint8_t* dev_rgb, int B, int H, int W, const bbocr_params* p, float* dev_heat_out);

int bbocr_boxes(bbocr_ctx* ctx, const float* dev_heat, int B, int h, int w, double ratio, const bbocr_params* p, bbocr_boxlist** out);

int bbocr_recognize(bbocr_ctx* ctx, const uint8_t* dev_gray, int B, int H, int W, const bbocr_boxlist* boxes, const bbocr_params* p,
                    bbocr_result** out);

int bbocr_readtext_batch(bbocr_ctx* ctx, const uint8_t* dev_rgb, const uint8_t* dev_gray, int B, int H, int W, const bbocr_params* p,
                         bbocr_result** out);

void bbocr_free_boxlist(bbocr_boxlist* b);
void bbocr_free_result(bbocr_result* r);

int bbocr_stage_times(bbocr_ctx* ctx, float* ms, int n);

int bbocr_set_profiling(bbocr_ctx* ctx, int on);
int bbocr_conv_profile(bbocr_ctx* ctx, int group, double* ms, double* flops, long long* launches);

int bbocr_host_cpu_share(void);
int bbocr_host_component_polys(const int* comps, const int* rowext, int n, int w, int h, double ratio, int* polys_out);
int bbocr_host_group_boxes(const int* polys, int n, const bbocr_params* p, bbocr_boxlist** out);
int bbocr_host_ctc_beam(const float* probs, int n, int T, int C, int cs, int beam_width, int* text_off, int* text_idx);

int bbocr_op_conv2d(bbocr_ctx* ctx, const uint16_t* dev_in, int N, int H, int W, int Cin, const float* w, const float* bias, int Cout,
                    int KH, int KW, int pad, int dil, int relu_in, int relu_out, int out_f32, void* dev_out, int pool_mode, int pool_relu,
                    uint16_t* dev_pool_out);
int bbocr_crnn_logits(bbocr_ctx* ctx, const uint16_t* dev_crops, int n, int imgW, float* dev_logits);
int bbocr_op_ctc(bbocr_ctx* ctx, const float* dev_logits, int n, int T, int C, int cs, int* text_off, int* text_idx, double* conf,
                 const unsigned int* ignore_mask, int beam_width);
int bbocr_op_resize_u8(bbocr_ctx* ctx, const uint8_t* dev_src, int N, int sh, int sw, int C, uint8_t* dev_dst, int dh, int dw);
int bbocr_op_ycc_to_rgb(bbocr_ctx* ctx, const uint8_t* dev_ycc, size_t npix, int pixel_stride, uint8_t* dev_rgb, uint8_t* dev_gray);
int bbocr_upload_pages(bbocr_ctx* ctx, const void* const* host_pages, int n, size_t bytes_each, void* dev_dst);
int bbocr_op_crops(bbocr_ctx* ctx, const uint8_t* dev_gray, int H, int W, const int* hori, int n_hori, const double* free_q, int n_free,
                   int imgW, float contrast, uint16_t* dev_out, int* n_out, int mode);

int bbocr_preprocess_book_cover(bbocr_ctx* ctx, const uint8_t* dev_bgr, int H, int W, uint8_t* dev_out, int* out_h, int* out_w);
typedef struct bbocr_preproc_params {
    double scale;
    double blur_sigma;
    double contrast;
    double brightness;
    double clahe_clip;
    double unsharp_radius;
    int unsharp_percent;
    int unsharp_threshold;
    int reserved[4];
} bbocr_preproc_params;
void bbocr_preproc_defaults(bbocr_preproc_params* p, int legacy);
int bbocr_preprocess_chain(bbocr_ctx* ctx, const uint8_t* dev_bgr, int H, int W, const bbocr_preproc_params* p, uint8_t* dev_out, int* out_h,
                           int* out_w);
int bbocr_op_preprocess_stage(bbocr_ctx* ctx, int stage, const uint8_t* dev_src, int H, int W, uint8_t* dev_dst, int dh, int dw, double param);

int bbocr_auto_crop(bbocr_ctx* ctx, const uint8_t* dev_src, int H, int W, long long pitch, int channels, int margin, int box[4], int* found,
                    int* comp_boxes, int max_comps, int* n_comps);
int bbocr_op_autocrop_stage(bbocr_ctx* ctx, int stage, const uint8_t* dev_src, int H, int W, long long pitch, int channels, uint8_t* dev_dst);

enum { BBOCR_PAGE_GRAY = 0, BBOCR_PAGE_BGR = 1, BBOCR_PAGE_RGB = 2, BBOCR_PAGE_YCBCR4 = 3, BBOCR_PAGE_YCBCR3 = 4 };
int bbocr_ocr_thumbnail(bbocr_ctx* ctx, const uint8_t* dev_src, int H, int W, long long pitch, int layout, int max_dim, int quality, uint8_t* dev_rgb,
                        uint8_t* dev_gray, int* out_h, int* out_w);
int bbocr_page_orient(bbocr_ctx* ctx, const uint8_t* dev_src, int H, int W, long long pitch, int layout, int orientation, int dst_layout,
                      uint8_t* dev_dst, long long dst_pitch, int* out_h, int* out_w);
int bbocr_op_thumbnail_stage(bbocr_ctx* ctx, int stage, const uint8_t* dev_src, int H, int W, long long pitch, int layout, int max_dim, int quality,
                             uint8_t* dev_dst, uint8_t* dev_gray, int* out_h, int* out_w);
int bbocr_thumbnail_dims(int H, int W, int max_dim, int* out_h, int* out_w);
int bbocr_host_thumbnail_plan(int H, int W, int max_dim, int* out_h, int* out_w, int factors[2], int reduce_box[4], float resize_box[4]);
int bbocr_host_resample_coeffs(int in_size, float in0, float in1, int out_size, int* bounds, int* coeffs, int max_ksize, int* ksize);
int bbocr_host_jpeg_qtables(int quality, uint16_t* out);


enum {
    BBOCR_JPEG_OK = 0,
    BBOCR_JPEG_NOT_JPEG = 1,
    BBOCR_JPEG_TRUNCATED = 2,
    BBOCR_JPEG_NO_EOI = 3,
    BBOCR_JPEG_SOF = 4,
    BBOCR_JPEG_PRECISION = 5,
    BBOCR_JPEG_COMPONENTS = 6,
    BBOCR_JPEG_SAMPLING = 7,
    BBOCR_JPEG_COLORSPACE = 8,
    BBOCR_JPEG_MULTISCAN = 9,
    BBOCR_JPEG_TABLES = 10,
    BBOCR_JPEG_RESTART = 11
};
typedef struct bbocr_jpeg_plan {
    int width, height, components;
    int sampling[3][2];
    int restart_interval;
    int mcu_cols, mcu_rows;
    int segments;
    long long scan_offset;
    long long scan_bytes;
    int supported;
    int reason;
    int orientation;
    int reserved[3];
} bbocr_jpeg_plan;
int bbocr_host_jpeg_plan(const uint8_t* file, size_t bytes, bbocr_jpeg_plan* plan);
int bbocr_jpeg_decode(bbocr_ctx* ctx, const uint8_t* const* files, const size_t* bytes, int n, int layout, uint8_t* const* dev_out,
                      const long long* pitches, int* status);
int bbocr_jpeg_imread(bbocr_ctx* ctx, const uint8_t* const* files, const size_t* bytes, int n, uint8_t* const* dev_out, const long long* pitches,
                      int* status);
int bbocr_op_jpeg_stage(bbocr_ctx* ctx, int stage, const uint8_t* file, size_t bytes, int subseq_bits, void* dev_dst, size_t dst_bytes,
                        int* file_status);

size_t bbocr_jpeg_encode_bound(int H, int W, int components);
int bbocr_host_jpeg_header(int H, int W, int components, int quality, const uint8_t* comment, int comment_bytes, uint8_t* out, size_t capacity,
                           size_t* bytes);
int bbocr_jpeg_encode(bbocr_ctx* ctx, const uint8_t* dev_src, int H, int W, long long pitch, int layout, int components, int quality,
                      const uint8_t* comment, int comment_bytes, uint8_t* host_out, size_t capacity, size_t* bytes);
int bbocr_op_jpeg_encode_stage(bbocr_ctx* ctx, int stage, const uint8_t* dev_src, int H, int W, long long pitch, int layout, int components,
                               int quality, void* dev_dst, size_t dst_bytes, size_t* bytes);

#ifdef __cplusplus
}
#endif
#endif
```

Measured before the change: 967.6.

## Fuse recogniser row-mean gather into last CRNN conv epilogue

Adds an epilogue variant to the 2x2 MFMA conv kernel that averages the three output rows (H=4 input) and scatters each column straight into the sequence buffer through a per-column map built by a small kernel. This removes the gap-zeroing pass, the full c6 activation write and read, and the separate rowmean3_gather launch in the recogniser feature path. It uses LDS exchange between waves and DPP shuffles, is limited to the 16-bit non-split mode, and adds a test entry point for comparing the fused and unfused paths.

```diff
diff --git a/bb-ocr_amd/_lib.py b/bb-ocr_amd/_lib.py
--- a/bb-ocr_amd/_lib.py
+++ b/bb-ocr_amd/_lib.py
@@ -97,6 +97,7 @@
     "bbocr_op_conv2d": (C.c_int, [_vp, _vp, C.c_int, C.c_int, C.c_int, C.c_int, C.POINTER(C.c_float), C.POINTER(C.c_float), C.c_int, C.c_int,
                                   C.c_int, C.c_int, C.c_int, C.c_int, C.c_int, C.c_int, _vp, C.c_int, C.c_int, _vp]),
     "bbocr_crnn_logits": (C.c_int, [_vp, _vp, C.c_int, C.c_int, _vp]),
+    "bbocr_op_crnn_features": (C.c_int, [_vp, _vp, C.c_int, C.POINTER(C.c_int), C.c_int, _vp, C.POINTER(C.c_longlong)]),
     "bbocr_op_ctc": (C.c_int, [_vp, _vp, C.c_int, C.c_int, C.c_int, C.c_int, C.POINTER(C.c_int), C.POINTER(C.c_int), C.POINTER(C.c_double),
                                C.POINTER(C.c_uint), C.c_int]),
     "bbocr_op_resize_u8": (C.c_int, [_vp, _vp, C.c_int, C.c_int, C.c_int, C.c_int, _vp, C.c_int, C.c_int]),
diff --git a/bb-ocr_amd/csrc/abi_ops.cpp b/bb-ocr_amd/csrc/abi_ops.cpp
--- a/bb-ocr_amd/csrc/abi_ops.cpp
+++ b/bb-ocr_amd/csrc/abi_ops.cpp
@@ -151,6 +151,42 @@
     });
 }
 
+int bbocr_op_crnn_features(bbocr_ctx* ctx, const uint16_t* dev_crops, int n, const int* imgW, int fused, uint16_t* dev_rows, long long* arena_bytes) {
+    return guarded(ctx, [&](bbocr_ctx* ctx) {
+        if (!ctx->crnn_loaded) fail(BBOCR_ERR_STATE, "recogniser weights not loaded");
+        if (rec_split(ctx)) fail(BBOCR_ERR_ARG, "the 16-bit recogniser modes only");
+        if (!dev_crops || !imgW || !dev_rows || n <= 0) fail(BBOCR_ERR_ARG, "bad crop batch");
+        RecPart part;
+        for (int i = 0; i < n; ++i) {
+            if (imgW[i] < 64 || (imgW[i] & 63)) fail(BBOCR_ERR_ARG, "crop widths are multiples of 64");
+            CropDesc d{};
+            d.imgW = imgW[i]; d.slot = (int)part.cols; d.pad_ = (int)part.rows;
+            part.cols += (size_t)imgW[i] + REC_GAP;
+            part.rows += (size_t)(imgW[i] / 4 - 1);
+            if (part.cols > 0x7ff00000u) fail(BBOCR_ERR_OVERFLOW, "recogniser pass wider than 2^31 columns");
+            part.descs.push_back(d);
+            part.order.push_back(i);
+        }
+        const size_t row_bytes = part.rows * 256 * 2;
+        ctx->seq_v.ensure(align_up(part.rows, 256) * 256 * 2);
+        HIPCHK(hipMemsetAsync(ctx->seq_v.p, 0xff, row_bytes, ctx->stream));
+        const CropDesc* dd = rec_upload_descs(ctx, part, ctx->crop_desc);
+        size_t dry = 0;
+        uint16_t* wide = rec_wide_image(ctx, part, fused != 0, &dry);
+        HIPCHK(hipMemsetAsync(wide, 0, 64 * part.cols * 2, ctx->stream));
+        size_t src = 0;
+        for (int i = 0; i < n; ++i) {
+            HIPCHK(hipMemcpy2DAsync(wide + part.descs[i].slot, part.cols * 2, dev_crops + src, (size_t)imgW[i] * 2, (size_t)imgW[i] * 2, 64,
+                                    hipMemcpyDeviceToDevice, ctx->stream));
+            src += (size_t)64 * imgW[i];
+        }
+        crnn_features_wide(ctx, part, dd, wide, fused != 0);
+        if (arena_bytes) { arena_bytes[0] = (long long)dry; arena_bytes[1] = (long long)ctx->arena.off; }
+        HIPCHK(hipMemcpyAsync(dev_rows, ctx->seq_v.p, row_bytes, hipMemcpyDeviceToDevice, ctx->stream));
+        slot_sync(ctx, ctx->stream);
+    });
+}
+
 int bbocr_op_ctc(bbocr_ctx* ctx, const float* dev_logits, int n, int T, int C, int cs, int* text_off, int* text_idx, double* conf,
                  const unsigned int* ignore_mask, int beam_width) {
     return guarded(ctx, [&](bbocr_ctx* ctx) {
diff --git a/bb-ocr_amd/csrc/common.h b/bb-ocr_amd/csrc/common.h
--- a/bb-ocr_amd/csrc/common.h
+++ b/bb-ocr_amd/csrc/common.h
@@ -76,6 +76,11 @@
 };
 __device__ __forceinline__ s16x8 sm16_key(s16x8 x) { return x ^ ((x >> 15) & (short)0x7fff); }
 
+template <class E> __device__ __forceinline__ unsigned int rowmean3_pair(unsigned int a, unsigned int b, unsigned int c) {
+    const f32x2_t m = (E::unpack2(a) + E::unpack2(b) + E::unpack2(c)) / 3.0f;
+    return E::pack2(m[0], m[1]);
+}
+
 __device__ __forceinline__ int xcd_remap(int bid, int nblk) {
     const int q = nblk >> 3, r = nblk & 7, x = bid & 7, i = bid >> 3;
     return (x < r ? x * (q + 1) : r * (q + 1) + (x - r) * q) + i;
diff --git a/bb-ocr_amd/csrc/conv_mfma.hip b/bb-ocr_amd/csrc/conv_mfma.hip
--- a/bb-ocr_amd/csrc/conv_mfma.hip
+++ b/bb-ocr_amd/csrc/conv_mfma.hip
@@ -352,6 +352,72 @@
 }
 
 template <int EL, int MF>
+__device__ __forceinline__ void conv_epilogue_rowmean3(const ConvArgs& a, f32x4 (&acc)[MF][4], int nt, int ox0, int wm, int wn, int lane, int BN,
+                                                       unsigned char* xch) {
+    static_assert(MF == 8, "two tile rows per wave, four fragments each");
+    const int g = lane >> 4, pl = lane & 15;
+    const int cout0 = nt * BN + wn * 64 + g * 8;
+    const float sc = a.acc_scale;
+    float bs[16];
+#pragma unroll
+    for (int h = 0; h < 2; ++h)
+#pragma unroll
+        for (int q = 0; q < 2; ++q) {
+            const f32x4 b4 = *(const f32x4*)(a.bias + cout0 + h * 32 + q * 4);
+            bs[h * 8 + q * 4 + 0] = b4[0]; bs[h * 8 + q * 4 + 1] = b4[1]; bs[h * 8 + q * 4 + 2] = b4[2]; bs[h * 8 + q * 4 + 3] = b4[3];
+        }
+    auto finish = [&](int f, u32x4& lo, u32x4& hi) {
+        float v[16];
+#pragma unroll
+        for (int j = 0; j < 4; ++j)
+#pragma unroll
+            for (int r = 0; r < 4; ++r) {
+                float x = fmaf(acc[f][j][r], sc, bs[j * 4 + r]);
+                if (a.relu_out) x = fmaxf(x, 0.f);
+                v[j * 4 + r] = x;
+            }
+        lo = (u32x4){El<EL>::pack2(v[0], v[1]), El<EL>::pack2(v[2], v[3]), El<EL>::pack2(v[4], v[5]), El<EL>::pack2(v[6], v[7])};
+        hi = (u32x4){El<EL>::pack2(v[8], v[9]), El<EL>::pack2(v[10], v[11]), El<EL>::pack2(v[12], v[13]), El<EL>::pack2(v[14], v[15])};
+    };
+    u32x4* const xq = (u32x4*)xch + wn * (4 * 2 * 64) + lane;
+    asm volatile("s_waitcnt lgkmcnt(0)\n\ts_barrier" ::: "memory");
+    if (wm == 1) {
+#pragma unroll
+        for (int f = 0; f < 4; ++f) {
+            u32x4 lo, hi;
+            finish(f, lo, hi);
+            xq[(f * 2) * 64] = lo;
+            xq[(f * 2 + 1) * 64] = hi;
+        }
+    }
+    asm volatile("s_waitcnt lgkmcnt(0)\n\ts_barrier" ::: "memory");
+    if (wm != 0) return;
+    typedef El<EL> E;
+#pragma unroll
+    for (int f = 0; f < 4; ++f) {
+        u32x4 a0, a1, b0, b1, lo, hi, dA, dB;
+        finish(f, a0, a1);
+        finish(f + 4, b0, b1);
+        const u32x4 c0 = xq[(f * 2) * 64], c1 = xq[(f * 2 + 1) * 64];
+#pragma unroll
+        for (int j = 0; j < 4; ++j) {
+            lo[j] = rowmean3_pair<E>(a0[j], b0[j], c0[j]);
+            hi[j] = rowmean3_pair<E>(a1[j], b1[j], c1[j]);
+        }
+#pragma unroll
+        for (int i = 0; i < 4; ++i) {
+            dA[i] = (unsigned)__builtin_amdgcn_update_dpp((int)lo[i], (int)hi[i], 0x118 , 0xF, 0xC, false);
+            dB[i] = (unsigned)__builtin_amdgcn_update_dpp((int)hi[i], (int)lo[i], 0x108 , 0xF, 0x3, false);
+        }
+        const int co = cout0 + (pl >> 3) * 32;
+        const int xA = ox0 + f * 16 + (pl & 7), xB = xA + 8;
+        const int rA = xA < a.OW ? a.rowmean_map[xA] : -1, rB = xB < a.OW ? a.rowmean_map[xB] : -1;
+        if (rA >= 0) *(u32x4*)(a.rowmean_out + (size_t)rA * a.out_cs + co) = dA;
+        if (rB >= 0) *(u32x4*)(a.rowmean_out + (size_t)rB * a.out_cs + co) = dB;
+    }
+}
+
+template <int EL, int MF>
 __device__ __forceinline__ void conv_epilogue_post1x1(const ConvArgs& a, f32x4 (&acc)[MF][4], int n, int oy0, int ox0, int wm, int fpr, int lane) {
     const int g = lane >> 4, pl = lane & 15;
     const int cout0 = g * 8;
@@ -588,7 +654,8 @@
 template <int EL, int WM, int WN, int MF, int NPB, int RING, int NPS = NPB * 64, bool FUSE1 = false, int NF = 4, int EPI = 0, int KS = 3>
 __global__ void __launch_bounds__(WM * WN * 64, 2) conv3x3_dma_kernel(const ConvArgs a) {
     constexpr int NTAP = KS * KS, PAD = KS == 3 ? 1 : 0;
-    static_assert((KS == 3 || KS == 2) && (KS == 3 || (!FUSE1 && EPI == 0)), "kernel size");
+    static_assert((KS == 3 || KS == 2) && (KS == 3 || (!FUSE1 && (EPI == 0 || EPI == 2))), "kernel size");
+    static_assert(EPI != 2 || (KS == 2 && WM == 2 && WN == 2 && MF == 8 && NPS * 64 >= 16 * 1024), "row-mean epilogue: the 4 x 64 tile of the 128-cout configuration");
     constexpr int NW = WM * WN, NT = NW * 64, BN = WN * 64;
     static_assert(NW == 4, "one wave per 8-channel group of the patch");
     constexpr int WBUF = BN * 64, WPIECES = WBUF / 16, WPT = WPIECES / NT;
@@ -882,6 +949,7 @@
     chunk(std::false_type{}, a.nchunks - 1);
     if constexpr (FUSE1) conv_epilogue_pool2x2_lean<EL, MF>(a, acc, cur.n, cur.oy0, cur.ox0, wm, lane);
     else if constexpr (EPI == 1) conv_epilogue_post1x1<EL, MF>(a, acc, cur.n, cur.oy0, cur.ox0, wm, fpr, lane);
+    else if constexpr (EPI == 2) conv_epilogue_rowmean3<EL, MF>(a, acc, cur.nt, cur.ox0, wm, wn, lane, BN, pbuf);
     else if constexpr (KS == 3 && NF == 4) {
         if (a.lean == 1) conv_epilogue_plain_lean<EL, MF>(a, acc, cur.n, cur.nt, cur.oy0, cur.ox0, wm, wn, fpr, lane, BN);
         else if (a.lean == 3) conv_epilogue_pool2x2_lean<EL, MF>(a, acc, cur.n, cur.oy0, cur.ox0, wm, lane, cur.nt * BN + wn * 64);
@@ -1409,6 +1477,11 @@
     return hipErrorInvalidValue;
 }
 
+bool conv_rowmean3_ok(const ConvPlan& p, int N, int H, int W, int cout_store) {
+    return p.KH == 2 && p.KW == 2 && p.dil == 1 && p.pad_h == 0 && p.pad_w == 0 && p.BN == 128 && !p.split && N == 1 && H == 4 && W >= 2 &&
+           cout_store == p.Cout_pad && p.Cout_pad % 128 == 0;
+}
+
 int conv_plan_bn(int Cout) {
     return Cout > 64 ? 128 : 64;
 }
@@ -1425,6 +1498,9 @@
     a.ntaps = p.KH * p.KW;
     a.sub = 1;
     if (a.post_w && !(a.zero && p.KH == 3 && p.KW == 3 && p.dil == 1 && p.pad_h == 1 && p.pad_w == 1 && BN == 64 && p.Cout_pad == 64))
+        return hipErrorNotSupported;
+    if (a.rowmean_map && !(a.zero && a.rowmean_out && conv_rowmean3_ok(p, a.N, a.H, a.W, a.cout_store) && !a.C1 && !a.out_f32 && !a.split_off &&
+                           !a.pool_mode && !a.tail && !a.addup && !a.post_w && !a.relu_in0 && a.out_cs % 8 == 0))
         return hipErrorNotSupported;
     if (a.zero && !a.pool_mode && p.KH == 3 && p.KW == 3 && p.dil > 1 && p.pad_h == p.dil && p.pad_w == p.dil) {
         const int d = p.dil, LH = cdiv(a.OH, d), LW = cdiv(a.OW, d);
@@ -1492,6 +1568,7 @@
         return hipErrorInvalidValue;
     if (p.KH == 1 && p.KW == 1 && p.pad_h == 0 && p.pad_w == 0 && a.zero && !a.pool_mode)
         return BN == 256 ? launch_dma1x1<EL, 2, 4, 8>(a, s) : (BN == 128 ? launch_dma1x1<EL, 2, 2, 8>(a, s) : launch_dma1x1<EL, 4, 1, 4>(a, s));
+    if (dma2x2 && a.rowmean_map) return launch_dma_one<EL, 2, 2, 8, 6, 4, 384, false, 4, 2, 2>(a, grid, s);
     if (dma2x2)
         return BN == 128 ? launch_dma_one<EL, 2, 2, 8, 6, 4, 384, false, 4, 0, 2>(a, grid, s) : launch_dma_one<EL, 4, 1, 4, 6, 3, 384, false, 4, 0, 2>(a, grid, s);
     if (p.KH == 3 && p.KW == 3 && p.dil == 1 && p.pad_h == 1 && p.pad_w == 1 && a.zero) {
diff --git a/bb-ocr_amd/csrc/crnn_misc.hip b/bb-ocr_amd/csrc/crnn_misc.hip
--- a/bb-ocr_amd/csrc/crnn_misc.hip
+++ b/bb-ocr_amd/csrc/crnn_misc.hip
@@ -415,10 +415,7 @@
         *(u32x4*)(o + lo_off) = ol;
     } else {
 #pragma unroll
-        for (int j = 0; j < 4; ++j) {
-            const f32x2_t m = (E::unpack2(a[j]) + E::unpack2(bq[j]) + E::unpack2(c[j])) / 3.0f;
-            oh[j] = E::pack2(m[0], m[1]);
-        }
+        for (int j = 0; j < 4; ++j) oh[j] = rowmean3_pair<E>(a[j], bq[j], c[j]);
         *(u32x4*)(o) = oh;
     }
 }
@@ -462,3 +459,15 @@
     else hipLaunchKernelGGL(rowmean3_gather_kernel<REC_BF16>, dim3(8, count), dim3(256), 0, s, in, Wc, C / 8, descs_dev, first, out);
     return hipGetLastError();
 }
+
+__global__ void __launch_bounds__(256) rowmean3_map_kernel(const CropDesc* __restrict__ descs, int first, int Wc, int* __restrict__ map) {
+    const CropDesc d = descs[first + blockIdx.x];
+    const int T = d.imgW / 4 - 1, xs = d.slot >> 2;
+    for (int t = threadIdx.x; t < T + 2; t += 256)
+        if (xs + t < Wc) map[xs + t] = t < T ? d.pad_ + t : -1;
+}
+hipError_t launch_rowmean3_map(const CropDesc* descs_dev, int first, int count, int Wc, int* map, hipStream_t s) {
+    if (count <= 0) return hipSuccess;
+    hipLaunchKernelGGL(rowmean3_map_kernel, dim3(count), dim3(256), 0, s, descs_dev, first, Wc, map);
+    return hipGetLastError();
+}
diff --git a/bb-ocr_amd/csrc/ctx.h b/bb-ocr_amd/csrc/ctx.h
--- a/bb-ocr_amd/csrc/ctx.h
+++ b/bb-ocr_amd/csrc/ctx.h
@@ -345,8 +345,8 @@
 bool contrast_lut(const unsigned int* hist, size_t npx, double target, uint8_t* lut);
 void rec_plan_part(const std::vector<BoxJob>& jobs, const std::vector<int>& sel, int res0, size_t row_base, RecPart& part);
 const CropDesc* rec_upload_descs(bbocr_ctx* c, const RecPart& part, DevBuf& desc_buf);
-uint16_t* rec_wide_image(bbocr_ctx* c, const RecPart& part);
-void crnn_features_wide(bbocr_ctx* c, const RecPart& part, const CropDesc* descs, const uint16_t* wide);
+uint16_t* rec_wide_image(bbocr_ctx* c, const RecPart& part, bool fused = true, size_t* dry_bytes = nullptr);
+void crnn_features_wide(bbocr_ctx* c, const RecPart& part, const CropDesc* descs, const uint16_t* wide, bool fused = true);
 void rec_add_tables(RecRun& run, const RecPart& part, int tile_seqs);
 void crnn_sequence(bbocr_ctx* c, size_t rows_pad, const int* tiles_dev, int ntiles, float* logits);
 void ctc_size(bbocr_ctx* c, size_t rows, int nseq, int cs, bool beam);
diff --git a/bb-ocr_amd/csrc/kernels.h b/bb-ocr_amd/csrc/kernels.h
--- a/bb-ocr_amd/csrc/kernels.h
+++ b/bb-ocr_amd/csrc/kernels.h
@@ -36,6 +36,8 @@
     float acc_scale;
     int lean;
     int split_off;
+    const int* rowmean_map;
+    uint16_t* rowmean_out;
 };
 
 struct ConvPlan {
@@ -54,6 +56,7 @@
 size_t conv_packed_elems(const ConvPlan& p);
 void pack_conv_weights(const ConvPlan& p, const float* w, uint16_t* out);
 hipError_t launch_conv(const ConvPlan& p, ConvArgs a, hipStream_t s);
+bool conv_rowmean3_ok(const ConvPlan& p, int N, int H, int W, int cout_store);
 hipError_t launch_up4_fused(const ConvPlan& p1, const ConvPlan& p3, ConvArgs a, hipStream_t s);
 
 void pack_post1x1_weights(const float* w , uint16_t* out , int el);
@@ -115,6 +118,7 @@
 hipError_t launch_crnn_zero_gaps(uint16_t* t, const CropDesc* descs_dev, int first, int count, int H, int Wl, int C, int shift, hipStream_t s);
 hipError_t launch_rowmean3_gather(const uint16_t* in, int Wc, int C, const CropDesc* descs_dev, int first, int count, uint16_t* out, int mode,
                                   hipStream_t s);
+hipError_t launch_rowmean3_map(const CropDesc* descs_dev, int first, int count, int Wc, int* map, hipStream_t s);
 hipError_t launch_lstm(const void* xproj, const uint16_t* whh_pk, uint16_t* out, const int* tiles_dev, int ntiles, int mode, float acc_scale,
                        hipStream_t s);
 int lstm_tile_seqs(int mode);
diff --git a/bb-ocr_amd/csrc/recognizer.cpp b/bb-ocr_amd/csrc/recognizer.cpp
--- a/bb-ocr_amd/csrc/recognizer.cpp
+++ b/bb-ocr_amd/csrc/recognizer.cpp
@@ -57,7 +57,7 @@
 int rec_mode(const bbocr_ctx* c) { return rec_split(c) ? REC_SPLIT : (rec_el(c) ? REC_F16 : REC_BF16); }
 static inline int rec_mul(const bbocr_ctx* c) { return rec_split(c) ? 2 : 1; }
 
-void crnn_features_wide(bbocr_ctx* c, const RecPart& part, const CropDesc* descs, const uint16_t* wide) {
+void crnn_features_wide(bbocr_ctx* c, const RecPart& part, const CropDesc* descs, const uint16_t* wide, bool fused) {
     Arena& ar = c->arena;
     c->prof_group = 1;
     const int m = rec_mul(c), Wt = (int)part.cols, count = (int)part.descs.size();
@@ -76,6 +76,17 @@
     Act c4 = conv_act(c, c->r4, q2, false, nullptr, false, true, 256);
     gaps(c4, 2);
     Act q3 = conv_pool_act(c, c->r5, c4, false, true, 256, 2, false, nullptr);
+    if (fused && !rec_split(c) && conv_rowmean3_ok(c->r6, q3.N, q3.H, q3.W, 256)) {
+        const int Wc = q3.W - 1;
+        int* map = ar.alloc<int>((size_t)Wc);
+        if (ar.dry) return;
+        HIPCHK(launch_rowmean3_map(descs, 0, count, Wc, map, c->cur));
+        ConvArgs a = conv_args(c->r6, q3);
+        a.relu_out = 1; a.out_cs = 256; a.cout_store = 256;
+        a.rowmean_map = map; a.rowmean_out = (uint16_t*)c->seq_v.p;
+        (void)launch_conv_profiled(c, c->r6, a);
+        return;
+    }
     gaps(q3, 2);
     Act c6 = conv_act(c, c->r6, q3, false, nullptr, false, true, 256);
     if (!ar.dry) HIPCHK(launch_rowmean3_gather(c6.p, c6.W, 256, descs, 0, count, (uint16_t*)c->seq_v.p, rec_mode(c), c->cur));
@@ -140,10 +151,11 @@
     return (const CropDesc*)desc_buf.p;
 }
 
-uint16_t* rec_wide_image(bbocr_ctx* c, const RecPart& part) {
+uint16_t* rec_wide_image(bbocr_ctx* c, const RecPart& part, bool fused, size_t* dry_bytes) {
     c->arena.begin(true);
     (void)c->arena.alloc<uint16_t>((size_t)64 * part.cols);
-    crnn_features_wide(c, part, nullptr, nullptr);
+    crnn_features_wide(c, part, nullptr, nullptr, fused);
+    if (dry_bytes) *dry_bytes = c->arena.off;
     c->arena.buf.ensure(c->arena.off);
     c->arena.begin(false);
     return c->arena.alloc<uint16_t>((size_t)64 * part.cols);
diff --git a/include/bbocr.h b/include/bbocr.h
--- a/include/bbocr.h
+++ b/include/bbocr.h
@@ -131,6 +131,7 @@
                     int KH, int KW, int pad, int dil, int relu_in, int relu_out, int out_f32, void* dev_out, int pool_mode, int pool_relu,
                     uint16_t* dev_pool_out);
 int bbocr_crnn_logits(bbocr_ctx* ctx, const uint16_t* dev_crops, int n, int imgW, float* dev_logits);
+int bbocr_op_crnn_features(bbocr_ctx* ctx, const uint16_t* dev_crops, int n, const int* imgW, int fused, uint16_t* dev_rows, long long* arena_bytes);
 int bbocr_op_ctc(bbocr_ctx* ctx, const float* dev_logits, int n, int T, int C, int cs, int* text_off, int* text_idx, double* conf,
                  const unsigned int* ignore_mask, int beam_width);
 int bbocr_op_resize_u8(bbocr_ctx* ctx, const uint8_t* dev_src, int N, int sh, int sw, int C, uint8_t* dev_dst, int dh, int dw);
```

New measurement: 970.2 (median of 5 runs). No clear change (+0.3%).
